# SMLC-NYSBC/TARGET-VAE

Hardware: AMD Instinct MI355X
Metric: training images/sec (fwd+bwd+Adam), P8 z=2 64x64 bs=256/GPU (higher is better)
Workload: dtype f32 (matrix products: operands as TWO fp16 parts under one power-of-two scale PER ROW of the operand (row / column of the product), 3 fp16 MFMAs per product block -- 2 where one operand is the exact 0 / 1 matrix -- fp32 accumulate: at least as accurate against fp64 as the fp32 matrix pipe (profiles/

## Files before the change

include/tvae_hip.h:

```cpp
#ifndef TVAE_HIP_H
#define TVAE_HIP_H
#ifdef __cplusplus
extern "C" {
#endif

typedef void* tvae_stream_t;

int tvae_abi_version(void);


int tvae_rotate_bank_fwd(const float* weight, const int* tap_idx, const float* tap_w, float* bank, int C, int Cin,
                         int ksz, int R, tvae_stream_t stream);
int tvae_rotate_bank_bwd(const float* dbank, const int* csr_ptr, const int* csr_r, const int* csr_dst,
                         const float* csr_w, float* dweight, int C, int Cin, int ksz, int R, int accumulate,
                         tvae_stream_t stream);

int tvae_conv1_fwd(const float* y, const float* bank, const float* bias, float* out, int B, int Cin, int n, int ksz,
                   int pad, int C, int R, int act, float slope, tvae_stream_t stream);
int tvae_conv1_wgrad(const float* y, const float* dpre, float* dbank, float* ws, long ws_floats, int B, int Cin,
                     int n, int ksz, int pad, int C, int R, tvae_stream_t stream);

int tvae_linear_fwd(const float* W, const float* X, const float* bias, const float* gbias, int group,
                    const float* res, float* Y, int M, int N, int K, long ldx, long ldy, int act, float slope,
                    tvae_stream_t stream);
int tvae_linear_dgrad(const float* W, const float* dpre, const float* add, const float* aux, float* dX, int M, int N,
                      int K, long ldd, long ldx, int mask, float slope, tvae_stream_t stream);
int tvae_linear_wgrad(const float* dpre, const float* X, float* dW, float* ws, long ws_floats, int M, int N, int K,
                      long ldd, long ldx, int accumulate, tvae_stream_t stream);

int tvae_rowdot_seg(const float* X, long ldx, const float* V, int no, int M, int N, int seglen, float* out, float* amax,
                    tvae_stream_t stream);
int tvae_seg_sum(const float* in, int S, long L, float* out, float scale, int accumulate, tvae_stream_t stream);
int tvae_coldot(const float* X, long ldx, int M, int N, const float* W, int wsm, int wso, const float* bias, int no,
                float* out, tvae_stream_t stream);
int tvae_outer_mask(const float* dy, int no, const float* W, int wsm, int wso, const float* H, long ldh, float* D,
                    long ldd, int M, int N, int act, float slope, tvae_stream_t stream);
int tvae_act_bwd(const float* dY, const float* Y, float* dpre, long n, int act, float slope, tvae_stream_t stream);

int tvae_conv1_x6_supported(int Cin, int n, int ksz, int pad);
long tvae_conv1_x6_bank_bytes(int C, int R, int Cin, int ksz);
long tvae_conv1_x6_dy_bytes(int B, int C, int R, int n, int ksz, int pad);
int tvae_bank_split3(const float* bank, void* a3, long a3_bytes, int C, int R, int Cin, int ksz, tvae_stream_t stream);
int tvae_conv1_fwd_x6(const float* y, const void* a3, const float* bias, float* out, int B, int Cin, int n, int ksz,
                      int pad, int C, int R, int act, float slope, tvae_stream_t stream);
int tvae_dy_split3(const float* dpre, void* d3, long d3_bytes, int B, int Cin, int n, int ksz, int pad, int C, int R,
                   tvae_stream_t stream);
int tvae_conv1_wgrad_x6(const float* y, const void* d3, float* dbank, float* ws, long ws_floats, int B, int Cin, int n,
                        int ksz, int pad, int C, int R, tvae_stream_t stream);

int tvae_conv1_dft_supported(int B, int Cin, int n, int ksz, int pad, int C, int R);
long tvae_conv1_dft_at_floats(int B, int Cin, int n, int ksz, int pad, int C, int R);
long tvae_conv1_dft_ws_floats(int B, int Cin, int n, int ksz, int pad, int C, int R);
int tvae_conv1_dft_frame(int B, int Cin, int n, int ksz, int pad, int C, int R);
int tvae_conv1_dft_ring(int B, int Cin, int n, int ksz, int pad, int C, int R);
int tvae_conv1_dft_route(int B, int Cin, int n, int ksz, int pad, int C, int R, int parts, int which);
int tvae_conv1_fwd_dft(const float* y, const float* bank, const float* bias, float* out, float* at, float* ws,
                       long ws_floats, int B, int Cin, int n, int ksz, int pad, int C, int R, int act, float slope,
                       int parts, tvae_stream_t stream);
int tvae_conv1_wgrad_dft(const float* dpre, const float* at, float* dbank, float* dbias, float* ws, long ws_floats, int B,
                         int Cin, int n, int ksz, int pad, int C, int R, int parts, tvae_stream_t stream);

long tvae_dense_x6_bytes(int rows, int K);
int tvae_dense_split3(const float* W, long ldw, void* a3, long a3_bytes, int rows, int K, int transpose,
                      const float* scale, float* rowsum, tvae_stream_t stream);
int tvae_dense_split2h(const float* W, long ldw, void* a3, long a3_bytes, int rows, int K, int transpose,
                       const float* scale, float* rowsum, tvae_stream_t stream);
int tvae_linear_fwd_x6(const void* w3, const float* X, const float* bias, const float* res, float* Y, int M, int N,
                       int K, long ldx, long ldy, int act, float slope, const float* col_w, const float* col_b,
                       float* col_y, const float* va_xr, const float* va_wc, const float* va_bc, const float* va_lb,
                       int va_np, void* sign_bits, int parts, const float* x_amax, float* y_amax, tvae_stream_t stream);
int tvae_linear_dgrad_x6(const void* w3t, const float* dpre, const float* add, const float* aux, float* dX, int M,
                         int N, int K, long ldd, long ldx, int mask, float slope, const float* in_xr,
                         const float* in_wc, float* in_gxr, float* in_part, long in_part_floats, const float* vg_wo,
                         const float* vg_gy, const float* vg_csum, const float* in_bc, const float* in_lb, int in_np,
                         float* rs_part, long rs_part_floats, const float* rs_wo, const float* rs_gysum, float* rs_db,
                         float* rs_dwo, int parts, const void* vg_bits, const float* rs_rowdot, const float* rs_bias,
                         const float* x_amax, float* y_amax, tvae_stream_t stream);
int tvae_dgrad_rowsum_total(const float* rs_part, int ntiles, int M, const float* rs_wo, const float* rs_gysum, float slope,
                            float* rs_db, float* rs_dwo, const float* rs_rowdot, const float* rs_bias, tvae_stream_t stream);
int tvae_dec_in_total(float* part, int B, int cpi, int F, float* Simg, float* dbc, float* dWc, tvae_stream_t stream);
long tvae_linear_wgrad_x6_ws_floats(int M, int N, int K);
int tvae_linear_wgrad_x6(const float* dpre, const float* X, float* dW, float* ws, long ws_floats, int M, int N, int K,
                         long ldd, long ldx, int accumulate, const float* vg_wo, const float* vg_gy, int vg_act,
                         float vg_slope, const float* va_xr, const float* va_wc, const float* va_bc, const float* va_lb,
                         int va_np, const void* vg_bits, int parts, const float* rd_w, long rd_ldw, float* rd_rowdot,
                         const float* a_amax, const float* x_amax, int x_amax_rows, tvae_stream_t stream);

int tvae_dec_out_bwd(const float* gy, int n_out, const float* Wo, const float* H, long ldh, float* D, long ldd, int F,
                     long N, int act, float slope, float* part, long part_floats, float* tot, tvae_stream_t stream);
int tvae_dec_in_bwd(const float* d, long ldd, const float* xr, const float* Wc, int F, int B, int Np, float* gxr,
                    float* Simg, float* dbc, float* dWc, float* part, long part_floats, tvae_stream_t stream);
int tvae_heads_fwd(const float* W, const float* X, long ldx, const float* bias, float* Y, long ldy, int nh, int C,
                   long N, tvae_stream_t stream);
int tvae_heads_bwd(const float* W, const float* dY, long ldy, const float* X, long ldx, float* dX, long lddx, int nh,
                   int C, long N, int act, float slope, float* part, long part_floats, float* tot,
                   tvae_stream_t stream);

int tvae_attn_head_fwd(const float* heads, long ldh, const float* E, const float* eps_z, const float* eps_t,
                       const float* p_r, const float* off, const float* p_tr, const float* grid, int B, int R, int P,
                       int zd, float sigma_p, float theta_off_scale, float* attn, float* q, float* a, float* z,
                       float* theta, float* dx, float* kl, float* part, long part_floats, tvae_stream_t stream);
int tvae_attn_head_bwd(const float* heads, long ldh, const float* q, const float* a, const float* eps_z,
                       const float* eps_t, const float* p_r, const float* off, const float* p_tr, const float* grid,
                       int B, int R, int P, int zd, float sigma_p, float theta_off_scale, const float* gz,
                       const float* gth, const float* gdx, const float* gkl, const float* g_attn, const float* g_q,
                       const float* g_a, float* dheads, float* part, long part_floats, tvae_stream_t stream);

int tvae_rot_pool_fwd(const float* A1, const float* fw, const float* fb, float* X, int C, int B, int R, int P,
                      tvae_stream_t stream);
int tvae_rot_pool_bwd(const float* A1, const float* dX, const float* fw, float* dA1, float* part, long part_floats,
                      float* dtot, int C, int B, int R, int P, int act, float slope, tvae_stream_t stream);

int tvae_enc_tail_fwd_x6(const void* w3, const float* A1, long lda, const float* b2, const float* Wh, const float* bh,
                         int nh, float* H, long ldh, float* heads, long ldo, void* bits_h, void* bits_a, int C, long N,
                         int act, float slope, int parts, const float* amax_a1, tvae_stream_t stream);
int tvae_enc_tail_dgrad_x6(const void* w3p, const void* wh3, const float* dheads, long ldd, int nh, const void* bits_h,
                           const void* bits_a, float* dA1, long lda, int C, long N, float slope, int parts,
                           tvae_stream_t stream);
long tvae_enc_tail_wgrad_x6_ws_floats(long N);
int tvae_enc_tail_wgrad_x6(const float* A1, long lda, const float* dheads, long ldd, int nh, const void* bits_h,
                           const float* Wh, float* dW2, float* ws, long ws_floats, int C, long N, float slope, int parts, const float* amax_a1,
                           tvae_stream_t stream);
int tvae_enc_tail_wide_max_rows(void);
int tvae_enc_tail_fwd_wide(const void* w3, const void* wh3, const float* A1, long lda, const float* b2, const float* bh, int nh,
                           float* H, long ldh, float* heads, long ldo, void* bits_h, void* bits_a, int C, long N, int act,
                           float slope, int parts, const float* amax_a1, tvae_stream_t stream);
int tvae_enc_tail_dgrad_wide(const void* wht3, const void* w3p, const float* dheads, long ldd, int nh, const void* bits_h,
                             const void* bits_a, float* dH, long ldh, float* dA1, long lda, int C, long N, float slope,
                             int parts, const float* amax_dheads, tvae_stream_t stream);
int tvae_enc_tail_wgrad_wide(const float* D, long ldd, int rows_d, const float* A, long lda, float* dW, float* ws,
                             long ws_floats, int C, long N, const float* amax_d, const float* amax_a, tvae_stream_t stream);
int tvae_get_latent(const float* heads, long ldh, const float* p_r, const float* off, const float* grid, int B, int R,
                    int P, int zd, float theta_off_scale, float* zc, float* theta_mu, float* dx, tvae_stream_t stream);

int tvae_coord_fwd(const float* xc, const float* dx, const float* theta, float* xr, int B, int Np,
                   tvae_stream_t stream);
int tvae_coord_bwd(const float* xc, const float* dx, const float* theta, const float* gxr, float* gdx, float* gtheta,
                   int B, int Np, tvae_stream_t stream);

int tvae_dec_l0_fwd(const float* xr, const float* Wc, const float* bc, const float* LB, float* h, long ldh, int F,
                    long Ntot, int Np, int act, float slope, tvae_stream_t stream);
int tvae_latent_bias(const float* Wl, const float* z, float* LB, int B, int F, int zd, tvae_stream_t stream);
int tvae_latent_bwd(const float* S, const float* Wl, const float* z, float* dWl, float* dz, int B, int F, int zd,
                    tvae_stream_t stream);
int tvae_fourier_fwd(const float* xr, const float* Wf, const float* bf, float sigma, float* feat, long ld, int F,
                     long Ntot, tvae_stream_t stream);
int tvae_fourier_bwd(const float* xr, const float* Wf, const float* bf, float sigma, const float* dfeat, long ld,
                     int F, long Ntot, float* gxr, tvae_stream_t stream);

int tvae_loglik_fwd(const float* yh, const float* y, float* lp, int B, int L, int kind, tvae_stream_t stream);
int tvae_loglik_bwd(const float* yh, const float* y, const float* glp, float* gyh, int B, int L, int kind,
                    tvae_stream_t stream);

int tvae_elbo_reduce(const float* lp, const float* kl, int B, double* elbo, float* logp, double* kld, tvae_stream_t stream);
int tvae_elbo_reduce_bwd(const double* g_elbo, const float* g_logp, const double* g_kld, int B, float* g_lp, float* g_kl,
                         tvae_stream_t stream);

int tvae_rccl_available(void);
int tvae_rccl_unique_id(void* id128);
int tvae_rccl_comm_init(void** comm, int nranks, const void* id128, int rank);
int tvae_allreduce_flat(void* comm, float* buf, long count, tvae_stream_t stream);
// ... 16 lines not shown
```

target-vae_amd/csrc/abi_common.hpp:

```cpp
#pragma once
#include <hip/hip_runtime.h>

#include <cstdlib>

#include "../../include/tvae_hip.h"
#include "gemm_f32_mfma.hpp"

#define TVAE_CHECK_LAUNCH()                      \
    do {                                         \
        hipError_t e__ = hipGetLastError();      \
        if (e__ != hipSuccess) return (int)e__;  \
    } while (0)

#define TVAE_INTERNAL __attribute__((visibility("hidden")))

namespace tvae {

static inline hipStream_t S(tvae_stream_t s) { return (hipStream_t)s; }
static inline bool aligned16(const void* p) { return (reinterpret_cast<size_t>(p) & 15) == 0; }
static inline int grid1d(long total, int block, int cap = 8192) {
    long g = (total + block - 1) / block;
    if (g < 1) g = 1;
    if (g > cap) g = cap;
    return (int)g;
}
template <class KernelT>
static hipError_t allow_big_lds(KernelT kernel, size_t bytes) {
    if (bytes <= 48 * 1024) return hipSuccess;
    return hipFuncSetAttribute(reinterpret_cast<const void*>(kernel), hipFuncAttributeMaxDynamicSharedMemorySize,
                               (int)bytes);
}
static inline int pick_splits(int tiles, long K) {
    long want = (1024 + tiles - 1) / tiles;
    long maxs = K / (4 * BK);
    if (maxs < 1) maxs = 1;
    if (want > maxs) want = maxs;
    if (want < 1) want = 1;
    return (int)want;
}
static inline int panels_of(long N, int width) { return (int)((N + width - 1) / width); }

static inline ConvGeom make_geom(int B, int Cin, int n, int ksz, int pad, int R) {
    ConvGeom g;
    g.B = B; g.Cin = Cin; g.n = n; g.ksz = ksz; g.pad = pad; g.R = R;
    g.Ho = n + 2 * pad - ksz + 1;
    g.P = g.Ho * g.Ho;
    g.K2 = ksz * ksz;
    return g;
}

static const size_t X6_LDS_MAX = 160 * 1024;

TVAE_INTERNAL int splitk_finalize(const float* ws, int splits, int M, int N, const Epilogue& ep, hipStream_t stream);

template <class AL, class BL>
static hipError_t launch_gemm(AL al, BL bl, const Epilogue& ep, int M, int N, int K, int splits_wanted,
                              float* ws, long ws_floats, hipStream_t stream) {
    if (M <= 0 || N <= 0) return hipSuccess;
    const int tilesM = cdiv(M, BM), tilesN = cdiv(N, BN);
    int splits = splits_wanted < 1 ? 1 : splits_wanted;
    if (splits > 1) {
        const long per = (long)M * N;
        const long cap = ws ? ws_floats / per : 0;
        if (cap < 2) splits = 1; else if (splits > cap) splits = (int)cap;
        if (splits > 65535) splits = 65535;
    }
    int kchunk = cdiv(cdiv(K > 0 ? K : 1, splits), BK) * BK;
    splits = cdiv(K > 0 ? K : 1, kchunk);
    const TileMap tm{tilesM, tilesN, splits};
    float* wsp = splits > 1 ? ws : nullptr;
    hipLaunchKernelGGL((gemm_f32_kernel<AL, BL>), dim3(tm.grid()), dim3(GEMM_THREADS), 0, stream, al, bl, ep, M, N, K,
                       kchunk, wsp, tm);
    hipError_t e = hipGetLastError();
    if (e != hipSuccess) return e;
    if (splits > 1) e = (hipError_t)splitk_finalize(ws, splits, M, N, ep, stream);
    return e;
}

}
```

target-vae_amd/csrc/abi_conv_dft.hip:

```cpp
#include "abi_dense_x6.hpp"
#include "conv_dft_kernels.hpp"
#include "conv_dft_h3_kernels.hpp"

using namespace tvae;

static __global__ void dft_zero_kernel(float4* __restrict__ p, long n4, float* __restrict__ tail, int ntail) {
    const float4 z = make_float4(0.f, 0.f, 0.f, 0.f);
    for (long i = (long)blockIdx.x * blockDim.x + threadIdx.x; i < n4; i += (long)gridDim.x * blockDim.x) p[i] = z;
    if (blockIdx.x == 0 && (int)threadIdx.x < ntail) tail[threadIdx.x] = 0.f;
}
static hipError_t dft_zero(float* p, long floats, hipStream_t st) {
    const long n4 = floats / 4;
    const int ntail = (int)(floats - 4 * n4);
    long blocks = (n4 + 255) / 256;
    if (blocks < 1) blocks = 1;
    if (blocks > 4096) blocks = 4096;
    hipLaunchKernelGGL(dft_zero_kernel, dim3((unsigned)blocks), dim3(256), 0, st, reinterpret_cast<float4*>(p), n4, p + 4 * n4,
                       ntail);
    return hipGetLastError();
}

static int dev_cu_count() {
    int dev = 0, n = 0;
    if (hipGetDevice(&dev) != hipSuccess) return 256;
// ... 374 lines not shown
    hipLaunchKernelGGL(dft_out_gen_kernel<N_>, dim3(grid), dim3(256), 0, st, (const float*)T, (const float*)EO, bias, out, \
                       q.M, R, B, q.Ho, q.Lh, q.NBpad, act, slope, a1max)
            switch (r_out - DFT_R_OUT_GEN) {
                case 1: TVAE_OUT_GEN(1); break;
                case 2: TVAE_OUT_GEN(2); break;
                case 3: TVAE_OUT_GEN(3); break;
                case 4: TVAE_OUT_GEN(4); break;
                default: TVAE_OUT_GEN(5); break;
            }
#undef TVAE_OUT_GEN
            TVAE_CHECK_LAUNCH();
            return 0;
        }
        if (r_out <= DFT_R_OUT_MF || r_out > DFT_R_OUT_MF + 9) return (int)hipErrorInvalidValue;
        const int mf_l = (r_out - DFT_R_OUT_MF - 1) / 3, mf_v = (r_out - DFT_R_OUT_MF - 1) % 3;
        const size_t lds_o = ((size_t)q.LHP * NTT * 64 + (size_t)4 * 32 * (q.Ho | 1)) * 4;
        const int grid = (int)((ntiles + 3) / 4 < 768 ? (ntiles + 3) / 4 : 768);
        const int iters = (int)((ntiles + 4L * grid - 1) / (4L * grid));
#define TVAE_OUT_MF(L_, N_, R_)                                                                                     \
    do {                                                                                                            \
        e = allow_big_lds(dft_out_mf_kernel<L_, N_, R_>, lds_o);                                                    \
        if (e != hipSuccess) return (int)e;                                                                         \
        hipLaunchKernelGGL((dft_out_mf_kernel<L_, N_, R_>), dim3(grid), dim3(256), lds_o, st, (const float*)T,      \
                           (const float*)EO, bias, out, q.M, R, B, q.Ho, q.Lh, q.NBpad, act, slope, iters, a1max); \
    } while (0)
#define TVAE_OUT_MF_L(L_)                                                                                           \
    do {                                                                                                            \
        if (mf_v == 1) TVAE_OUT_MF(L_, 1, true); else if (mf_v == 0) TVAE_OUT_MF(L_, 1, false); else TVAE_OUT_MF(L_, 2, false); \
    } while (0)
        if (mf_l == 0) TVAE_OUT_MF_L(23); else if (mf_l == 1) TVAE_OUT_MF_L(49); else TVAE_OUT_MF_L(64);
#undef TVAE_OUT_MF_L
#undef TVAE_OUT_MF
        TVAE_CHECK_LAUNCH();
    }
    return 0;
}

int tvae_conv1_wgrad_dft(const float* dpre, const float* at, float* dbank, float* dbias, float* ws, long ws_floats, int B,
                         int Cin, int n, int ksz, int pad, int C, int R, int parts, tvae_stream_t stream) {
    const DftPlan q = dft_plan(B, Cin, n, ksz, pad, C, R);
    const int r_dy = dft_route(q, parts, DFT_STEP_DY), r_wg = dft_route(q, parts, DFT_STEP_WGRAD_GEMM);
    if (r_dy < 0 || r_wg < 0 || ws_floats < tvae_conv1_dft_ws_floats(B, Cin, n, ksz, pad, C, R) || !aligned16(ws) ||
        !aligned16(at))
        return (int)hipErrorInvalidValue;
    hipStream_t st = S(stream);
    float* amax = const_cast<float*>(at) + ((q.at_floats + 3) & ~3L);
    float* smax = amax + q.o_smax;
    constexpr bool bf16_store = true;
    const bool s16 = bf16_store && parts == 1 && q.ring;
    const int rc0 = h3_zero_slots(smax, q.M, 256, st);
    if (rc0) return rc0;
    float* Sp = ws;
    float* slabs = Sp + ((q.t_floats + 3) & ~3L);
    float* tab = slabs + (((long)(q.splits > q.wsplits ? q.splits : q.wsplits) * q.g_floats + 3) & ~3L);
    float* EO = tab;
    float* ED = EO + ((q.eo_floats + 3) & ~3L);
    {
        hipLaunchKernelGGL(dft_wtab_kernel, dim3(64), dim3(256), 0, st, EO, ED, q.L, q.Lh, q.Ho, q.LHP, q.NT,
                           q.NT + q.REM1, q.NS, q.NRT, q.mixed ? 1.f / (float)q.L : 1.f / ((float)q.L * (float)q.L));
        TVAE_CHECK_LAUNCH();
        const long ntiles = (long)q.M * (q.NBpad / 32);
        if (r_dy == q.ring) {
            const int cus = dev_cu_count();
            const int grid = (int)((ntiles + 3) / 4 < 2 * cus ? (ntiles + 3) / 4 : 2 * cus);
            hipError_t er = hipSuccess;
#define TVAE_DY_RING_ONE(S_, T_, L2_, H_, Q_, S16_)                                                                  \
    do {                                                                                                            \
        const size_t lds_r = (size_t)4 * 2 * ((32 * H_ + 63) / 64) * 256;                                           \
        er = allow_big_lds(dft_dy_ring_kernel<S_, T_, L2_, H_, Q_, S16_>, lds_r);                                   \
        if (er != hipSuccess) return (int)er;                                                                       \
        hipLaunchKernelGGL((dft_dy_ring_kernel<S_, T_, L2_, H_, Q_, S16_>), dim3(grid), dim3(256), lds_r, st, dpre, \
                           (const float*)ED, Sp, q.M, R, B, q.Lh, q.NBpad, smax);                                   \
    } while (0)
#define TVAE_DY_RING(S_, T_, L2_, H_, Q_)                                                                           \
    do { if (s16) TVAE_DY_RING_ONE(S_, T_, L2_, H_, Q_, true); else TVAE_DY_RING_ONE(S_, T_, L2_, H_, Q_, false); } while (0)
            if (q.ring == 1) TVAE_DY_RING(9, 2, 38, 17, false);
            else if (q.ring == 2) TVAE_DY_RING(17, 3, 82, 33, false);
            else if (q.ring == 3) TVAE_DY_RING(20, 2, 62, 39, false);
            else if (q.ring == 4) TVAE_DY_RING(9, 2, 46, 17, false);
            else if (q.ring == 5) TVAE_DY_RING(17, 3, 98, 33, true);
            else TVAE_DY_RING(20, 3, 68, 39, false);
#undef TVAE_DY_RING
#undef TVAE_DY_RING_ONE
            TVAE_CHECK_LAUNCH();
        } else if (r_dy == DFT_R_H3) {
            uint4* EOc = reinterpret_cast<uint4*>(ED + ((q.ed_floats + 3) & ~3L) + ((q.M + 3) & ~3L));
            uint4* EDc = EOc + q.eoc_floats / 4;
            hipLaunchKernelGGL(dft_wtab_h3_kernel, dim3(64), dim3(256), 0, st, EOc, EDc, q.L, q.Lh, q.Ho, OH3_KS, OH3_NWT, DH3_WS,
                               DH3_NKT, q.mixed ? 1.f / (float)q.L : 1.f / ((float)q.L * (float)q.L));
            TVAE_CHECK_LAUNCH();
            const size_t lds_h = ((size_t)((32 * (q.Ho | 1) + 3) & ~3) + 2 * 2 * DH3_WS * 32 * 4 + 32) * 4;
            hipError_t eh = allow_big_lds(dft_dy_h3_kernel<DH3_WS, DH3_NKT, DH3_NLD>, lds_h);
            if (eh != hipSuccess) return (int)eh;
            const int cus = dev_cu_count();
            const int gridh = (int)(ntiles < 2L * cus ? ntiles : 2L * cus);
            hipLaunchKernelGGL((dft_dy_h3_kernel<DH3_WS, DH3_NKT, DH3_NLD>), dim3(gridh), dim3(64 * DH3_NKT), lds_h, st, dpre,
                               (const uint4*)EDc, Sp, q.M, R, B, q.Ho, q.Lh, q.NBpad, ldexpf(1.f, -14), smax);
            TVAE_CHECK_LAUNCH();
        } else if (r_dy >= DFT_R_DY_WIDE50 && r_dy <= DFT_R_DY_WIDE80) {
            const int NSR = r_dy == DFT_R_DY_WIDE50 ? 50 : (r_dy == DFT_R_DY_WIDE66 ? 66 : DFT_WIDE_NS);
            const size_t lds_w = (size_t)2 * (32 * (q.Ho | 1) + 2 * NSR + 2) * 4;
            const int cus = dev_cu_count();
            const long fit = (long)(150 * 1024 / lds_w);
            const long wg_per_cu = fit < 2 ? fit : 2;
            const int gridw = (int)(ntiles < wg_per_cu * cus ? ntiles : wg_per_cu * cus);
            hipError_t ew = hipSuccess;
#define TVAE_DY_WIDE(NSR_, NLD_, WPE_)                                                                               \
    do {                                                                                                            \
        ew = allow_big_lds(dft_dy_wide_kernel<NSR_, NLD_, WPE_>, lds_w);                                            \
        if (ew != hipSuccess) return (int)ew;                                                                       \
        hipLaunchKernelGGL((dft_dy_wide_kernel<NSR_, NLD_, WPE_>), dim3(gridw), dim3(64 * q.NRT), lds_w, st, dpre,  \
                           (const float*)ED, Sp, q.M, R, B, q.Ho, q.Lh, q.NBpad, q.NS, q.NRT, smax);                \
    } while (0)
            if (NSR == 50) TVAE_DY_WIDE(50, 16, 2);
            else if (NSR == 66) TVAE_DY_WIDE(66, 16, 2);
            else TVAE_DY_WIDE(DFT_WIDE_NS, 16, 2);
#undef TVAE_DY_WIDE
            TVAE_CHECK_LAUNCH();
        } else if (r_dy == DFT_R_DY_GEN) {
            const size_t lds_g = (size_t)4 * 32 * ((2 * q.NS) | 1) * 4;
            hipError_t eg = allow_big_lds(dft_dy_gen_kernel, lds_g);
            if (eg != hipSuccess) return (int)eg;
            const int gridg = (int)((ntiles + 3) / 4 < 4096 ? (ntiles + 3) / 4 : 4096);
            hipLaunchKernelGGL(dft_dy_gen_kernel, dim3(gridg), dim3(256), lds_g, st, dpre, (const float*)ED, Sp, q.M, R, B,
                               q.Ho, q.Lh, q.NBpad, q.NS, q.NRT, smax);
            TVAE_CHECK_LAUNCH();
        } else {
        if (r_dy <= DFT_R_DY_MF || r_dy > DFT_R_DY_MF + 5) return (int)hipErrorInvalidValue;
        const size_t lds_d = ((size_t)q.NS * q.NRT * 64 + (size_t)4 * (32 * ((2 * q.NS) | 1) + 64)) * 4;
        const int grid = (int)((ntiles + 3) / 4 < 768 ? (ntiles + 3) / 4 : 768);
        const int iters = (int)((ntiles + 4L * grid - 1) / (4L * grid));
        hipError_t e0 = hipSuccess;
#define TVAE_DY_MF(S_, T_, L2_, A_)                                                                                 \
    do {                                                                                                            \
        e0 = allow_big_lds(dft_dy_mf_kernel<S_, T_, L2_, A_>, lds_d);                                               \
        if (e0 != hipSuccess) return (int)e0;                                                                       \
        hipLaunchKernelGGL((dft_dy_mf_kernel<S_, T_, L2_, A_>), dim3(grid), dim3(256), lds_d, st, dpre,             \
                           (const float*)ED, Sp, q.M, R, B, q.Ho, q.Lh, q.NBpad, iters,                             \
                           smax);                                                        \
    } while (0)
        switch (r_dy - DFT_R_DY_MF) {
            case 1: TVAE_DY_MF(9, 2, 46, true); break;
            case 2: TVAE_DY_MF(9, 2, 0, true); break;
            case 3: TVAE_DY_MF(17, 4, 98, true); break;
            case 4: TVAE_DY_MF(17, 4, 0, true); break;
            default: TVAE_DY_MF(32, 4, 0, false); break;
        }
#undef TVAE_DY_MF
        TVAE_CHECK_LAUNCH();
        }
    }
    if (dbias) {
        float* dbpart = ED + ((q.ed_floats + 3) & ~3L);
        hipLaunchKernelGGL(dft_dbias_rows_kernel, dim3(q.M), dim3(256), 0, st, (const float*)Sp, dbpart, q.Lh, q.NB, q.M,
                           s16 ? 1 : 0);
        TVAE_CHECK_LAUNCH();
        hipLaunchKernelGGL(dft_dbias_kernel, dim3((C + 63) / 64), dim3(64), 0, st, (const float*)dbpart, dbias, R, C);
        TVAE_CHECK_LAUNCH();
    }
    const bool wide = r_wg == DFT_R_WG_WIDE;
    const int nslabs = wide ? q.wsplits : q.splits;
    {
        const int M2 = 2 * q.M;
        const int tiles_b = wide ? M2 / WW_ROWS : q.Mb / DX6_ROWS, tilesM = q.Lh * tiles_b;
        const int tilesK = wide ? (q.K2 <= 160 ? 1 : cdiv(q.K2, 192)) : cdiv(q.K2, 128);
        const int splits = nslabs;
        const int nchunk = cdiv(cdiv((int)q.NBpad, splits), 16) * 16;
        const TileMap tmk{tilesM, tilesK, splits};
        const DenseBatch bt{tiles_b, (long)q.K2 * q.NBpad, 0};
        int rc = dense_wgrad_x6_batched(Sp, (long)q.Lh * 128, at, q.NBpad, slabs, M2, q.K2, (int)q.NBpad, nchunk, tmk, bt,
                                        128L, ATile{7, 127, (long)M2 * q.Lh * 128}, parts, st,
                                        H3Scale{smax, amax + q.o_fmax, 1, 0, q.M, 1 << 30, 1}, s16, wide);
        if (rc) return rc;
    }
    constexpr bool dbank_mf = true;
    if (q.mixed) {
        hipError_t e = allow_big_lds(dft_dbank_x_kernel, q.lds_db);
        if (e != hipSuccess) return (int)e;
        hipLaunchKernelGGL(dft_dbank_x_kernel, dim3(q.M * Cin), dim3(256), q.lds_db, st, (const float*)slabs, nslabs, q.g_floats,
                           dbank, ksz, q.L, q.Lh, q.M, Cin);
    } else if (dbank_mf && ksz <= 64 && q.FXBd >= 17 && q.FXBd <= 64) {
        hipError_t e = allow_big_lds(dft_dbank_mf_kernel, q.lds_db);
        if (e != hipSuccess) return (int)e;
        hipLaunchKernelGGL(dft_dbank_mf_kernel, dim3(q.M * Cin), dim3(256), q.lds_db, st, (const float*)slabs, nslabs,
                           q.g_floats, dbank, ksz, q.L, q.Lh, q.M, Cin, q.FXBd);
    } else {
        hipError_t e = allow_big_lds(dft_dbank_kernel, q.lds_db);
        if (e != hipSuccess) return (int)e;
        hipLaunchKernelGGL(dft_dbank_kernel, dim3(q.M * Cin), dim3(256), q.lds_db, st, (const float*)slabs, nslabs, q.g_floats,
                           dbank, ksz, q.L, q.Lh, q.M, Cin, q.FXBd);
    }
    TVAE_CHECK_LAUNCH();
    return 0;
}

}
```

target-vae_amd/csrc/abi_dense_wgrad_x6.hip:

```cpp
#include "abi_dense_x6.hpp"

using namespace tvae;

namespace tvae {
static __global__ void dense_absmax_kernel(const float* __restrict__ W, long ldw, int Rrows, int K, int transpose,
                                           const float* __restrict__ scale, float* __restrict__ amax) {
    const long total = (long)Rrows * K;
    float mx = 0.f;
    if (!scale && (transpose ? ldw == Rrows : ldw == K) && (reinterpret_cast<size_t>(W) & 15) == 0) {
        const float4* w4 = reinterpret_cast<const float4*>(W);
        const long n4 = total / 4, gsz = (long)gridDim.x * blockDim.x;
        for (long i = (long)blockIdx.x * blockDim.x + threadIdx.x; i < n4; i += gsz) {
            const float4 v = w4[i];
            mx = fmaxf(fmaxf(mx, fabsf(v.x)), fmaxf(fabsf(v.y), fmaxf(fabsf(v.z), fabsf(v.w))));
        }
        for (long i = 4 * n4 + (long)blockIdx.x * blockDim.x + threadIdx.x; i < total; i += gsz) mx = fmaxf(mx, fabsf(W[i]));
        h3_block_amax(mx, amax);
        return;
    }
    for (long i = (long)blockIdx.x * blockDim.x + threadIdx.x; i < total; i += (long)gridDim.x * blockDim.x) {
        const int k = transpose ? (int)(i / Rrows) : (int)(i % K);
        const int row = transpose ? (int)(i % Rrows) : (int)(i / K);
        float v = transpose ? W[(long)k * ldw + row] : W[(long)row * ldw + k];
        if (scale) v *= scale[k];
        mx = fmaxf(mx, fabsf(v));
    }
    h3_block_amax(mx, amax);
}

int dense_wgrad_x6_batched(const float* dY, long ldd, const float* X, long ldx, float* slabs, int M, int Kf, int N,
                           int nchunk, const TileMap& tm, const DenseBatch& bt, long dy_stride, const ATile& atile,
                           int parts, hipStream_t st, H3Scale hs, bool a_bf16, bool wide) {
    const VirtGrad vg{nullptr, nullptr, 0, 0.f, nullptr, nullptr, nullptr, 0};
    const VirtAct va{nullptr, nullptr, nullptr, nullptr, 1, 0, 0.f};
    if (a_bf16) {
        if (parts != 1 || dy_stride % 2 != 0) return (int)hipErrorInvalidValue;
        return dense_wgrad_x6_launch_p1_abf(0, dY, ldd, X, ldx, slabs, M, Kf, N, nchunk, tm, bt, dy_stride, vg, va, atile, st, hs);
    }
    if (wide) {
        if (parts == 2 && hs.amax_a && hs.amax_x)
            return dense_wgrad_x6_wide_p2(dY, ldd, X, ldx, slabs, M, Kf, N, nchunk, tm, bt, dy_stride, atile, st, hs);
        if (parts == 3) return dense_wgrad_x6_wide_p3(dY, ldd, X, ldx, slabs, M, Kf, N, nchunk, tm, bt, dy_stride, atile, st, hs);
        return (int)hipErrorInvalidValue;
    }
    if (parts == 1) return dense_wgrad_x6_launch_p1(0, dY, ldd, X, ldx, slabs, M, Kf, N, nchunk, tm, bt, dy_stride, vg, va, atile, st, hs);
    if (parts == 2 && hs.amax_a && hs.amax_x)
        return dense_wgrad_x6_launch_p2(0, dY, ldd, X, ldx, slabs, M, Kf, N, nchunk, tm, bt, dy_stride, vg, va, atile, st, hs);
    if (parts == 3) return dense_wgrad_x6_launch_p3(0, dY, ldd, X, ldx, slabs, M, Kf, N, nchunk, tm, bt, dy_stride, vg, va, atile, st, hs);
    return (int)hipErrorInvalidValue;
}
}

namespace {
__global__ void wgrad_lrf_rowdot_kernel(int K, const float* __restrict__ wo, const float* __restrict__ W, long ldw,
                                        float* __restrict__ dW, float* __restrict__ rowdot) {
    __shared__ float sm[16];
    const int m = blockIdx.x;
    float acc[1] = {0.f};
    for (int k = threadIdx.x; k < K; k += blockDim.x) {
        const float g = dW[(long)m * K + k];
        dW[(long)m * K + k] = wo[m] * g;
        acc[0] = __fmaf_rn(W[(long)m * ldw + k], g, acc[0]);
    }
    block_sum<1>(acc, sm);
    if (threadIdx.x == 0) rowdot[m] = acc[0];
}
}

extern "C" {

static int wgrad_x6_splits(int M, int N, int K) {
    const int tilesM = cdiv(M, DX6_ROWS), tilesK = cdiv(K, 128);
    int splits = (2 * 256) / (tilesM * tilesK);
    if (splits > N / 16) splits = N / 16;
    if (splits < 2) splits = 2;
    const int nchunk = cdiv(cdiv(N, splits), 16) * 16;
    return cdiv(N, nchunk);
}
constexpr int WG_H3_SLOTS = 8;
long tvae_linear_wgrad_x6_ws_floats(int M, int N, int K) {
    if (M <= 0 || K <= 0 || N < 32) return 0;
    return (long)wgrad_x6_splits(M, N, K) * M * K + WG_H3_SLOTS + K;
}

int tvae_linear_wgrad_x6(const float* dpre, const float* X, float* dW, float* ws, long ws_floats, int M, int N, int K,
                         long ldd, long ldx, int accumulate, const float* vg_wo, const float* vg_gy, int vg_act,
                         float vg_slope, const float* va_xr, const float* va_wc, const float* va_bc, const float* va_lb,
                         int va_np, const void* vg_bits, int parts, const float* rd_w, long rd_ldw, float* rd_rowdot,
                         const float* a_amax, const float* x_amax, int x_amax_rows, tvae_stream_t stream) {
    if (M <= 0 || K <= 0) return 0;
    if (parts != 1 && parts != 2 && parts != 3) return (int)hipErrorInvalidValue;
    const bool from_bits = vg_bits && vg_wo && vg_act == ACT_LRELU;
    const bool h3_recomp = from_bits && va_xr && vg_gy;
    const bool h3_bits_mem = from_bits && !va_xr && vg_gy && x_amax;
    const bool h3_plain = !vg_wo && !va_xr && !vg_bits && a_amax && x_amax;
    if (parts == 2 && !(h3_recomp || h3_bits_mem || h3_plain)) return (int)hipErrorInvalidValue;
    if (vg_bits && !from_bits) return (int)hipErrorInvalidValue;
    if (N <= 0 || N % 16 != 0 || !ws || (from_bits ? N % 32 != 0 : (ldd % 4 != 0 || !dpre || !aligned16(dpre))))
        return (int)hipErrorInvalidValue;
    if (va_xr ? (va_np % 16 != 0 || !aligned16(va_xr))
            : (ldx % 4 != 0 || !X || !aligned16(X)))
        return (int)hipErrorInvalidValue;
    if (rd_rowdot && (!rd_w || !(vg_wo && vg_act == ACT_LRELU) || accumulate)) return (int)hipErrorInvalidValue;
    const VirtGrad vgs{vg_wo, vg_gy, vg_act, vg_slope, nullptr, (const unsigned*)vg_bits, nullptr, rd_rowdot ? 1 : 0};
    const VirtAct vas{va_xr, va_wc, va_bc, va_lb, va_np > 0 ? va_np : 1, vg_act, vg_slope};
    const int tilesM = cdiv(M, DX6_ROWS), tilesK = cdiv(K, 128);
    const long per = (long)M * K;
    if (N < 32 || ws_floats < tvae_linear_wgrad_x6_ws_floats(M, N, K)) return (int)hipErrorInvalidValue;
    const int splits = wgrad_x6_splits(M, N, K);
    const int nchunk = cdiv(cdiv(N, splits), 16) * 16;
    if (splits < 2) return (int)hipErrorInvalidValue;
    const TileMap tmk{tilesM, tilesK, splits};
    const bool lrf = vg_wo && vg_act == ACT_LRELU;
    const int variant = (vg_wo ? 1 : 0) | (va_xr ? 2 : 0) | (lrf ? (from_bits ? 8 : 4) : 0);
    int rc;
    if (parts == 2 && !h3_recomp) {
        rc = dense_wgrad_x6_launch_p2(variant, dpre, ldd, X, ldx, ws, M, K, N, nchunk, tmk, DenseBatch{0, 0, 0}, 0L, vgs, vas,
                                      ATILE_PLAIN, S(stream),
                                      H3Scale{a_amax, x_amax, 0, 0, 0, x_amax_rows ? 1 : 0, x_amax_rows ? K : 0});
    } else if (parts == 2) {
        float* slots = ws + (long)splits * per;
        rc = h3_zero_slots(slots, 4 + K, 256, S(stream));
        if (rc) return rc;
        const long nlb = va_lb ? (long)(N / vas.Np) * K : 0;
        rc = dec_l0_bound(va_xr, N, va_wc, va_bc, va_lb, nlb, K, slots, S(stream));
        if (rc) return rc;
        hipLaunchKernelGGL(dense_absmax_kernel, dim3(grid1d((long)N, 256 * 8, 512)), dim3(256), 0, S(stream), vg_gy, (long)N, 1, N,
                           0, (const float*)nullptr, slots + 3);
        TVAE_CHECK_LAUNCH();
        rc = dense_wgrad_x6_launch_p2(variant, dpre, ldd, X, ldx, ws, M, K, N, nchunk, tmk, DenseBatch{0, 0, 0}, 0L, vgs, vas,
                                      ATILE_PLAIN, S(stream), H3Scale{nullptr, slots, 0, 0, 0, 0, 0});
    } else {
        rc = parts == 1
            ? dense_wgrad_x6_launch_p1(variant, dpre, ldd, X, ldx, ws, M, K, N, nchunk, tmk, DenseBatch{0, 0, 0}, 0L, vgs, vas, ATILE_PLAIN, S(stream), H3_NONE)
            : dense_wgrad_x6_launch_p3(variant, dpre, ldd, X, ldx, ws, M, K, N, nchunk, tmk, DenseBatch{0, 0, 0}, 0L, vgs, vas, ATILE_PLAIN, S(stream), H3_NONE);
    }
    if (rc) return rc;
    TVAE_CHECK_LAUNCH();
    Epilogue ep;
    ep.C = dW; ep.ldc = K;
    ep.accumulate = accumulate;
    rc = splitk_finalize(ws, splits, M, K, ep, S(stream));
    if (rc) return rc;
    if (rd_rowdot) {
        hipLaunchKernelGGL(wgrad_lrf_rowdot_kernel, dim3(M), dim3(128), 0, S(stream), K, vg_wo, rd_w, rd_ldw, dW, rd_rowdot);
        TVAE_CHECK_LAUNCH();
    }
    return 0;
}

}
```

target-vae_amd/csrc/abi_dense_x6.hip:

```cpp
#include "abi_dense_x6.hpp"
#include "dense_prepass_kernels.hpp"

using namespace tvae;

namespace {
struct Dx6Instance {
    int xv, epi, parts;
    int (*launch)(TVAE_DX6_LAUNCH_ARGS);
};
const Dx6Instance DX6_INSTANCES[] = {
#define TVAE_DX6(XV_, E_, NP_) {XV_, E_, NP_, dense_x6_launch<XV_, E_, NP_>},
#include "dense_x6_instances.def"
#undef TVAE_DX6
};
int dense_x6_dispatch(int xv, int epi, int parts, TVAE_DX6_LAUNCH_ARGS) {
    for (const Dx6Instance& i : DX6_INSTANCES)
        if (i.xv == xv && i.epi == epi && i.parts == parts)
            return i.launch(a3, X, ldx, ep, M, Mpad, N, K, K8pad, tm, bt, cd, it, vg, va, st, hs);
    return (int)hipErrorInvalidValue;
}
}

namespace tvae {
int h3_zero_slots(float* p, int n, int threads, hipStream_t st) {
    hipLaunchKernelGGL(h3_zero_slots_kernel, dim3(1), dim3(threads), 0, st, p, n);
    return (int)hipGetLastError();
}
int dense_split2h(const float* W, long ldw, uint4* a3, int rows, int Rpad, int K, int K8pad, int transpose, const float* scale,
                  const float* rowmax, hipStream_t st) {
    if (!transpose && K8pad <= 48)
        hipLaunchKernelGGL(dense_split2h_rows_kernel, dim3(Rpad / 32), dim3(256), (size_t)32 * K8pad * 32, st, W, ldw, a3, rows,
                           Rpad, K, K8pad, scale, rowmax);
    else
        hipLaunchKernelGGL(dense_split2h_kernel, dim3(grid1d((long)K8pad * Rpad, 256)), dim3(256), 0, st, W, ldw, a3, rows, Rpad,
                           K, K8pad, transpose, scale, rowmax);
    return (int)hipGetLastError();
}
int dec_l0_bound(const float* xr, int N, const float* wc, const float* bc, const float* lb, long nlb, int K, float* slots,
                 hipStream_t st) {
    hipLaunchKernelGGL(dec_l0_bound_kernel, dim3(grid1d(N / 2, 256, 512)), dim3(256), 0, st, xr, 2L * N, wc, bc, lb, nlb, K,
                       slots);
    return (int)hipGetLastError();
}

int dense_x6_batched(const void* w3, const float* X, long ldx, const Epilogue& ep, int rows_per_problem, int rows_total,
                     int N, int K, const TileMap& tm, const DenseBatch& bt, int parts, hipStream_t st, H3Scale hs) {
    const int Rpad = x6_round_up(rows_total, DX6_ROWS), K8pad = dense_k8pad(K);
    if (N % 128 != 0 || !aligned16(w3)) return (int)hipErrorInvalidValue;
    if (parts != 1 && parts != 2 && parts != 3) return (int)hipErrorInvalidValue;
    if (parts == 2 && (!hs.amax_a || !hs.amax_x)) return (int)hipErrorInvalidValue;
    const bool lean = !ep.bias && !ep.res && !ep.aux && ep.act == ACT_NONE && ep.mask == ACT_NONE && ep.ctile > 0 && ep.C &&
                      !ep.accumulate && !ep.amax_out && rows_per_problem % DX6_ROWS == 0 && ep.ldc * 8 * 4 < (1L << 31);
    return dense_x6_dispatch(0, lean ? 4 : 0, parts, (const uint4*)w3, X, ldx, ep, rows_per_problem, Rpad, N, K, K8pad, tm, bt,
                             ColDot{nullptr, nullptr, nullptr},
                             InTail{nullptr, nullptr, nullptr, nullptr, nullptr, nullptr, 1},
                             VirtGrad{nullptr, nullptr, 0, 0.f, nullptr, nullptr, nullptr, 0},
                             VirtAct{nullptr, nullptr, nullptr, nullptr, 1, 0, 0.f}, st, hs);
}
int dense_x6_batched4(const void* w3, const float* X, long ldx, const Epilogue& ep, int rows_per_problem, int rows_total,
                      int N, int K, const TileMap& tm, const DenseBatch& bt, int parts, hipStream_t st, H3Scale hs, bool out_bf16) {
    const int Rpad = x6_round_up(rows_total, DX6_ROWS), K8pad = dense_k8pad(K);
    if (N % 128 != 0 || !aligned16(w3) || (parts != 1 && parts != 2 && parts != 3)) return (int)hipErrorInvalidValue;
    if (parts == 2 && (!hs.amax_a || !hs.amax_x)) return (int)hipErrorInvalidValue;
    const bool lean = !ep.bias && !ep.res && !ep.aux && ep.act == ACT_NONE && ep.mask == ACT_NONE && ep.ctile > 0 && ep.C &&
                      !ep.accumulate && rows_per_problem % DX4_ROWS == 0 && ep.ldc * 8 * 4 < (1L << 31);
#define TVAE_DX4_LAUNCH(NP_, E_)                                                                                       \
    hipLaunchKernelGGL((dense_x6_plain4_kernel<NP_, E_>), dim3(tm.grid()), dim3(DX4_THREADS), 0, st, (const uint4*)w3, X, ldx, \
                       ep, rows_per_problem, Rpad, N, K, K8pad, tm, bt, hs)
    if (out_bf16) {
        if (!lean || parts != 1) return (int)hipErrorInvalidValue;
        TVAE_DX4_LAUNCH(1, 2);
        return (int)hipGetLastError();
    }
    if (parts == 3) { if (lean) TVAE_DX4_LAUNCH(3, 1); else TVAE_DX4_LAUNCH(3, 0); }
    else if (parts == 2) { if (lean) TVAE_DX4_LAUNCH(2, 1); else TVAE_DX4_LAUNCH(2, 0); }
    else { if (lean) TVAE_DX4_LAUNCH(1, 1); else TVAE_DX4_LAUNCH(1, 0); }
#undef TVAE_DX4_LAUNCH
    return (int)hipGetLastError();
}
bool dense_x6_batched_xres(const void* w3, const float* X, long ldx, const Epilogue& ep, int rows_per_problem, int Mb, int nprob,
                           int N, int K, long x_stride, long c_stride, int parts, hipStream_t st, H3Scale hs, int* rc) {
    constexpr bool on = true;
    const int K8pad = dense_k8pad(K), nk = K8pad / 2;
    const size_t lds = (size_t)nk * parts * 256 * 16 + (size_t)(Mb + 128) * 4;
    const bool lean = !ep.bias && !ep.res && !ep.aux && ep.act == ACT_NONE && ep.mask == ACT_NONE && ep.ctile > 0 && ep.C &&
                      !ep.accumulate && rows_per_problem % DX6_ROWS == 0 && ep.ldc * 8 * 4 < (1L << 31);
    if (!on || !lean || !dense_x6_xres_fits(rows_per_problem, Mb, N, K, parts) || !aligned16(w3) ||
        (parts == 2 && (!hs.amax_a || !hs.amax_x)))
        return false;
    const int Rpad = x6_round_up(nprob * Mb, DX6_ROWS), tilesN = N / 128, nch = 4, cs = cdiv(tilesN, nch);
    const unsigned grid = 8u * cdiv(nprob * nch, 8) * cs;
#define TVAE_XRES_LAUNCH(NP_, NK_)                                                                                     \
    do {                                                                                                               \
        hipError_t e_ = allow_big_lds(dense_x6_xres_kernel<NP_, NK_>, lds);                                            \
        if (e_ != hipSuccess) { *rc = (int)e_; return true; }                                                          \
        hipLaunchKernelGGL((dense_x6_xres_kernel<NP_, NK_>), dim3(grid), dim3(256), lds, st, (const uint4*)w3, X, ldx, ep.C,  \
                           ep.ldc, ep.ctile, rows_per_problem, Mb, Rpad, K, nprob, tilesN, nch, x_stride, c_stride, hs);  \
    } while (0)
    if (nk == 12) { if (parts == 3) TVAE_XRES_LAUNCH(3, 12); else TVAE_XRES_LAUNCH(2, 12); }
    else if (nk == 10) { if (parts == 3) TVAE_XRES_LAUNCH(3, 10); else TVAE_XRES_LAUNCH(2, 10); }
    else { if (parts == 3) TVAE_XRES_LAUNCH(3, 8); else TVAE_XRES_LAUNCH(2, 8); }
#undef TVAE_XRES_LAUNCH
    *rc = (int)hipGetLastError();
    return true;
}
}

namespace {
__global__ void dgrad_rowsum_total_kernel(const float* __restrict__ part, int ntiles, int K, const float* __restrict__ wo,
                                          const float* __restrict__ gysum, float slope, float* __restrict__ db,
                                          float* __restrict__ dwo, const float* __restrict__ rowdot,
                                          const float* __restrict__ bias) {
    __shared__ float sm[2 * 16];
    const int m = blockIdx.x;
    float s[2] = {0.f, 0.f};
    for (int t = threadIdx.x; t < ntiles; t += blockDim.x) {
        const float2 v = *reinterpret_cast<const float2*>(part + ((long)m * ntiles + t) * 2);
        s[0] += v.x;
        if (!rowdot) s[1] += v.y;
    }
    block_sum<2>(s, sm);
    if (threadIdx.x == 0) {
        const float g0 = __fmaf_rn(1.f - slope, s[0], slope * gysum[0]);
        db[m] = wo[m] * g0;
        dwo[m] = rowdot ? __fmaf_rn(bias ? bias[m] : 0.f, g0, rowdot[m]) : s[1];
    }
}
}

extern "C" {

long tvae_dense_x6_bytes(int rows, int K) { return dense_x6_bytes(rows, K); }
static int dense_split(const float* W, long ldw, void* a3, long a3_bytes, int rows, int K, int transpose,
                       const float* scale, float* rowsum, int parts, tvae_stream_t stream) {
    if (rows <= 0 || K <= 0) return 0;
    if (a3_bytes < tvae_dense_x6_bytes(rows, K) || !aligned16(a3)) return (int)hipErrorInvalidValue;
    const int Rpad = x6_round_up(rows, DX6_ROWS), K8pad = dense_k8pad(K);
    const long total = (long)K8pad * Rpad;
    if (parts == 2) {
        float* tr = h3_trailer(a3, rows, K);
        if (transpose)
            hipLaunchKernelGGL(dense_rowmax_kernel, dim3(Rpad / 64), dim3(1024), 0, S(stream), W, ldw, rows, Rpad, K, transpose,
                               scale, tr);
        else
            hipLaunchKernelGGL(dense_rowmax_rows_kernel, dim3(Rpad / 4), dim3(256), 0, S(stream), W, ldw, rows, Rpad, K, scale, tr);
        TVAE_CHECK_LAUNCH();
        const int rc = dense_split2h(W, ldw, (uint4*)a3, rows, Rpad, K, K8pad, transpose, scale, tr, S(stream));
        if (rc) return rc;
    } else {
        hipLaunchKernelGGL(dense_split3_kernel, dim3(grid1d(total, 256)), dim3(256), 0, S(stream), W, ldw, (uint4*)a3, rows,
                           Rpad, K, K8pad, transpose, scale);
        TVAE_CHECK_LAUNCH();
    }
    if (rowsum) {
        hipLaunchKernelGGL(dense_rowsum_kernel, dim3((rows + 63) / 64), dim3(1024), 0, S(stream), W, ldw, rows, K, transpose,
                           scale, rowsum);
        TVAE_CHECK_LAUNCH();
    }
    return 0;
}
int tvae_dense_split3(const float* W, long ldw, void* a3, long a3_bytes, int rows, int K, int transpose,
                      const float* scale, float* rowsum, tvae_stream_t stream) {
    return dense_split(W, ldw, a3, a3_bytes, rows, K, transpose, scale, rowsum, 3, stream);
}
int tvae_dense_split2h(const float* W, long ldw, void* a3, long a3_bytes, int rows, int K, int transpose,
                       const float* scale, float* rowsum, tvae_stream_t stream) {
    return dense_split(W, ldw, a3, a3_bytes, rows, K, transpose, scale, rowsum, 2, stream);
}
static int launch_dense_x6(const void* a3, const float* X, long ldx, const Epilogue& ep, int rows, int N, int K, int parts,
                           hipStream_t st, ColDot cd = ColDot{nullptr, nullptr, nullptr},
                           InTail it = InTail{nullptr, nullptr, nullptr, nullptr, nullptr, nullptr, 1},
                           VirtGrad vg = VirtGrad{nullptr, nullptr, 0, 0.f, nullptr, nullptr, nullptr, 0},
                           VirtAct va = VirtAct{nullptr, nullptr, nullptr, nullptr, 1, 0, 0.f}, const float* x_amax = nullptr) {
    if ((cd.w || it.xr) && rows > DX6_ROWS) return (int)hipErrorInvalidValue;
    if (rows <= 0 || N <= 0) return 0;
    if (N % 128 != 0 || !aligned16(a3) || (parts != 1 && parts != 2 && parts != 3)) return (int)hipErrorInvalidValue;
    const int Rpad = x6_round_up(rows, DX6_ROWS), K8pad = dense_k8pad(K);
    TileMap tm{Rpad / DX6_ROWS, N / 128, 1};
    tm.pack = 1;
    H3Scale hs = H3_NONE;
    if (parts == 2) {
        float* tr = h3_trailer(a3, rows, K);
        hs.amax_a = tr;
        hs.a_rows = 1;
        if (va.xr) {
            float* bw = tr + Rpad;
            int rc = h3_zero_slots(bw, 4 + K, 256, st);
            if (rc) return rc;
            const long nlb = va.lb ? (long)(N / va.Np) * K : 0;
            rc = dec_l0_bound(va.xr, N, va.wc, va.bc, va.lb, nlb, K, bw, st);
            if (rc) return rc;
            hs.amax_x = bw;
        } else if (x_amax && !vg.wo && !vg.csum) {
            hs.amax_x = x_amax;
        } else if (!vg.csum) {
            return (int)hipErrorInvalidValue;
        }
    }
    if ((va.xr && (K > 512 || va.Np % 128 != 0 || vg.wo || vg.csum)) || (vg.csum && (!vg.gy || vg.act != ACT_LRELU)) || (it.bc && it.Np % 128 != 0) ||
        (!va.xr && !X && !(vg.bits && vg.csum && vg.rpart)))
        return (int)hipErrorInvalidValue;
    const DenseBatch nb{0, 0, 0};
    if (vg.csum && vg.rpart && vg.bits) {
        if (K > DX6_ROWS || N % 32 != 0) return (int)hipErrorInvalidValue;
        if (rows == DX6_ROWS && !ep.C && it.xr && it.bc && !ep.res && ep.mask == ACT_LRELU && !cd.w && !cd.bits)
            return dense_x6_dispatch(5, 2, parts, (const uint4*)a3, X, ldx, ep, rows, Rpad, N, K, K8pad, tm, nb, cd, it, vg, va, st, hs);
        if (rows % DX6_ROWS == 0 && ep.C && !it.xr && !ep.res && ep.mask == ACT_LRELU && ep.aux && !cd.w && !cd.bits && !ep.ctile &&
            ep.ldc * 8 * 4 < (1L << 31) && ep.ldaux * 8 * 4 < (1L << 31))
            return dense_x6_dispatch(5, 3, parts, (const uint4*)a3, X, ldx, ep, rows, Rpad, N, K, K8pad, tm, nb, cd, it, vg, va, st, hs);
        return dense_x6_dispatch(5, 0, parts, (const uint4*)a3, X, ldx, ep, rows, Rpad, N, K, K8pad, tm, nb, cd, it, vg, va, st, hs);
    }
    if (vg.csum && vg.rpart) {
        if (K > DX6_ROWS) return (int)hipErrorInvalidValue;
        return dense_x6_dispatch(4, 0, parts, (const uint4*)a3, X, ldx, ep, rows, Rpad, N, K, K8pad, tm, nb, cd, it, vg, va, st, hs);
    }
    if (vg.csum) return dense_x6_dispatch(3, 0, parts, (const uint4*)a3, X, ldx, ep, rows, Rpad, N, K, K8pad, tm, nb, cd, it, vg, va, st, hs);
    if (va.xr && rows == DX6_ROWS && !ep.C && cd.w && !it.xr && !ep.res && ep.mask == ACT_NONE && ep.act == ACT_LRELU)
        return dense_x6_dispatch(2, 1, parts, (const uint4*)a3, X, ldx, ep, rows, Rpad, N, K, K8pad, tm, nb, cd, it, vg, va, st, hs);
    if (va.xr) return dense_x6_dispatch(2, 0, parts, (const uint4*)a3, X, ldx, ep, rows, Rpad, N, K, K8pad, tm, nb, cd, it, vg, va, st, hs);
    if (!vg.wo && X && rows == DX6_ROWS && N % 128 == 0 && !ep.C && cd.w && !it.xr && !ep.res && ep.mask == ACT_NONE &&
        ep.act == ACT_LRELU)
        return dense_x6_dispatch(0, 1, parts, (const uint4*)a3, X, ldx, ep, rows, Rpad, N, K, K8pad, tm, nb, cd, it, vg, va, st, hs);
    if (vg.wo) return dense_x6_dispatch(1, 0, parts, (const uint4*)a3, X, ldx, ep, rows, Rpad, N, K, K8pad, tm, nb, cd, it, vg, va, st, hs);
    if (X && rows % DX6_ROWS == 0 && ep.C && !ep.res && !cd.w && !cd.bits && !it.xr && !ep.ctile && !ep.accumulate && !ep.gbias &&
        ((ep.mask == ACT_NONE && (ep.act == ACT_LRELU || ep.act == ACT_NONE)) || (ep.mask == ACT_LRELU && ep.aux && ep.act == ACT_NONE && !ep.bias)) &&
        ep.ldc * 8 * 4 < (1L << 31) && ep.ldaux * 8 * 4 < (1L << 31))
        return dense_x6_dispatch(0, 3, parts, (const uint4*)a3, X, ldx, ep, rows, Rpad, N, K, K8pad, tm, nb, cd, it, vg, va, st, hs);
    return dense_x6_dispatch(0, 0, parts, (const uint4*)a3, X, ldx, ep, rows, Rpad, N, K, K8pad, tm, nb, cd, it, vg, va, st, hs);
}
int tvae_linear_fwd_x6(const void* w3, const float* X, const float* bias, const float* res, float* Y, int M, int N,
                       int K, long ldx, long ldy, int act, float slope, const float* col_w, const float* col_b,
                       float* col_y, const float* va_xr, const float* va_wc, const float* va_bc, const float* va_lb,
                       int va_np, void* sign_bits, int parts, const float* x_amax, float* y_amax, tvae_stream_t stream) {
    Epilogue ep;
    ep.C = Y; ep.ldc = ldy;
    if (y_amax && (!Y || col_w || sign_bits)) return (int)hipErrorInvalidValue;
    ep.amax_out = y_amax;
    if (sign_bits && (act != ACT_LRELU || N % 32 != 0)) return (int)hipErrorInvalidValue;
    ep.bias = bias;
    ep.res = res; ep.ldres = ldy;
    ep.act = act; ep.slope = slope;
    return launch_dense_x6(w3, X, ldx, ep, M, N, K, parts, S(stream), ColDot{col_w, col_b, col_y, (unsigned*)sign_bits},
                           InTail{nullptr, nullptr, nullptr, nullptr, nullptr, nullptr, 1}, VirtGrad{nullptr, nullptr, 0, 0.f, nullptr, nullptr, nullptr, 0},
                           VirtAct{va_xr, va_wc, va_bc, va_lb, va_np > 0 ? va_np : 1, act, slope}, x_amax);
}
int tvae_linear_dgrad_x6(const void* w3t, const float* dpre, const float* add, const float* aux, float* dX, int M,
                         int N, int K, long ldd, long ldx, int mask, float slope, const float* in_xr,
                         const float* in_wc, float* in_gxr, float* in_part, long in_part_floats, const float* vg_wo,
                         const float* vg_gy, const float* vg_csum, const float* in_bc, const float* in_lb, int in_np,
                         float* rs_part, long rs_part_floats, const float* rs_wo, const float* rs_gysum, float* rs_db,
                         float* rs_dwo, int parts, const void* vg_bits, const float* rs_rowdot, const float* rs_bias,
                         const float* x_amax, float* y_amax, tvae_stream_t stream) {
    Epilogue ep;
    ep.C = dX; ep.ldc = ldx;
    if (y_amax && (!dX || in_xr)) return (int)hipErrorInvalidValue;
    ep.amax_out = y_amax;
    ep.res = add; ep.ldres = ldx;
    ep.aux = aux; ep.ldaux = ldx;
    ep.mask = (aux || in_bc) ? mask : ACT_NONE; ep.slope = slope;
    if (in_bc && !in_xr) return (int)hipErrorInvalidValue;
    if (in_xr) {
        if (!in_wc || !in_gxr || !in_part || in_part_floats < (long)(N / 128) * K * 3) return (int)hipErrorInvalidValue;
    } else if (!dX) {
        return (int)hipErrorInvalidValue;
    }
    if (vg_bits && !(vg_csum && rs_part && (rs_rowdot || !rs_db) && N % 32 == 0))
        return (int)hipErrorInvalidValue;
    if (rs_rowdot && !vg_bits) return (int)hipErrorInvalidValue;
    if (rs_part) {
        if (!vg_csum || !vg_gy || !rs_wo || !rs_gysum || (!rs_db != !rs_dwo) || M > DX6_ROWS || N % 128 != 0 ||
            rs_part_floats < (long)(N / 128) * M * 2 || (reinterpret_cast<size_t>(rs_part) & 7))
            return (int)hipErrorInvalidValue;
    }
    int rc = launch_dense_x6(w3t, dpre, ldd, ep, K, N, M, parts, S(stream), ColDot{nullptr, nullptr, nullptr},
                             InTail{in_xr, in_wc, in_gxr, in_part, in_bc, in_lb, in_np > 0 ? in_np : 1},
                             VirtGrad{vg_wo, vg_gy, mask, slope, vg_csum, (const unsigned*)vg_bits, rs_part, 0},
                             VirtAct{nullptr, nullptr, nullptr, nullptr, 1, 0, 0.f}, x_amax);
    if (rc || !rs_part || !rs_db || N <= 0 || K <= 0) return rc;
    hipLaunchKernelGGL(dgrad_rowsum_total_kernel, dim3(M), dim3(256), 0, S(stream), (const float*)rs_part, N / 128, M, rs_wo,
                       rs_gysum, slope, rs_db, rs_dwo, rs_rowdot, rs_bias);
    TVAE_CHECK_LAUNCH();
    return 0;
}
int tvae_dgrad_rowsum_total(const float* rs_part, int ntiles, int M, const float* rs_wo, const float* rs_gysum, float slope,
                            float* rs_db, float* rs_dwo, const float* rs_rowdot, const float* rs_bias, tvae_stream_t stream) {
    if (!rs_part || !rs_wo || !rs_gysum || !rs_db || !rs_dwo || ntiles <= 0 || M <= 0) return (int)hipErrorInvalidValue;
    hipLaunchKernelGGL(dgrad_rowsum_total_kernel, dim3(M), dim3(256), 0, S(stream), rs_part, ntiles, M, rs_wo, rs_gysum, slope,
                       rs_db, rs_dwo, rs_rowdot, rs_bias);
    TVAE_CHECK_LAUNCH();
    return 0;
}


}
```

target-vae_amd/csrc/abi_dense_x6.hpp:

```cpp
#pragma once
#include "abi_common.hpp"
#include "dense_x6_kernels.hpp"

namespace tvae {

static inline int dense_k8pad(int K) { return x6_round_up((K + 7) / 8, 2); }
static inline long dense_x6_bytes(int rows, int K) {
    const long Rpad = x6_round_up(rows, DX6_ROWS), K8pad = dense_k8pad(K);
    return 3 * K8pad * Rpad * 16;
}

static inline bool dense_x6_xres_fits(int rows_per_problem, int Mb, int N, int K, int parts) {
    const int nk = dense_k8pad(K) / 2;
    const size_t lds = (size_t)nk * parts * 256 * 16 + (size_t)(Mb + 128) * 4;
    return (parts == 2 || parts == 3) && (nk == 12 || nk == 10 || nk == 8) && N % 128 == 0 && rows_per_problem % DX6_ROWS == 0 &&
           Mb >= rows_per_problem && lds <= X6_LDS_MAX;
}

static inline float* h3_trailer(const void* a3, int rows, int K) {
    const long total = (long)dense_k8pad(K) * x6_round_up(rows, DX6_ROWS);
    return reinterpret_cast<float*>(const_cast<void*>(a3)) + 2 * total * 4;
}

#define TVAE_DX6_LAUNCH_ARGS                                                                                          \
    const uint4 *a3, const float *X, long ldx, const Epilogue &ep, int M, int Mpad, int N, int K, int K8pad,          \
        const TileMap &tm, const DenseBatch &bt, const ColDot &cd, const InTail &it, const VirtGrad &vg,              \
        const VirtAct &va, hipStream_t st, const H3Scale &hs
template <int XV, int EPI, int NP>
TVAE_INTERNAL int dense_x6_launch(TVAE_DX6_LAUNCH_ARGS);

#define TVAE_WG_LAUNCH_ARGS                                                                                           \
    int variant, const float *dY, long ldd, const float *X, long ldx, float *ws, int M, int Kf, int N, int nchunk,     \
        const TileMap &tm, const DenseBatch &bt, long dy_stride, const VirtGrad &vg, const VirtAct &va,               \
        const ATile &atile, hipStream_t st, const H3Scale &hs
TVAE_INTERNAL int dense_wgrad_x6_launch_p3(TVAE_WG_LAUNCH_ARGS);
TVAE_INTERNAL int dense_wgrad_x6_launch_p2(TVAE_WG_LAUNCH_ARGS);
TVAE_INTERNAL int dense_wgrad_x6_launch_p1(TVAE_WG_LAUNCH_ARGS);
TVAE_INTERNAL int dense_wgrad_x6_launch_p1_abf(TVAE_WG_LAUNCH_ARGS);

#define TVAE_WGW_LAUNCH_ARGS                                                                                          \
    const float *dY, long ldd, const float *X, long ldx, float *ws, int M, int Kf, int N, int nchunk, const TileMap &tm, \
        const DenseBatch &bt, long dy_stride, const ATile &atile, hipStream_t st, const H3Scale &hs
TVAE_INTERNAL int dense_wgrad_x6_wide_p3(TVAE_WGW_LAUNCH_ARGS);
TVAE_INTERNAL int dense_wgrad_x6_wide_p2(TVAE_WGW_LAUNCH_ARGS);

TVAE_INTERNAL int h3_zero_slots(float* p, int n, int threads, hipStream_t st);
TVAE_INTERNAL int dense_split2h(const float* W, long ldw, uint4* a3, int rows, int Rpad, int K, int K8pad, int transpose,
                                const float* scale, const float* rowmax, hipStream_t st);
TVAE_INTERNAL int dec_l0_bound(const float* xr, int N, const float* wc, const float* bc, const float* lb, long nlb, int K,
                               float* slots, hipStream_t st);

TVAE_INTERNAL int dense_x6_batched4(const void* w3, const float* X, long ldx, const Epilogue& ep, int rows_per_problem,
                                    int rows_total, int N, int K, const TileMap& tm, const DenseBatch& bt, int parts,
                                    hipStream_t st, H3Scale hs = H3_NONE, bool out_bf16 = false);
TVAE_INTERNAL bool dense_x6_batched_xres(const void* w3, const float* X, long ldx, const Epilogue& ep, int rows_per_problem,
                                         int Mb, int nprob, int N, int K, long x_stride, long c_stride, int parts,
                                         hipStream_t st, H3Scale hs, int* rc);
TVAE_INTERNAL int dense_x6_batched(const void* w3, const float* X, long ldx, const Epilogue& ep, int rows_per_problem,
                                   int rows_total, int N, int K, const TileMap& tm, const DenseBatch& bt, int parts,
                                   hipStream_t st, H3Scale hs = H3_NONE);
TVAE_INTERNAL int dense_wgrad_x6_batched(const float* dY, long ldd, const float* X, long ldx, float* slabs, int M,
                                         int Kf, int N, int nchunk, const TileMap& tm, const DenseBatch& bt,
                                         long dy_stride, const ATile& atile, int parts, hipStream_t st,
                                         H3Scale hs = H3_NONE, bool a_bf16 = false, bool wide = false);

}
```

target-vae_amd/csrc/abi_small.hip:

```cpp
#include "abi_common.hpp"
#include "small_kernels.hpp"
#include "rotate_bank_kernels.hpp"
#include "fused_tail_kernels.hpp"

using namespace tvae;

template <int NO>
static void launch_heads_fwd(const float* W, const float* X, long ldx, const float* bias, float* Y, long ldy, int C,
                             long N, int vec, hipStream_t st) {
    hipLaunchKernelGGL(heads_fwd_kernel<NO>, dim3(panels_of(N, 1024)), dim3(256), 0, st, W, X, ldx, bias, Y, ldy, C, N,
                       vec);
}
template <int NO>
static void launch_heads_bwd(const float* W, const float* dY, long ldy, const float* X, long ldx, float* dX, long lddx,
                             int C, long N, int act, float slope, float* part, int vec, hipStream_t st) {
    hipLaunchKernelGGL(heads_bwd_kernel<NO>, dim3(panels_of(N, PANEL8)), dim3(256), 0, st, W, dY, ldy, X, ldx, dX, lddx,
                       C, N, act, slope, part, vec);
}

extern "C" {

int tvae_abi_version(void) { return 7; }

int tvae_rotate_bank_fwd(const float* weight, const int* tap_idx, const float* tap_w, float* bank, int C, int Cin,
                         int ksz, int R, tvae_stream_t stream) {
    const int k2 = ksz * ksz;
    const long total = (long)C * R * Cin * k2;
    if (total >= 2147483647L || !aligned16(tap_idx) || !aligned16(tap_w)) return (int)hipErrorInvalidValue;
    const long npair = (long)C * Cin;
    if ((npair + RB_CH - 1) / RB_CH > 65535) return (int)hipErrorInvalidValue;
    const int npx32 = (ksz + 31) / 32, npy8 = (ksz + 7) / 8;
    hipLaunchKernelGGL(rotate_bank_fwd_kernel, dim3((unsigned)(R * npx32 * npy8), (unsigned)((npair + RB_CH - 1) / RB_CH)),
                       dim3(256), 0, S(stream), weight, tap_idx, tap_w, bank, C, Cin, ksz, R);
    TVAE_CHECK_LAUNCH();
    return 0;
}

int tvae_rotate_bank_bwd(const float* dbank, const int* csr_ptr, const int* csr_r, const int* csr_dst,
                         const float* csr_w, float* dweight, int C, int Cin, int ksz, int R, int accumulate,
                         tvae_stream_t stream) {
    const int k2 = ksz * ksz;
    const long total = (long)C * Cin * k2;
    if (total * R >= 2147483647L) return (int)hipErrorInvalidValue;
    const long npair = (long)C * Cin;
    if (k2 > (1 << 24) || R > 127) return (int)hipErrorInvalidValue;
    const int npx = (ksz + 7) / 8;
    const bool big = (long)npx * npx * ((npair + 15) / 16) >= 512;
    const int ppw = big ? 16 : 8;
    if ((npair + ppw - 1) / ppw > 65535) return (int)hipErrorInvalidValue;
    const dim3 grid((unsigned)(npx * npx), (unsigned)((npair + ppw - 1) / ppw));
    if (big)
        hipLaunchKernelGGL(rotate_bank_bwd_kernel<4>, grid, dim3(256), 0, S(stream), dbank, csr_ptr, csr_r, csr_dst, csr_w, dweight,
                           C, Cin, ksz, R, accumulate);
    else
        hipLaunchKernelGGL(rotate_bank_bwd_kernel<2>, grid, dim3(256), 0, S(stream), dbank, csr_ptr, csr_r, csr_dst, csr_w, dweight,
                           C, Cin, ksz, R, accumulate);
    TVAE_CHECK_LAUNCH();
    return 0;
}
int tvae_rowdot_seg(const float* X, long ldx, const float* V, int no, int M, int N, int seglen, float* out, float* amax,
                    tvae_stream_t stream) {
    if (seglen <= 0 || M <= 0) return (int)hipErrorInvalidValue;
    const int nseg = (N + seglen - 1) / seglen;
    dim3 grid(M, nseg), block(256);
    if (!V) no = 1;
    switch (no) {
        case 1: hipLaunchKernelGGL(rowdot_seg_kernel<1>, grid, block, 0, S(stream), X, ldx, V, N, seglen, out, M, amax); break;
        case 2: hipLaunchKernelGGL(rowdot_seg_kernel<2>, grid, block, 0, S(stream), X, ldx, V, N, seglen, out, M, amax); break;
        case 3: hipLaunchKernelGGL(rowdot_seg_kernel<3>, grid, block, 0, S(stream), X, ldx, V, N, seglen, out, M, amax); break;
        case 4: hipLaunchKernelGGL(rowdot_seg_kernel<4>, grid, block, 0, S(stream), X, ldx, V, N, seglen, out, M, amax); break;
        default: return (int)hipErrorInvalidValue;
    }
    TVAE_CHECK_LAUNCH();
    return 0;
}

int tvae_seg_sum(const float* in, int S_, long L, float* out, float scale, int accumulate, tvae_stream_t stream) {
    if (L <= 64 && S_ >= 32)
        hipLaunchKernelGGL(seg_sum_wave_kernel, dim3((unsigned)L), dim3(64), 0, S(stream), in, S_, L, out, scale, accumulate);
    else if (S_ >= 64 && L <= 65536)
        hipLaunchKernelGGL(seg_sum_tile_kernel, dim3((unsigned)((L + 63) / 64)), dim3(1024), 0, S(stream), in, S_, L, out, scale,
                           accumulate);
    else
        hipLaunchKernelGGL(seg_sum_kernel, dim3(grid1d(L, 256)), dim3(256), 0, S(stream), in, S_, L, out, scale, accumulate);
    TVAE_CHECK_LAUNCH();
    return 0;
}

int tvae_elbo_reduce(const float* lp, const float* kl, int B, double* elbo, float* logp, double* kld, tvae_stream_t stream) {
    if (B <= 0 || !lp || !kl || !elbo || !logp || !kld) return (int)hipErrorInvalidValue;
    hipLaunchKernelGGL(elbo_reduce_kernel, dim3(1), dim3(256), 0, S(stream), lp, kl, B, elbo, logp, kld);
    TVAE_CHECK_LAUNCH();
    return 0;
}
int tvae_elbo_reduce_bwd(const double* g_elbo, const float* g_logp, const double* g_kld, int B, float* g_lp, float* g_kl,
                         tvae_stream_t stream) {
    if (B <= 0 || !g_lp || !g_kl) return (int)hipErrorInvalidValue;
    hipLaunchKernelGGL(elbo_reduce_bwd_kernel, dim3((B + 255) / 256), dim3(256), 0, S(stream), g_elbo, g_logp, g_kld, B, g_lp, g_kl);
    TVAE_CHECK_LAUNCH();
    return 0;
}

int tvae_coldot(const float* X, long ldx, int M, int N, const float* W, int wsm, int wso, const float* bias, int no,
                float* out, tvae_stream_t stream) {
    dim3 grid((N + 255) / 256), block(256);
    const size_t sh = (size_t)M * no * sizeof(float);
    switch (no) {
        case 1: hipLaunchKernelGGL(coldot_kernel<1>, grid, block, sh, S(stream), X, ldx, M, N, W, wsm, wso, bias, out); break;
        case 2: hipLaunchKernelGGL(coldot_kernel<2>, grid, block, sh, S(stream), X, ldx, M, N, W, wsm, wso, bias, out); break;
        case 3: hipLaunchKernelGGL(coldot_kernel<3>, grid, block, sh, S(stream), X, ldx, M, N, W, wsm, wso, bias, out); break;
        case 4: hipLaunchKernelGGL(coldot_kernel<4>, grid, block, sh, S(stream), X, ldx, M, N, W, wsm, wso, bias, out); break;
        default: return (int)hipErrorInvalidValue;
    }
    TVAE_CHECK_LAUNCH();
    return 0;
}

int tvae_outer_mask(const float* dy, int no, const float* W, int wsm, int wso, const float* H, long ldh, float* D,
                    long ldd, int M, int N, int act, float slope, tvae_stream_t stream) {
    dim3 grid((N + 255) / 256, (M + 15) / 16), block(256);
    switch (no) {
        case 1: hipLaunchKernelGGL(outer_mask_kernel<1>, grid, block, 0, S(stream), dy, W, wsm, wso, H, ldh, D, ldd, M, N, act, slope); break;
        case 2: hipLaunchKernelGGL(outer_mask_kernel<2>, grid, block, 0, S(stream), dy, W, wsm, wso, H, ldh, D, ldd, M, N, act, slope); break;
        case 3: hipLaunchKernelGGL(outer_mask_kernel<3>, grid, block, 0, S(stream), dy, W, wsm, wso, H, ldh, D, ldd, M, N, act, slope); break;
        case 4: hipLaunchKernelGGL(outer_mask_kernel<4>, grid, block, 0, S(stream), dy, W, wsm, wso, H, ldh, D, ldd, M, N, act, slope); break;
        default: return (int)hipErrorInvalidValue;
    }
    TVAE_CHECK_LAUNCH();
    return 0;
}


int tvae_dec_out_bwd(const float* gy, int n_out, const float* Wo, const float* H, long ldh, float* D, long ldd, int F,
                     long N, int act, float slope, float* part, long part_floats, float* tot, tvae_stream_t stream) {
    if (F <= 0 || N <= 0) return 0;
    const int np = panels_of(N, PANEL16);
    if (n_out < 1 || n_out > 4 || part_floats < (long)np * F * (1 + n_out)) return (int)hipErrorInvalidValue;
    const int vec = (aligned16(H) && (!D || aligned16(D)) && ldh % 4 == 0 && ldd % 4 == 0) ? 1 : 0;
    int fs = np >= 1024 ? 1 : (1024 + np - 1) / np;
    if (fs > F / 16) fs = F / 16 > 0 ? F / 16 : 1;
    dim3 grid(np, fs), block(256);
    switch (n_out) {
        case 1: hipLaunchKernelGGL(dec_out_bwd_kernel<1>, grid, block, 0, S(stream), gy, Wo, H, ldh, D, ldd, F, N, act, slope, part, vec); break;
        case 2: hipLaunchKernelGGL(dec_out_bwd_kernel<2>, grid, block, 0, S(stream), gy, Wo, H, ldh, D, ldd, F, N, act, slope, part, vec); break;
        case 3: hipLaunchKernelGGL(dec_out_bwd_kernel<3>, grid, block, 0, S(stream), gy, Wo, H, ldh, D, ldd, F, N, act, slope, part, vec); break;
        default: hipLaunchKernelGGL(dec_out_bwd_kernel<4>, grid, block, 0, S(stream), gy, Wo, H, ldh, D, ldd, F, N, act, slope, part, vec); break;
    }
    TVAE_CHECK_LAUNCH();
    hipLaunchKernelGGL(part_total_kernel, dim3(F), dim3(256), 0, S(stream), (const float*)part, np, F, 1 + n_out, tot);
    TVAE_CHECK_LAUNCH();
    return 0;
}

int tvae_dec_in_bwd(const float* d, long ldd, const float* xr, const float* Wc, int F, int B, int Np, float* gxr,
                    float* Simg, float* dbc, float* dWc, float* part, long part_floats, tvae_stream_t stream) {
    if (F <= 0 || B <= 0 || Np <= 0) return 0;
    const int cpi = panels_of(Np, PANEL16);
    if (part_floats < (long)B * cpi * F * 3) return (int)hipErrorInvalidValue;
    const int vec = (aligned16(d) && ldd % 4 == 0 && Np % 4 == 0) ? 1 : 0;
    hipLaunchKernelGGL(dec_in_bwd_kernel, dim3(B * cpi), dim3(256), 0, S(stream), d, ldd, xr, Wc, F, Np, cpi, gxr, part,
                       vec);
    TVAE_CHECK_LAUNCH();
    return tvae_dec_in_total(part, B, cpi, F, Simg, dbc, dWc, stream);
}

int tvae_heads_fwd(const float* W, const float* X, long ldx, const float* bias, float* Y, long ldy, int nh, int C,
                   long N, tvae_stream_t stream) {
    if (N <= 0 || C <= 0) return 0;
    if (nh < 1 || nh > 8) return (int)hipErrorInvalidValue;
    const int vec = (aligned16(X) && aligned16(Y) && ldx % 4 == 0 && ldy % 4 == 0) ? 1 : 0;
    switch (nh) {
        case 1: launch_heads_fwd<1>(W, X, ldx, bias, Y, ldy, C, N, vec, S(stream)); break;
        case 2: launch_heads_fwd<2>(W, X, ldx, bias, Y, ldy, C, N, vec, S(stream)); break;
        case 3: launch_heads_fwd<3>(W, X, ldx, bias, Y, ldy, C, N, vec, S(stream)); break;
        case 4: launch_heads_fwd<4>(W, X, ldx, bias, Y, ldy, C, N, vec, S(stream)); break;
        case 5: launch_heads_fwd<5>(W, X, ldx, bias, Y, ldy, C, N, vec, S(stream)); break;
        case 6: launch_heads_fwd<6>(W, X, ldx, bias, Y, ldy, C, N, vec, S(stream)); break;
        case 7: launch_heads_fwd<7>(W, X, ldx, bias, Y, ldy, C, N, vec, S(stream)); break;
        default: launch_heads_fwd<8>(W, X, ldx, bias, Y, ldy, C, N, vec, S(stream)); break;
    }
    TVAE_CHECK_LAUNCH();
    return 0;
}

int tvae_heads_bwd(const float* W, const float* dY, long ldy, const float* X, long ldx, float* dX, long lddx, int nh,
                   int C, long N, int act, float slope, float* part, long part_floats, float* tot,
                   tvae_stream_t stream) {
    if (N <= 0 || C <= 0) return 0;
    const int np = panels_of(N, PANEL8);
    if (nh < 1 || nh > 8 || part_floats < (long)np * C * (nh + 1)) return (int)hipErrorInvalidValue;
    const int vec = (aligned16(X) && (!dX || aligned16(dX)) && aligned16(dY) && ldx % 4 == 0 && lddx % 4 == 0 && ldy % 4 == 0) ? 1 : 0;
    switch (nh) {
        case 1: launch_heads_bwd<1>(W, dY, ldy, X, ldx, dX, lddx, C, N, act, slope, part, vec, S(stream)); break;
        case 2: launch_heads_bwd<2>(W, dY, ldy, X, ldx, dX, lddx, C, N, act, slope, part, vec, S(stream)); break;
        case 3: launch_heads_bwd<3>(W, dY, ldy, X, ldx, dX, lddx, C, N, act, slope, part, vec, S(stream)); break;
        case 4: launch_heads_bwd<4>(W, dY, ldy, X, ldx, dX, lddx, C, N, act, slope, part, vec, S(stream)); break;
        case 5: launch_heads_bwd<5>(W, dY, ldy, X, ldx, dX, lddx, C, N, act, slope, part, vec, S(stream)); break;
        case 6: launch_heads_bwd<6>(W, dY, ldy, X, ldx, dX, lddx, C, N, act, slope, part, vec, S(stream)); break;
        case 7: launch_heads_bwd<7>(W, dY, ldy, X, ldx, dX, lddx, C, N, act, slope, part, vec, S(stream)); break;
        default: launch_heads_bwd<8>(W, dY, ldy, X, ldx, dX, lddx, C, N, act, slope, part, vec, S(stream)); break;
    }
    TVAE_CHECK_LAUNCH();
    const long used = (long)np * C * (nh + 1), mv = (long)C * (nh + 1);
    if (np >= 4 * PT_GROUPS && mv % 4 == 0 && part_floats >= ((used + 3) & ~3L) + PT_GROUPS * mv && aligned16(part)) {
        float* partial = part + ((used + 3) & ~3L);
        hipLaunchKernelGGL(part_total_s1_kernel, dim3(PT_GROUPS), dim3(256), 0, S(stream), (const float*)part, np, (int)(mv / 4),
                           partial);
        TVAE_CHECK_LAUNCH();
        hipLaunchKernelGGL(part_total_s2_kernel, dim3((unsigned)((mv + 255) / 256)), dim3(256), 0, S(stream),
                           (const float*)partial, C, nh + 1, tot);
        TVAE_CHECK_LAUNCH();
        return 0;
    }
    hipLaunchKernelGGL(part_total_kernel, dim3(C), dim3(256), 0, S(stream), (const float*)part, np, C, nh + 1, tot);
    TVAE_CHECK_LAUNCH();
    return 0;
}

int tvae_act_bwd(const float* dY, const float* Y, float* dpre, long n, int act, float slope, tvae_stream_t stream) {
    hipLaunchKernelGGL(act_bwd_kernel, dim3(grid1d(n, 256)), dim3(256), 0, S(stream), dY, Y, dpre, n, act, slope);
    TVAE_CHECK_LAUNCH();
    return 0;
}

static HeadParams make_head(const float* heads, long ldh, const float* E, const float* eps_z, const float* eps_t,
                            const float* p_r, const float* off, const float* p_tr, const float* grid, int R, int P,
                            int zd, float sigma_p, float theta_off_scale) {
    HeadParams hp;
    hp.heads = heads; hp.ldh = ldh; hp.E = E; hp.eps_z = eps_z; hp.eps_t = eps_t;
    hp.p_r = p_r; hp.off = off; hp.p_tr = p_tr; hp.grid = grid;
    hp.R = R; hp.P = P; hp.zd = zd; hp.sigma_p = sigma_p; hp.theta_off_scale = theta_off_scale;
    return hp;
}

static int head_chunks(int B, int RP, int zd, long part_floats, int per_chunk_floats, int& chunk) {
    chunk = RP;
    if (B >= 128 || RP < 16384 || zd > 64) return 1;
    int G = (RP + 4095) / 4096;
    const int cap = 1024 / (B > 0 ? B : 1);
    if (G > cap) G = cap;
    if (G < 2 || part_floats < (long)B * G * per_chunk_floats) return 1;
    chunk = (RP + G - 1) / G;
    return (RP + chunk - 1) / chunk;
}

int tvae_attn_head_fwd(const float* heads, long ldh, const float* E, const float* eps_z, const float* eps_t,
                       const float* p_r, const float* off, const float* p_tr, const float* grid, int B, int R, int P,
                       int zd, float sigma_p, float theta_off_scale, float* attn, float* q, float* a, float* z,
                       float* theta, float* dx, float* kl, float* part, long part_floats, tvae_stream_t stream) {
    if (B <= 0) return 0;
    HeadParams hp = make_head(heads, ldh, E, eps_z, eps_t, p_r, off, p_tr, grid, R, P, zd, sigma_p, theta_off_scale);
    int chunk;
    const int G = part ? head_chunks(B, R * P, zd, part_floats, head_part_floats(zd), chunk) : 1;
    if (G > 1) {
        hipLaunchKernelGGL(attn_head_fwd_a_kernel, dim3(B * G), dim3(1024), 0, S(stream), hp, G, chunk, attn, part);
        TVAE_CHECK_LAUNCH();
        hipLaunchKernelGGL(attn_head_fwd_b_kernel, dim3(B * G), dim3(1024), 0, S(stream), hp, G, chunk, (const float*)attn,
                           q, a, part);
        TVAE_CHECK_LAUNCH();
        hipLaunchKernelGGL(attn_head_fwd_c_kernel, dim3(B), dim3(256), 0, S(stream), hp, B, G, (const float*)part, z, theta,
                           dx, kl);
        TVAE_CHECK_LAUNCH();
        return 0;
    }
    hipLaunchKernelGGL(attn_head_fwd_kernel, dim3(B), dim3(1024), 0, S(stream), hp, attn, q, a, z, theta, dx, kl);
    TVAE_CHECK_LAUNCH();
    return 0;
}

int tvae_attn_head_bwd(const float* heads, long ldh, const float* q, const float* a, const float* eps_z,
                       const float* eps_t, const float* p_r, const float* off, const float* p_tr, const float* grid,
                       int B, int R, int P, int zd, float sigma_p, float theta_off_scale, const float* gz,
                       const float* gth, const float* gdx, const float* gkl, const float* g_attn, const float* g_q,
                       const float* g_a, float* dheads, float* part, long part_floats, tvae_stream_t stream) {
    if (B <= 0) return 0;
    HeadParams hp = make_head(heads, ldh, nullptr, eps_z, eps_t, p_r, off, p_tr, grid, R, P, zd, sigma_p,
                              theta_off_scale);
    int chunk;
    const int G = part ? head_chunks(B, R * P, zd, part_floats, 2, chunk) : 1;
    if (G > 1) {
        hipLaunchKernelGGL(attn_head_bwd_a_kernel, dim3(B * G), dim3(1024), 0, S(stream), hp, G, chunk, q, a, gz, gth, gdx,
                           gkl, g_q, g_a, part);
        TVAE_CHECK_LAUNCH();
        hipLaunchKernelGGL(attn_head_bwd_b_kernel, dim3(B * G), dim3(1024), 0, S(stream), hp, G, chunk, q, a, gz, gth, gdx,
                           gkl, g_attn, g_q, g_a, (const float*)part, dheads);
        TVAE_CHECK_LAUNCH();
        return 0;
    }
    hipLaunchKernelGGL(attn_head_bwd_kernel, dim3(B), dim3(1024), 0, S(stream), hp, q, a, gz, gth, gdx, gkl, g_attn,
                       g_q, g_a, dheads);
    TVAE_CHECK_LAUNCH();
    return 0;
}

int tvae_rot_pool_fwd(const float* A1, const float* fw, const float* fb, float* X, int C, int B, int R, int P,
                      tvae_stream_t stream) {
    if ((long)C * B * P <= 0) return 0;
    if (R < 1 || R > 16) return (int)hipErrorInvalidValue;
    hipLaunchKernelGGL(rot_pool_fwd_kernel, dim3(grid1d((long)C * B * P, 256)), dim3(256), 0, S(stream), A1, fw, fb, X, C, B,
                       R, P);
    TVAE_CHECK_LAUNCH();
    return 0;
}

int tvae_rot_pool_bwd(const float* A1, const float* dX, const float* fw, float* dA1, float* part, long part_floats,
                      float* dtot, int C, int B, int R, int P, int act, float slope, tvae_stream_t stream) {
    if ((long)C * B * P <= 0) return 0;
    const int nb = grid1d((long)C * B * P, 256, 1024);
    if (R < 1 || R > 16 || part_floats < (long)(R + 1) * nb) return (int)hipErrorInvalidValue;
    hipLaunchKernelGGL(rot_pool_bwd_kernel, dim3(nb), dim3(256), 0, S(stream), A1, dX, fw, dA1, part, C, B, R, P, act, slope);
    TVAE_CHECK_LAUNCH();
    hipLaunchKernelGGL(seg_sum_kernel, dim3(1), dim3(64), 0, S(stream), (const float*)part, nb, (long)(R + 1), dtot, 1.f, 0);
    TVAE_CHECK_LAUNCH();
    return 0;
}

int tvae_get_latent(const float* heads, long ldh, const float* p_r, const float* off, const float* grid, int B, int R,
                    int P, int zd, float theta_off_scale, float* zc, float* theta_mu, float* dx, tvae_stream_t stream) {
    if (B <= 0) return 0;
    HeadParams hp = make_head(heads, ldh, nullptr, nullptr, nullptr, p_r, off, nullptr, grid, R, P, zd, 1.f,
                              theta_off_scale);
    hipLaunchKernelGGL(get_latent_kernel, dim3(B), dim3(1024), 0, S(stream), hp, zc, theta_mu, dx);
    TVAE_CHECK_LAUNCH();
    return 0;
}

int tvae_coord_fwd(const float* xc, const float* dx, const float* theta, float* xr, int B, int Np,
                   tvae_stream_t stream) {
    hipLaunchKernelGGL(coord_fwd_kernel, dim3(grid1d((long)B * Np, 256)), dim3(256), 0, S(stream), xc, dx, theta, xr,
                       B, Np);
    TVAE_CHECK_LAUNCH();
    return 0;
}

int tvae_coord_bwd(const float* xc, const float* dx, const float* theta, const float* gxr, float* gdx, float* gtheta,
                   int B, int Np, tvae_stream_t stream) {
    if (B <= 0) return 0;
    hipLaunchKernelGGL(coord_bwd_kernel, dim3(B), dim3(256), 0, S(stream), xc, dx, theta, gxr, gdx, gtheta, Np);
    TVAE_CHECK_LAUNCH();
    return 0;
}

int tvae_dec_l0_fwd(const float* xr, const float* Wc, const float* bc, const float* LB, float* h, long ldh, int F,
                    long Ntot, int Np, int act, float slope, tvae_stream_t stream) {
    dim3 grid((unsigned)((Ntot + 255) / 256), (F + 15) / 16), block(256);
    hipLaunchKernelGGL(dec_l0_fwd_kernel, grid, block, 0, S(stream), xr, Wc, bc, LB, h, ldh, F, Ntot, Np, act, slope);
    TVAE_CHECK_LAUNCH();
    return 0;
}

int tvae_latent_bias(const float* Wl, const float* z, float* LB, int B, int F, int zd, tvae_stream_t stream) {
    hipLaunchKernelGGL(latent_bias_kernel, dim3((B * F + 255) / 256), dim3(256), 0, S(stream), Wl, z, LB, B, F, zd);
    TVAE_CHECK_LAUNCH();
    return 0;
}

int tvae_latent_bwd(const float* S_, const float* Wl, const float* z, float* dWl, float* dz, int B, int F, int zd,
                    tvae_stream_t stream) {
    const int tot = (F * zd > B * zd) ? F * zd : B * zd;
    if (tot <= 0) return 0;
    hipLaunchKernelGGL(latent_bwd_kernel, dim3((tot + 63) / 64), dim3(1024), 0, S(stream), S_, Wl, z, dWl, dz, B, F, zd);
    TVAE_CHECK_LAUNCH();
    return 0;
}

int tvae_fourier_fwd(const float* xr, const float* Wf, const float* bf, float sigma, float* feat, long ld, int F,
                     long Ntot, tvae_stream_t stream) {
    dim3 grid((unsigned)((Ntot + 255) / 256), (F + 15) / 16), block(256);
    hipLaunchKernelGGL(fourier_fwd_kernel, grid, block, 0, S(stream), xr, Wf, bf, sigma, feat, ld, F, Ntot);
    TVAE_CHECK_LAUNCH();
    return 0;
}

int tvae_fourier_bwd(const float* xr, const float* Wf, const float* bf, float sigma, const float* dfeat, long ld,
                     int F, long Ntot, float* gxr, tvae_stream_t stream) {
    hipLaunchKernelGGL(fourier_bwd_kernel, dim3((unsigned)((Ntot + 255) / 256)), dim3(256), 0, S(stream), xr, Wf, bf,
                       sigma, dfeat, ld, F, Ntot, gxr);
    TVAE_CHECK_LAUNCH();
    return 0;
}

int tvae_loglik_fwd(const float* yh, const float* y, float* lp, int B, int L, int kind, tvae_stream_t stream) {
    if (B <= 0) return 0;
    const int bt = (B < 256 && L >= 16384) ? 1024 : 256;
    hipLaunchKernelGGL(loglik_fwd_kernel, dim3(B), dim3(bt), 0, S(stream), yh, y, lp, L, kind);
    TVAE_CHECK_LAUNCH();
    return 0;
}

int tvae_loglik_bwd(const float* yh, const float* y, const float* glp, float* gyh, int B, int L, int kind,
                    tvae_stream_t stream) {
    hipLaunchKernelGGL(loglik_bwd_kernel, dim3(grid1d((long)B * L, 256)), dim3(256), 0, S(stream), yh, y, glp, gyh, B,
                       L, kind);
    TVAE_CHECK_LAUNCH();
    return 0;
}

int tvae_ctf_corr(const float* in, const float* ctf, float* out, int B, int n, int kc, int flip, tvae_stream_t stream) {
    if (B <= 0) return 0;
    if ((kc & 1) == 0) return (int)hipErrorInvalidValue;
    dim3 grid((n * n + 255) / 256, B), block(256);
    hipLaunchKernelGGL(ctf_corr_kernel, grid, block, 0, S(stream), in, ctf, out, n, kc, flip);
    TVAE_CHECK_LAUNCH();
    return 0;
}

int tvae_loglik_masked_fwd(const float* yh, const float* y, const float* dx, float inv_spacing, float radius, int B,
                           int n, float* lp, tvae_stream_t stream) {
    if (B <= 0) return 0;
    hipLaunchKernelGGL(loglik_masked_fwd_kernel, dim3(B), dim3(256), 0, S(stream), yh, y, dx, inv_spacing, radius, n,
                       lp);
    TVAE_CHECK_LAUNCH();
    return 0;
}

int tvae_loglik_masked_bwd(const float* yh, const float* y, const float* dx, float inv_spacing, float radius, int B,
                           int n, const float* glp, float* gyh, tvae_stream_t stream) {
    hipLaunchKernelGGL(loglik_masked_bwd_kernel, dim3(grid1d((long)B * n * n, 256)), dim3(256), 0, S(stream), yh, y, dx,
                       inv_spacing, radius, n, glp, gyh, B);
    TVAE_CHECK_LAUNCH();
    return 0;
}

int tvae_adam_flat(float* p, const float* g, float* m, float* v, long n, float lr, float b1, float b2, float eps,
                   float bc1, float bc2_sqrt, float grad_scale, tvae_stream_t stream) {
    hipLaunchKernelGGL(adam_flat_kernel, dim3(grid1d(n, 256, 2048)), dim3(256), 0, S(stream), p, g, m, v, n, lr, b1,
                       b2, eps, bc1, bc2_sqrt, grad_scale);
    TVAE_CHECK_LAUNCH();
    return 0;
}
int tvae_dec_in_total(float* part, int B, int cpi, int F, float* Simg, float* dbc, float* dWc, tvae_stream_t stream) {
    if (B <= 0 || F <= 0 || cpi <= 0) return 0;
    hipLaunchKernelGGL(dec_in_total_img_kernel, dim3(B), dim3(256), 0, S(stream), part, cpi, F, Simg);
    TVAE_CHECK_LAUNCH();
    hipLaunchKernelGGL(dec_in_total_sum_kernel, dim3((3 * F + 63) / 64), dim3(256), 0, S(stream), (const float*)part, B, cpi, F,
                       dbc, dWc);
    TVAE_CHECK_LAUNCH();
    return 0;
}

}
```

target-vae_amd/csrc/conv_dft_kernels.hpp:

```cpp
#pragma once
#include <hip/hip_runtime.h>
#include "small_device.hpp"
#include "conv_x6_device.hpp"

namespace tvae {

__device__ __forceinline__ long dft_t_off(long n, int row, int rows2, int Lh) {
    return (((n >> 7) * rows2 + row) * Lh) * 128 + (n & 127);
}

__device__ __forceinline__ float2 cmul(float2 a, float2 b) { return make_float2(a.x * b.x - a.y * b.y, a.x * b.y + a.y * b.x); }

__device__ __forceinline__ void fill_twiddles(float2* tw, int L) {
    for (int j = threadIdx.x; j < L; j += blockDim.x) {
        float s, c;
        sincospif(2.0f * (float)j / (float)L, &s, &c);
        tw[j] = make_float2(c, s);
    }
}

__device__ __forceinline__ void dft_plane_spectrum(float* sm_dft, const float* __restrict__ pl, int S, int pad, int L,
                                                   int fx0, int nfx, int FXB, float2*& Yh, float2*& tw) {
    float2* Rw = reinterpret_cast<float2*>(sm_dft);
    Yh = Rw + S * FXB;
// ... 1045 lines not shown
#pragma unroll
        for (int s_ = 0; s_ < NSR; s_ += 2) {
            acc0 = __builtin_amdgcn_mfma_f32_32x32x2f32(areg[s_], bs[2 * s_], acc0, 0, 0, 0);
            if (s_ + 1 < NSR) acc1 = __builtin_amdgcn_mfma_f32_32x32x2f32(areg[s_ + 1 < NSR ? s_ + 1 : s_], bs[2 * s_ + 2], acc1, 0, 0, 0);
        }
        if (m != m_prev && m_prev >= 0) h3_tile_flush_rd(mx, amax + m_prev, lane);
        m_prev = m;
        if (tile + 1 < t_end) tile_put(slot ^ 1);
        float* p0 = Sp + dft_t_off(n0 + j, m, 2 * M, Lh);
        float* p1 = Sp + dft_t_off(n0 + j, M + m, 2 * M, Lh);
#pragma unroll
        for (int r = 0; r < 16; ++r) {
            const int kk = 32 * rt + (r & 3) + 8 * (r >> 2) + 4 * kh;
            const int fx = kk >> 1;
            const float v = acc0[r] + acc1[r];
            if (fx < Lh) {
                ((kk & 1) ? p1 : p0)[(long)fx * 128] = v;
                mx = fmaxf(mx, fabsf(v));
            }
        }
        dft_lds_barrier();
    }
    if (m_prev >= 0) h3_tile_flush_rd(mx, amax + m_prev, lane);
}

template <int LHR, int NLD>
static __global__ __launch_bounds__(512) void dft_out_wide_kernel(const float* __restrict__ T, const float* __restrict__ EO,
                                                                  const float* __restrict__ bias, float* __restrict__ out,
                                                                  int M, int R, int B, int Ho, int Lh, long NBpad, int NT,
                                                                  int NTW, int act, float slope, float* __restrict__ amax) {
    extern __shared__ __attribute__((aligned(16))) float sm_w[];
    const int lane = threadIdx.x & 63, j = lane & 31, ri = lane >> 5;
    const int wt = __builtin_amdgcn_readfirstlane((int)(threadIdx.x >> 6));
    const int SLOT = LHR * 64, nthr = blockDim.x;
    const bool xrow = NT > NTW;
    float* patch = sm_w + 2 * SLOT + wt * (32 * 33);
    float* ex = sm_w + 2 * SLOT + NTW * (32 * 33);
    float eo[LHR];
#pragma unroll
    for (int fx = 0; fx < LHR; ++fx) eo[fx] = fx < Lh ? EO[((long)fx * NT + wt) * 64 + lane] : 0.f;
    if (xrow)
        for (int i = threadIdx.x; i < 2 * Lh; i += nthr) ex[i] = EO[((long)(i >> 1) * NT + NTW) * 64 + (i & 1) * 32];
    const long tiles_n = NBpad / 32, ntiles = (long)M * tiles_n, NB = (long)B * Ho;
    const int P = Ho * Ho;
    const long per = (ntiles + gridDim.x - 1) / gridDim.x;
    const long t_beg = (long)blockIdx.x * per, t_end = min(ntiles, t_beg + per);
    if (t_beg >= t_end) return;
    const int npc = Lh * 16;
    float4 stage[NLD];
    auto tile_load = [&](long tile) __attribute__((always_inline)) {
        const int m = (int)(tile / tiles_n);
        const long n0 = (tile - (long)m * tiles_n) * 32;
        const float* t0 = T + dft_t_off(n0, m, 2 * M, Lh);
        const float* t1 = T + dft_t_off(n0, M + m, 2 * M, Lh);
#pragma unroll
        for (int i = 0; i < NLD; ++i) {
            const int pc = min(i * nthr + (int)threadIdx.x, npc - 1);
            const int q4 = pc & 7, rr = pc >> 3, fx = rr >> 1;
            stage[i] = *reinterpret_cast<const float4*>(((rr & 1) ? t1 : t0) + (long)fx * 128 + 4 * q4);
        }
    };
    auto tile_put = [&](int slot) __attribute__((always_inline)) {
        float4* dst = reinterpret_cast<float4*>(sm_w + slot * SLOT);
#pragma unroll
        for (int i = 0; i < NLD; ++i) {
            const int pc = i * nthr + (int)threadIdx.x;
            if (pc < npc) dst[pc] = stage[i];
        }
    };
    for (int i = threadIdx.x; i < 2 * SLOT; i += nthr) sm_w[i] = 0.f;
    __syncthreads();
    tile_load(t_beg);
    tile_put(0);
    __syncthreads();
    float amx = 0.f;
    int c_prev = -1;
    for (long tile = t_beg; tile < t_end; ++tile) {
        const int slot = (int)((tile - t_beg) & 1);
        if (tile + 1 < t_end) tile_load(tile + 1);
        const int m = (int)(tile / tiles_n);
        const long n0 = (tile - (long)m * tiles_n) * 32;
        const float* vs = sm_w + slot * SLOT + lane;
        f32x16 acc0, acc1;
#pragma unroll
        for (int r = 0; r < 16; ++r) acc0[r] = acc1[r] = 0.f;
#pragma unroll
        for (int fx = 0; fx < LHR; fx += 2) {
            acc0 = __builtin_amdgcn_mfma_f32_32x32x2f32(eo[fx], vs[fx * 64], acc0, 0, 0, 0);
            if (fx + 1 < LHR) acc1 = __builtin_amdgcn_mfma_f32_32x32x2f32(eo[fx + 1 < LHR ? fx + 1 : fx], vs[(fx + 1) * 64], acc1, 0, 0, 0);
        }
        float racc = 0.f;
        if (xrow && wt == 0) {
            for (int fx = 0; fx < Lh; ++fx) racc = __fmaf_rn(ex[2 * fx + ri], vs[fx * 64], racc);
            racc += __shfl_xor(racc, 32, 64);
        }
        const int c = m / R, r_ = m - c * R;
        if (c != c_prev && c_prev >= 0) h3_tile_flush_rd(amx, amax + c_prev, lane);
        c_prev = c;
        if (tile + 1 < t_end) tile_put(slot ^ 1);
        if (n0 < NB) {
            const float bv = bias ? bias[c] : 0.f;
#pragma unroll
            for (int r = 0; r < 16; ++r) {
                float x = acc0[r] + acc1[r] + bv;
                if (act == ACT_LRELU) x = x > 0.f ? x : x * slope;
                else if (act == ACT_TANH) x = tanhf(x);
                patch[j * 33 + (r & 3) + 8 * (r >> 2) + 4 * ri] = x;
            }
            __builtin_amdgcn_wave_barrier();
            const int tmax = (int)(NB - n0 < 32 ? NB - n0 : 32);
            const int wn = min(32, Ho - 32 * wt);
            const int w = lane & 31;
            const int b0 = (int)(n0 / Ho), h0 = (int)(n0 - (long)b0 * Ho);
            float* obase = out + (((long)c * B + b0) * R + r_) * P + (long)h0 * Ho + 32 * wt + w;
            const long jump = (long)(R - 1) * P;
#pragma unroll 4
            for (int col = lane >> 5; col < tmax; col += 2) {
                if (w < wn) {
                    const int nb = Ho >= 32 ? (h0 + col >= Ho ? 1 : 0) : (h0 + col) / Ho;
                    const float sv = patch[col * 33 + w];
                    amx = fmaxf(amx, fabsf(sv));
                    obase[(long)col * Ho + nb * jump] = sv;
                }
            }
            if (xrow && wt == 0 && ri == 0 && j < tmax) {
                float x = racc + bv;
                if (act == ACT_LRELU) x = x > 0.f ? x : x * slope;
                else if (act == ACT_TANH) x = tanhf(x);
                const int nb = Ho >= 32 ? (h0 + j >= Ho ? 1 : 0) : (h0 + j) / Ho;
                amx = fmaxf(amx, fabsf(x));
                out[(((long)c * B + b0) * R + r_) * P + (long)h0 * Ho + (long)j * Ho + nb * jump + 32 * NTW] = x;
            }
            __builtin_amdgcn_wave_barrier();
        }
        dft_lds_barrier();
    }
    if (c_prev >= 0) h3_tile_flush_rd(amx, amax + c_prev, lane);
}

static __global__ void dft_dbias_rows_kernel(const float* __restrict__ Sp, float* __restrict__ part, int Lh, long NB, int M,
                                             int s16) {
    __shared__ float sm[16];
    const int m = blockIdx.x;
    float acc[1] = {0.f};
    if (s16) {
        const unsigned short* S16p = reinterpret_cast<const unsigned short*>(Sp);
        for (long n = threadIdx.x; n < NB; n += blockDim.x)
            acc[0] += __uint_as_float((unsigned)S16p[dft_t_off(n, m, 2 * M, Lh)] << 16);
    } else
    for (long n = threadIdx.x; n < NB; n += blockDim.x) acc[0] += Sp[dft_t_off(n, m, 2 * M, Lh)];
    block_sum<1>(acc, sm);
    if (threadIdx.x == 0) part[m] = acc[0];
}
static __global__ void dft_dbias_kernel(const float* __restrict__ part, float* __restrict__ db, int R, int C) {
    const int c = blockIdx.x * blockDim.x + threadIdx.x;
    if (c >= C) return;
    float s = 0.f;
    for (int r = 0; r < R; ++r) s += part[c * R + r];
    db[c] = s;
}

static __global__ void dft_dbank_kernel(const float* __restrict__ G, int nsl, long gs, float* __restrict__ dbank, int ksz,
                                        int L, int Lh, int M, int Cin, int FXB) {
    extern __shared__ float sm_dft[];
    float2* Kh = reinterpret_cast<float2*>(sm_dft);
    float2* Z = Kh + L * FXB;
    float2* tw = Z + ksz * FXB;
    float* outp = reinterpret_cast<float*>(tw + L);
    const int m = blockIdx.x / Cin, ci = blockIdx.x - m * Cin;
    fill_twiddles(tw, L);
    for (int i = threadIdx.x; i < ksz * ksz; i += blockDim.x) outp[i] = 0.f;
    const long rowlen = 2L * L * Cin;
    for (int fx0 = 0; fx0 < Lh; fx0 += FXB) {
        const int nfx = min(FXB, Lh - fx0);
        __syncthreads();
        for (int i = threadIdx.x; i < nfx * L; i += blockDim.x) {
            const int fy = i % L, f = i / L;
            const float* r0 = G + ((long)(fx0 + f) * 2 * M + m) * rowlen + (long)(2 * ci) * L;
            const float* r1 = G + ((long)(fx0 + f) * 2 * M + M + m) * rowlen + (long)(2 * ci) * L;
            float a = 0.f, b = 0.f, c = 0.f, d = 0.f;
            for (int sl = 0; sl < nsl; ++sl) {
                a += r0[sl * gs + fy];
                b += r1[sl * gs + L + fy];
                c += r0[sl * gs + L + fy];
                d += r1[sl * gs + fy];
            }
            Kh[fy * FXB + f] = make_float2(a + b, c - d);
        }
        __syncthreads();
        for (int i = threadIdx.x; i < ksz * nfx; i += blockDim.x) {
            const int u = i / nfx, f = i - u * nfx;
            float2 acc = make_float2(0.f, 0.f);
            int ph = 0;
#pragma unroll 4
            for (int fy = 0; fy < L; ++fy) {
                const float2 p = cmul(Kh[fy * FXB + f], tw[ph]);
                acc.x += p.x;
                acc.y += p.y;
                ph += u;
                if (ph >= L) ph -= L;
            }
            Z[u * FXB + f] = acc;
        }
        __syncthreads();
        for (int i = threadIdx.x; i < ksz * ksz; i += blockDim.x) {
            const int u = i / ksz, v = i - u * ksz;
            float acc = 0.f;
            int ph = (int)(((long)fx0 * v) % L);
            for (int f = 0; f < nfx; ++f) {
                const int fx = fx0 + f;
                const float cf = ((fx == 0) || (2 * fx == L)) ? 1.f : 2.f;
                const float2 z = Z[u * FXB + f];
                acc += cf * (z.x * tw[ph].x - z.y * tw[ph].y);
                ph += v;
                if (ph >= L) ph -= L;
            }
            outp[i] += acc;
        }
    }
    const float inv = 1.f / ((float)L * (float)L);
    for (int i = threadIdx.x; i < ksz * ksz; i += blockDim.x) dbank[((long)m * Cin + ci) * ksz * ksz + i] = outp[i] * inv;
}

static __global__ __launch_bounds__(256) void dft_dbank_mf_kernel(const float* __restrict__ G, int nsl, long gs,
                                                                  float* __restrict__ dbank, int ksz, int L, int Lh, int M,
                                                                  int Cin, int FXB) {
    extern __shared__ float sm_dft[];
    float2* Kh = reinterpret_cast<float2*>(sm_dft);
    float2* Z = Kh + L * FXB;
    float2* tw = Z + ksz * FXB;
    float* outp = reinterpret_cast<float*>(tw + L);
    const int m = blockIdx.x / Cin, ci = blockIdx.x - m * Cin;
    const int lane = threadIdx.x & 63, wave = threadIdx.x >> 6, li = lane & 31, kh = lane >> 5;
    const int ut = wave & 1, xt = wave >> 1;
    fill_twiddles(tw, L);
    for (int i = threadIdx.x; i < ksz * ksz; i += blockDim.x) outp[i] = 0.f;
    const long rowlen = 2L * L * Cin;
    const int u = 32 * ut + li;
    for (int fx0 = 0; fx0 < Lh; fx0 += FXB) {
        const int nfx = min(FXB, Lh - fx0);
        __syncthreads();
        for (int i = threadIdx.x; i < nfx * L; i += blockDim.x) {
            const int fy = i % L, f = i / L;
            const float* r0 = G + ((long)(fx0 + f) * 2 * M + m) * rowlen + (long)(2 * ci) * L;
            const float* r1 = G + ((long)(fx0 + f) * 2 * M + M + m) * rowlen + (long)(2 * ci) * L;
            float a = 0.f, b = 0.f, c = 0.f, d = 0.f;
            for (int sl = 0; sl < nsl; ++sl) {
                a += r0[sl * gs + fy];
                b += r1[sl * gs + L + fy];
                c += r0[sl * gs + L + fy];
                d += r1[sl * gs + fy];
            }
            Kh[fy * FXB + f] = make_float2(a + b, c - d);
        }
        __syncthreads();
        if (32 * ut < ksz && 32 * xt < nfx) {
            f32x16 zr, zi;
#pragma unroll
            for (int r = 0; r < 16; ++r) zr[r] = zi[r] = 0.f;
            const int f = min(32 * xt + li, nfx - 1);
            int ph = (kh * u) % L;
            const int dph = (2 * u) % L;
            for (int t = 0; 2 * t < L; ++t) {
                const int fy = 2 * t + kh;
                const float2 w = tw[ph];
                const float2 kv = Kh[min(fy, L - 1) * FXB + f];
                const float ok = fy < L ? 1.f : 0.f;
                const float c = w.x * ok, s_ = w.y * ok;
                zr = __builtin_amdgcn_mfma_f32_32x32x2f32(c, kv.x, zr, 0, 0, 0);
                zr = __builtin_amdgcn_mfma_f32_32x32x2f32(-s_, kv.y, zr, 0, 0, 0);
                zi = __builtin_amdgcn_mfma_f32_32x32x2f32(s_, kv.x, zi, 0, 0, 0);
                zi = __builtin_amdgcn_mfma_f32_32x32x2f32(c, kv.y, zi, 0, 0, 0);
                ph += dph;
                if (ph >= L) ph -= L;
            }
            const int fc = 32 * xt + li;
            if (fc < nfx) {
#pragma unroll
                for (int r = 0; r < 16; ++r) {
                    const int ur = 32 * ut + (r & 3) + 8 * (r >> 2) + 4 * kh;
                    if (ur < ksz) Z[ur * FXB + fc] = make_float2(zr[r], zi[r]);
                }
            }
        }
        __syncthreads();
        if (32 * ut < ksz && 32 * xt < ksz) {
            f32x16 o;
#pragma unroll
            for (int r = 0; r < 16; ++r) o[r] = 0.f;
            const int v = 32 * xt + li;
            const int ua = min(u, ksz - 1);
            int ph = (int)(((long)(fx0 + kh) * v) % L);
            const int dph = (2 * v) % L;
            for (int t = 0; 2 * t < nfx; ++t) {
                const int fl = 2 * t + kh, fx = fx0 + fl;
                const float2 z = Z[ua * FXB + min(fl, nfx - 1)];
                const float cf = fl < nfx ? (((fx == 0) || (2 * fx == L)) ? 1.f : 2.f) : 0.f;
                const float2 w = tw[ph];
                o = __builtin_amdgcn_mfma_f32_32x32x2f32(z.x, cf * w.x, o, 0, 0, 0);
                o = __builtin_amdgcn_mfma_f32_32x32x2f32(z.y, -cf * w.y, o, 0, 0, 0);
                ph += dph;
                if (ph >= L) ph -= L;
            }
            if (v < ksz) {
#pragma unroll
                for (int r = 0; r < 16; ++r) {
// ... 68 lines not shown
```

target-vae_amd/csrc/dense_prepass_kernels.hpp:

```cpp
#pragma once
#include "conv_x6_device.hpp"

namespace tvae {

static __global__ void dense_split3_kernel(const float* __restrict__ W, long ldw, uint4* __restrict__ A3, int Rrows, int Rpad,
                                           int K, int K8pad, int transpose, const float* __restrict__ scale) {
    const long total = (long)K8pad * Rpad;
    for (long i = (long)blockIdx.x * blockDim.x + threadIdx.x; i < total; i += (long)gridDim.x * blockDim.x) {
        const int row = (int)(i % Rpad);
        const int o = (int)(i / Rpad);
        float r[8];
#pragma unroll
        for (int j = 0; j < 8; ++j) {
            const int k = 8 * o + j;
            r[j] = (row < Rrows && k < K) ? (transpose ? W[(long)k * ldw + row] : W[(long)row * ldw + k]) : 0.f;
            if (scale && k < K) r[j] *= scale[k];
        }
        Cell16 h, m, l;
        split3x8(r, h, m, l);
        A3[i] = h.u;
        A3[total + i] = m.u;
        A3[2 * total + i] = l.u;
    }
}

static __global__ __launch_bounds__(1024) void dense_rowmax_kernel(const float* __restrict__ W, long ldw, int Rrows, int Rpad,
                                                                   int K, int transpose, const float* __restrict__ scale,
                                                                   float* __restrict__ rowmax) {
    __shared__ float part[16][64];
    const int r = threadIdx.x & 63, sl = threadIdx.x >> 6;
    const int row = blockIdx.x * 64 + r;
    float mx = 0.f;
    if (row < Rrows)
        for (int k = sl; k < K; k += 16) {
            float v = transpose ? W[(long)k * ldw + row] : W[(long)row * ldw + k];
            if (scale) v *= scale[k];
            mx = fmaxf(mx, fabsf(v));
        }
    part[sl][r] = mx;
    __syncthreads();
    if (sl == 0 && row < Rpad) {
        float t = 0.f;
#pragma unroll
        for (int q = 0; q < 16; ++q) t = fmaxf(t, part[q][r]);
        rowmax[row] = t;
    }
}
static __global__ __launch_bounds__(256) void dense_rowmax_rows_kernel(const float* __restrict__ W, long ldw, int Rrows, int Rpad,
                                                                      int K, const float* __restrict__ scale,
                                                                      float* __restrict__ rowmax) {
    const int lane = threadIdx.x & 63, row = blockIdx.x * 4 + (threadIdx.x >> 6);
    if (row >= Rpad) return;
    float mx = 0.f;
    if (row < Rrows)
        for (int k = lane; k < K; k += 64) {
            float v = W[(long)row * ldw + k];
            if (scale) v *= scale[k];
            mx = fmaxf(mx, fabsf(v));
        }
    mx = h3_wave_max(mx);
    if (lane == 0) rowmax[row] = mx;
}
static __global__ void h3_zero_slots_kernel(float* p, int n) {
    for (int i = threadIdx.x; i < n; i += blockDim.x) p[i] = 0.f;
}
static __global__ void dense_split2h_kernel(const float* __restrict__ W, long ldw, uint4* __restrict__ A3, int Rrows, int Rpad,
                                            int K, int K8pad, int transpose, const float* __restrict__ scale,
                                            const float* __restrict__ rowmax) {
    const long total = (long)K8pad * Rpad;
    for (long i = (long)blockIdx.x * blockDim.x + threadIdx.x; i < total; i += (long)gridDim.x * blockDim.x) {
        const int row = transpose ? (int)(i % Rpad) : (int)(i / K8pad);
        const int o = transpose ? (int)(i / Rpad) : (int)(i % K8pad);
        const long ci = (long)o * Rpad + row;
        const float s = h3_scale(rowmax[row]);
        float r[8];
#pragma unroll
        for (int j = 0; j < 8; ++j) {
            const int k = 8 * o + j;
            r[j] = (row < Rrows && k < K) ? (transpose ? W[(long)k * ldw + row] : W[(long)row * ldw + k]) : 0.f;
            if (scale && k < K) r[j] *= scale[k];
            r[j] *= s;
        }
        Cell16 h, l;
        split2hx8(r, h, l);
        A3[ci] = h.u;
        A3[total + ci] = l.u;
    }
}

static __global__ __launch_bounds__(256) void dense_split2h_rows_kernel(const float* __restrict__ W, long ldw, uint4* __restrict__ A3,
                                                                        int Rrows, int Rpad, int K, int K8pad,
                                                                        const float* __restrict__ scale,
                                                                        const float* __restrict__ rowmax) {
    extern __shared__ __attribute__((aligned(16))) unsigned char split_lds[];
    uint4* Hs = reinterpret_cast<uint4*>(split_lds);
    uint4* Ls = Hs + 32 * K8pad;
    const long total = (long)K8pad * Rpad;
    const int r0 = blockIdx.x * 32, ncell = 32 * K8pad;
    const bool vec = (ldw & 3) == 0 && (reinterpret_cast<size_t>(W) & 15) == 0;
    for (int c = threadIdx.x; c < ncell; c += 256) {
        const int rl = c / K8pad, o = c - rl * K8pad, row = r0 + rl;
        const float s = h3_scale(rowmax[row]);
        float r[8];
        if (vec && row < Rrows && 8 * o + 8 <= K) {
            const float4 a = *reinterpret_cast<const float4*>(W + (long)row * ldw + 8 * o);
            const float4 b = *reinterpret_cast<const float4*>(W + (long)row * ldw + 8 * o + 4);
            r[0] = a.x; r[1] = a.y; r[2] = a.z; r[3] = a.w; r[4] = b.x; r[5] = b.y; r[6] = b.z; r[7] = b.w;
        } else {
#pragma unroll
            for (int j = 0; j < 8; ++j) {
                const int k = 8 * o + j;
                r[j] = (row < Rrows && k < K) ? W[(long)row * ldw + k] : 0.f;
            }
        }
#pragma unroll
        for (int j = 0; j < 8; ++j) {
            const int k = 8 * o + j;
            if (scale && k < K) r[j] *= scale[k];
            r[j] *= s;
        }
        Cell16 h, l;
        split2hx8(r, h, l);
        Hs[o * 32 + rl] = h.u;
        Ls[o * 32 + rl] = l.u;
    }
    __syncthreads();
    for (int c = threadIdx.x; c < ncell; c += 256) {
        const int o = c >> 5, rl = c & 31;
        const long ci = (long)o * Rpad + r0 + rl;
        A3[ci] = Hs[c];
        A3[total + ci] = Ls[c];
    }
}

static __global__ void dec_l0_bound_kernel(const float* __restrict__ xr, long nxr, const float* __restrict__ wc,
                                           const float* __restrict__ bc, const float* __restrict__ lb, long nlb, int K,
                                           float* __restrict__ slots) {
    const long gid = (long)blockIdx.x * blockDim.x + threadIdx.x, gsz = (long)gridDim.x * blockDim.x;
    float m0 = 0.f, m1 = 0.f, m2 = 0.f;
    const long n4 = (reinterpret_cast<size_t>(xr) & 15) == 0 ? nxr / 4 : 0;
    const float4* x4 = reinterpret_cast<const float4*>(xr);
#pragma unroll 4
    for (long i = gid; i < n4; i += gsz) {
        const float4 v = x4[i];
        m0 = fmaxf(fmaxf(m0, fabsf(v.x)), fmaxf(fabsf(v.y), fmaxf(fabsf(v.z), fabsf(v.w))));
    }
    for (long i = 4 * n4 + gid; i < nxr; i += gsz) m0 = fmaxf(m0, fabsf(xr[i]));
    for (long i = gid; i < K; i += gsz) m1 = fmaxf(m1, fabsf(wc[2 * i]) + fabsf(wc[2 * i + 1]));
    if (lb) {
        const long nimg = nlb / K, per = (nimg + 15) / 16;
        for (long t = gid; t < 16L * K; t += gsz) {
            const int k = (int)(t % K);
            const long b0 = (t / K) * per, b1 = b0 + per < nimg ? b0 + per : nimg;
            float v = 0.f;
            for (long b = b0; b < b1; ++b) v = fmaxf(v, fabsf(bc[k] + lb[b * K + k]));
            if (b1 > b0) {
                m2 = fmaxf(m2, v);
                h3_atomic_amax(slots + 4 + k, v);
            }
        }
    } else {
        for (long i = gid; i < K; i += gsz) {
            m2 = fmaxf(m2, fabsf(bc[i]));
            slots[4 + i] = fabsf(bc[i]);
        }
    }
    h3_block_amax(m0, slots);
    h3_block_amax(m1, slots + 1);
    h3_block_amax(m2, slots + 2);
}

static __global__ __launch_bounds__(1024) void dense_rowsum_kernel(const float* __restrict__ W, long ldw, int Rrows, int K,
                                                                   int transpose, const float* __restrict__ scale,
                                                                   float* __restrict__ rowsum) {
    __shared__ float part[16][64];
    const int r = threadIdx.x & 63, sl = threadIdx.x >> 6;
    const int row = blockIdx.x * 64 + r;
    float s = 0.f;
    if (row < Rrows)
        for (int k = sl; k < K; k += 16) {
            float v = transpose ? W[(long)k * ldw + row] : W[(long)row * ldw + k];
            if (scale) v *= scale[k];
            s += v;
        }
    part[sl][r] = s;
    __syncthreads();
    if (sl == 0 && row < Rrows) {
        float t = 0.f;
#pragma unroll
        for (int q = 0; q < 16; ++q) t += part[q][r];
        rowsum[row] = t;
    }
}
}
```

target-vae_amd/csrc/fused_tail_kernels.hpp:

```cpp
#pragma once
#include <hip/hip_runtime.h>
#include "small_kernels.hpp"

namespace tvae {

constexpr int PANEL16 = 1024;
constexpr int PANEL8 = 512;

__device__ __forceinline__ float4 load4(const float* __restrict__ row, long col, long cend, bool vec) {
    if (vec && col + 3 < cend) return *reinterpret_cast<const float4*>(row + col);
    float4 v;
    v.x = col < cend ? row[col] : 0.f;
    v.y = col + 1 < cend ? row[col + 1] : 0.f;
    v.z = col + 2 < cend ? row[col + 2] : 0.f;
    v.w = col + 3 < cend ? row[col + 3] : 0.f;
    return v;
}
__device__ __forceinline__ void store4(float* __restrict__ row, long col, long cend, bool vec, float4 v) {
    if (vec && col + 3 < cend) { *reinterpret_cast<float4*>(row + col) = v; return; }
    if (col < cend) row[col] = v.x;
    if (col + 1 < cend) row[col + 1] = v.y;
    if (col + 2 < cend) row[col + 2] = v.z;
    if (col + 3 < cend) row[col + 3] = v.w;
}
__device__ __forceinline__ float f4get(const float4& v, int e) { return e == 0 ? v.x : (e == 1 ? v.y : (e == 2 ? v.z : v.w)); }

static __global__ void part_total_kernel(const float* __restrict__ part, int npanels, int M, int NV, float* __restrict__ out) {
    __shared__ float sm[16 * 16];
    const int m = blockIdx.x;
    float s[16];
#pragma unroll
    for (int v = 0; v < 16; ++v) s[v] = 0.f;
    for (int p = threadIdx.x; p < npanels; p += blockDim.x) {
        const float* q = part + ((long)p * M + m) * NV;
#pragma unroll
        for (int v = 0; v < 16; ++v)
            if (v < NV) s[v] += q[v];
    }
    block_sum<16>(s, sm);
    if (threadIdx.x == 0) {
#pragma unroll
        for (int v = 0; v < 16; ++v)
            if (v < NV) out[(long)v * M + m] = s[v];
    }
}

constexpr int PT_GROUPS = 64;
static __global__ __launch_bounds__(256) void part_total_s1_kernel(const float* __restrict__ part, int npanels, int MV4,
                                                                  float* __restrict__ partial) {
    const float4* p4 = reinterpret_cast<const float4*>(part);
    const int per = (npanels + PT_GROUPS - 1) / PT_GROUPS;
    const int pb = blockIdx.x * per, pe = min(npanels, pb + per);
    for (int idx = threadIdx.x; idx < MV4; idx += 256) {
        float4 a = make_float4(0.f, 0.f, 0.f, 0.f), b = make_float4(0.f, 0.f, 0.f, 0.f);
        int p = pb;
        for (; p + 1 < pe; p += 2) {
            const float4 u = p4[(long)p * MV4 + idx], v = p4[(long)(p + 1) * MV4 + idx];
            a.x += u.x; a.y += u.y; a.z += u.z; a.w += u.w;
            b.x += v.x; b.y += v.y; b.z += v.z; b.w += v.w;
        }
        if (p < pe) {
            const float4 u = p4[(long)p * MV4 + idx];
            a.x += u.x; a.y += u.y; a.z += u.z; a.w += u.w;
        }
        reinterpret_cast<float4*>(partial)[(long)blockIdx.x * MV4 + idx] = make_float4(a.x + b.x, a.y + b.y, a.z + b.z, a.w + b.w);
    }
}
static __global__ void part_total_s2_kernel(const float* __restrict__ partial, int M, int NV, float* __restrict__ out) {
    const int i = blockIdx.x * blockDim.x + threadIdx.x;
    if (i >= M * NV) return;
    float s = 0.f;
#pragma unroll 8
    for (int g = 0; g < PT_GROUPS; ++g) s += partial[(long)g * M * NV + i];
    const int m = i / NV, v = i - m * NV;
    out[(long)v * M + m] = s;
}

template <int NO>
static __global__ __launch_bounds__(256) void dec_out_bwd_kernel(const float* __restrict__ gy, const float* __restrict__ Wo,
                                                          const float* __restrict__ H, long ldh, float* __restrict__ D,
                                                          long ldd, int F, long N, int act, float slope,
                                                          float* __restrict__ part, int vec) {
    const int lane = threadIdx.x & 63, wave = threadIdx.x >> 6;
    const long c0 = (long)blockIdx.x * PANEL16;
    const long cend = min(N, c0 + PANEL16);
    float g[4][4][NO];
#pragma unroll
    for (int q = 0; q < 4; ++q)
#pragma unroll
        for (int e = 0; e < 4; ++e) {
            const long n = c0 + q * 256 + lane * 4 + e;
#pragma unroll
            for (int o = 0; o < NO; ++o) g[q][e][o] = n < cend ? gy[n * NO + o] : 0.f;
        }
    const int fper = (F + (int)gridDim.y - 1) / (int)gridDim.y;
    const int f_beg = (int)blockIdx.y * fper, f_end = min(F, f_beg + fper);
    for (int f = f_beg + wave; f < f_end; f += 4) {
        float w[NO];
#pragma unroll
        for (int o = 0; o < NO; ++o) w[o] = Wo[(long)o * F + f];
        const float* hrow = H + (long)f * ldh;
        float* drow = D + (long)f * ldd;
        float acc[1 + NO];
#pragma unroll
        for (int v = 0; v <= NO; ++v) acc[v] = 0.f;
        float4 h[4];
#pragma unroll
        for (int q = 0; q < 4; ++q) h[q] = load4(hrow, c0 + q * 256 + lane * 4, cend, vec);
#pragma unroll
        for (int q = 0; q < 4; ++q) {
            float dv[4];
#pragma unroll
            for (int e = 0; e < 4; ++e) {
                const float he = f4get(h[q], e);
                float s = 0.f;
#pragma unroll
                for (int o = 0; o < NO; ++o) {
                    s += w[o] * g[q][e][o];
                    acc[1 + o] += he * g[q][e][o];
                }
                dv[e] = s * act_deriv_from_out(he, act, slope);
                acc[0] += dv[e];
            }
            if (D) store4(drow, c0 + q * 256 + lane * 4, cend, vec, make_float4(dv[0], dv[1], dv[2], dv[3]));
        }
#pragma unroll
        for (int v = 0; v <= NO; ++v) acc[v] = wave_sum(acc[v]);
        if (lane == 0) {
#pragma unroll
            for (int v = 0; v <= NO; ++v) part[((long)blockIdx.x * F + f) * (1 + NO) + v] = acc[v];
        }
    }
}

static __global__ __launch_bounds__(256) void dec_in_bwd_kernel(const float* __restrict__ d, long ldd,
                                                         const float* __restrict__ xr, const float* __restrict__ Wc,
                                                         int F, int Np, int cpi, float* __restrict__ gxr,
                                                         float* __restrict__ part, int vec) {
    __shared__ float sm[4 * PANEL16 * 2];
    const int lane = threadIdx.x & 63, wave = threadIdx.x >> 6;
    const int img = blockIdx.x / cpi, ch = blockIdx.x - img * cpi;
    const long c0 = (long)img * Np + (long)ch * PANEL16;
    const long cend = min((long)(img + 1) * Np, c0 + PANEL16);
    float x0[4][4], x1[4][4], gx0[4][4], gx1[4][4];
#pragma unroll
    for (int q = 0; q < 4; ++q)
#pragma unroll
        for (int e = 0; e < 4; ++e) {
            const long n = c0 + q * 256 + lane * 4 + e;
            x0[q][e] = n < cend ? xr[2 * n] : 0.f;
            x1[q][e] = n < cend ? xr[2 * n + 1] : 0.f;
            gx0[q][e] = 0.f;
            gx1[q][e] = 0.f;
        }
    for (int f = wave; f < F; f += 4) {
        const float wc0 = Wc[2 * f], wc1 = Wc[2 * f + 1];
        const float* drow = d + (long)f * ldd;
        float4 v[4];
#pragma unroll
        for (int q = 0; q < 4; ++q) v[q] = load4(drow, c0 + q * 256 + lane * 4, cend, vec);
        float acc[3] = {0.f, 0.f, 0.f};
#pragma unroll
        for (int q = 0; q < 4; ++q)
#pragma unroll
            for (int e = 0; e < 4; ++e) {
                const float de = f4get(v[q], e);
                gx0[q][e] += wc0 * de;
                gx1[q][e] += wc1 * de;
                acc[0] += de;
                acc[1] += de * x0[q][e];
                acc[2] += de * x1[q][e];
            }
#pragma unroll
        for (int k = 0; k < 3; ++k) acc[k] = wave_sum(acc[k]);
        if (lane == 0) {
#pragma unroll
            for (int k = 0; k < 3; ++k) part[((long)blockIdx.x * F + f) * 3 + k] = acc[k];
        }
    }
#pragma unroll
    for (int q = 0; q < 4; ++q)
#pragma unroll
        for (int e = 0; e < 4; ++e) {
            const int cl = q * 256 + lane * 4 + e;
            sm[(wave * PANEL16 + cl) * 2] = gx0[q][e];
            sm[(wave * PANEL16 + cl) * 2 + 1] = gx1[q][e];
        }
    __syncthreads();
    for (int i = threadIdx.x; i < PANEL16 * 2; i += 256) {
        const long n = c0 + (i >> 1);
        if (n < cend) gxr[2 * n + (i & 1)] = sm[i] + sm[PANEL16 * 2 + i] + sm[2 * PANEL16 * 2 + i] + sm[3 * PANEL16 * 2 + i];
    }
}

static __global__ void dec_in_total_img_kernel(float* __restrict__ part, int cpi, int F, float* __restrict__ Simg) {
    const int b = blockIdx.x, n3 = 3 * F;
    float* base = part + (long)b * cpi * n3;
    for (int e = threadIdx.x; e < n3; e += blockDim.x) {
        float s = 0.f;
#pragma unroll 4
        for (int c = 0; c < cpi; ++c) s += base[(long)c * n3 + e];
        base[e] = s;
        const int f = e / 3;
        if (e - 3 * f == 0) Simg[(long)b * F + f] = s;
    }
}
static __global__ void dec_in_total_sum_kernel(const float* __restrict__ part, int B, int cpi, int F, float* __restrict__ dbc,
                                               float* __restrict__ dWc) {
    __shared__ float sm[4][64];
    const int n3 = 3 * F, e = blockIdx.x * 64 + (threadIdx.x & 63), q = threadIdx.x >> 6;
    float s = 0.f;
    if (e < n3)
        for (int b = q; b < B; b += 4) s += part[(long)b * cpi * n3 + e];
    sm[q][threadIdx.x & 63] = s;
    __syncthreads();
    if (q == 0 && e < n3) {
        const float t = (sm[0][threadIdx.x] + sm[1][threadIdx.x]) + (sm[2][threadIdx.x] + sm[3][threadIdx.x]);
        const int f = e / 3, k = e - 3 * f;
        if (k == 0) dbc[f] = t;
        else dWc[2 * f + k - 1] = t;
    }
}

template <int NO>
static __global__ __launch_bounds__(256) void heads_fwd_kernel(const float* __restrict__ W, const float* __restrict__ X,
                                                        long ldx, const float* __restrict__ bias,
                                                        float* __restrict__ Y, long ldy, int C, long N, int vec) {
    const long col = ((long)blockIdx.x * 256 + threadIdx.x) * 4;
    if (col >= N) return;
    float acc[NO][4];
#pragma unroll
    for (int j = 0; j < NO; ++j) {
        const float b = bias ? bias[j] : 0.f;
#pragma unroll
        for (int e = 0; e < 4; ++e) acc[j][e] = b;
    }
#pragma unroll 8
    for (int c = 0; c < C; ++c) {
        const float4 x = load4(X + (long)c * ldx, col, N, vec);
#pragma unroll
        for (int j = 0; j < NO; ++j) {
            const float w = W[(long)j * C + c];
            acc[j][0] += w * x.x; acc[j][1] += w * x.y; acc[j][2] += w * x.z; acc[j][3] += w * x.w;
        }
    }
#pragma unroll
    for (int j = 0; j < NO; ++j)
        store4(Y + (long)j * ldy, col, N, vec, make_float4(acc[j][0], acc[j][1], acc[j][2], acc[j][3]));
}

template <int NO>
static __global__ __launch_bounds__(256) void heads_bwd_kernel(const float* __restrict__ W, const float* __restrict__ dY,
                                                        long ldy, const float* __restrict__ X, long ldx,
                                                        float* __restrict__ dX, long lddx, int C, long N, int act,
                                                        float slope, float* __restrict__ part, int vec) {
    const int lane = threadIdx.x & 63, wave = threadIdx.x >> 6;
    const long c0 = (long)blockIdx.x * PANEL8;
    const long cend = min(N, c0 + PANEL8);
    float g[2][4][NO];
#pragma unroll
    for (int j = 0; j < NO; ++j)
#pragma unroll
        for (int q = 0; q < 2; ++q) {
            const float4 t = load4(dY + (long)j * ldy, c0 + q * 256 + lane * 4, cend, vec);
            g[q][0][j] = t.x; g[q][1][j] = t.y; g[q][2][j] = t.z; g[q][3][j] = t.w;
        }
    for (int c = wave; c < C; c += 4) {
        float w[NO];
#pragma unroll
        for (int j = 0; j < NO; ++j) w[j] = W[(long)j * C + c];
        const float* xrow = X + (long)c * ldx;
        float* orow = dX + (long)c * lddx;
        float4 x[2];
#pragma unroll
        for (int q = 0; q < 2; ++q) x[q] = load4(xrow, c0 + q * 256 + lane * 4, cend, vec);
        float acc[NO + 1];
#pragma unroll
        for (int v = 0; v <= NO; ++v) acc[v] = 0.f;
#pragma unroll
        for (int q = 0; q < 2; ++q) {
            float dv[4];
#pragma unroll
            for (int e = 0; e < 4; ++e) {
                const float xe = f4get(x[q], e);
                float s = 0.f;
#pragma unroll
                for (int j = 0; j < NO; ++j) {
                    s += w[j] * g[q][e][j];
                    acc[j] += g[q][e][j] * xe;
                }
                dv[e] = s * act_deriv_from_out(xe, act, slope);
                acc[NO] += dv[e];
            }
            if (dX) store4(orow, c0 + q * 256 + lane * 4, cend, vec, make_float4(dv[0], dv[1], dv[2], dv[3]));
        }
        if (NO == 7) {
            float a8[8];
#pragma unroll
            for (int v = 0; v < 8; ++v) a8[v] = acc[v < NO + 1 ? v : 0];
            const float tot = wave_sum8(a8, lane);
            if (lane < 8) part[((long)blockIdx.x * C + c) * (NO + 1) + lane] = tot;
        } else {
#pragma unroll
            for (int v = 0; v <= NO; ++v) acc[v] = wave_sum(acc[v]);
            if (lane == 0) {
#pragma unroll
                for (int v = 0; v <= NO; ++v) part[((long)blockIdx.x * C + c) * (NO + 1) + v] = acc[v];
            }
        }
    }
}

}
```

target-vae_amd/csrc/small_kernels.hpp:

```cpp
#pragma once
#include <hip/hip_runtime.h>
#include "gemm_f32_mfma.hpp"
#include "small_device.hpp"

namespace tvae {


template <int NO>
static __global__ void rowdot_seg_kernel(const float* __restrict__ X, long ldx, const float* __restrict__ V, int N,
                                  int seglen, float* __restrict__ out, int M, float* __restrict__ amax) {
    __shared__ float sm[NO * 16];
    const int m = blockIdx.x, seg = blockIdx.y;
    const int nbeg = seg * seglen;
    const int nend = min(N, nbeg + seglen);
    float acc[NO];
#pragma unroll
    for (int o = 0; o < NO; ++o) acc[o] = 0.f;
    float mx = 0.f;
    const float* xr = X + (long)m * ldx;
    if (!V && ((ldx | nbeg) & 3) == 0 && (reinterpret_cast<size_t>(X) & 15) == 0) {
        const float4* x4 = reinterpret_cast<const float4*>(xr + nbeg);
        const int n4 = (nend - nbeg) >> 2;
        float a0 = 0.f, a1 = 0.f;
        int i = threadIdx.x;
// ... 64 lines not shown

static __global__ __launch_bounds__(1024) void seg_sum_tile_kernel(const float* __restrict__ in, int S, long L,
                                                                   float* __restrict__ out, float scale, int accumulate) {
    __shared__ float sm[16][64];
    const int li = threadIdx.x & 63, sl = threadIdx.x >> 6;
    const long i = (long)blockIdx.x * 64 + li;
    float s0 = 0.f, s1 = 0.f, s2 = 0.f, s3 = 0.f;
    if (i < L) {
        int k = sl;
        for (; k + 48 < S; k += 64) {
            s0 += in[(long)k * L + i];
            s1 += in[(long)(k + 16) * L + i];
            s2 += in[(long)(k + 32) * L + i];
            s3 += in[(long)(k + 48) * L + i];
        }
        for (; k < S; k += 16) s0 += in[(long)k * L + i];
    }
    sm[sl][li] = (s0 + s1) + (s2 + s3);
    __syncthreads();
    if (sl == 0 && i < L) {
        float s = 0.f;
#pragma unroll
        for (int j = 0; j < 16; ++j) s += sm[j][li];
        s *= scale;
        if (accumulate) out[i] += s; else out[i] = s;
    }
}

template <int NO>
static __global__ void coldot_kernel(const float* __restrict__ X, long ldx, int M, int N, const float* __restrict__ W,
                              int wsm, int wso, const float* __restrict__ bias, float* __restrict__ out) {
    extern __shared__ float wsh[];
    for (int i = threadIdx.x; i < M * NO; i += blockDim.x) {
        const int m = i / NO, o = i - m * NO;
        wsh[i] = W[(long)m * wsm + (long)o * wso];
    }
    __syncthreads();
    const int n = blockIdx.x * blockDim.x + threadIdx.x;
    if (n >= N) return;
    float acc[NO];
#pragma unroll
    for (int o = 0; o < NO; ++o) acc[o] = bias ? bias[o] : 0.f;
    for (int m = 0; m < M; ++m) {
        const float x = X[(long)m * ldx + n];
#pragma unroll
        for (int o = 0; o < NO; ++o) acc[o] += wsh[m * NO + o] * x;
    }
#pragma unroll
    for (int o = 0; o < NO; ++o) out[(long)n * NO + o] = acc[o];
}

template <int NO>
static __global__ void outer_mask_kernel(const float* __restrict__ dy, const float* __restrict__ W, int wsm, int wso,
                                  const float* __restrict__ H, long ldh, float* __restrict__ D, long ldd, int M, int N,
                                  int act, float slope) {
    const int n = blockIdx.x * blockDim.x + threadIdx.x;
    if (n >= N) return;
    float g[NO];
#pragma unroll
    for (int o = 0; o < NO; ++o) g[o] = dy[(long)n * NO + o];
    const int mbeg = blockIdx.y * 16;
    const int mend = min(M, mbeg + 16);
    for (int m = mbeg; m < mend; ++m) {
        float s = 0.f;
#pragma unroll
        for (int o = 0; o < NO; ++o) s += W[(long)m * wsm + (long)o * wso] * g[o];
        const float h = H[(long)m * ldh + n];
        D[(long)m * ldd + n] = s * act_deriv_from_out(h, act, slope);
    }
}

static __global__ void act_bwd_kernel(const float* __restrict__ dY, const float* __restrict__ Y, float* __restrict__ dpre,
                               long n, int act, float slope) {
    for (long i = (long)blockIdx.x * blockDim.x + threadIdx.x; i < n; i += (long)gridDim.x * blockDim.x)
        dpre[i] = dY[i] * act_deriv_from_out(Y[i], act, slope);
}

static __global__ void coord_fwd_kernel(const float* __restrict__ xc, const float* __restrict__ dx,
                                 const float* __restrict__ theta, float* __restrict__ xr, int B, int Np) {
    const long total = (long)B * Np;
    for (long i = (long)blockIdx.x * blockDim.x + threadIdx.x; i < total; i += (long)gridDim.x * blockDim.x) {
        const int b = (int)(i / Np), p = (int)(i - (long)b * Np);
        const float c = cosf(theta[b]), s = sinf(theta[b]);
        const float x0 = xc[2 * p] - dx[2 * b], x1 = xc[2 * p + 1] - dx[2 * b + 1];
        xr[2 * i] = x0 * c - x1 * s;
        xr[2 * i + 1] = x0 * s + x1 * c;
    }
}
static __global__ void coord_bwd_kernel(const float* __restrict__ xc, const float* __restrict__ dx,
                                 const float* __restrict__ theta, const float* __restrict__ gxr,
                                 float* __restrict__ gdx, float* __restrict__ gtheta, int Np) {
    __shared__ float sm[3 * 16];
    const int b = blockIdx.x;
    const float c = cosf(theta[b]), s = sinf(theta[b]);
    float acc[3] = {0.f, 0.f, 0.f};
    for (int p = threadIdx.x; p < Np; p += blockDim.x) {
        const float x0 = xc[2 * p] - dx[2 * b], x1 = xc[2 * p + 1] - dx[2 * b + 1];
        const float g0 = gxr[2 * ((long)b * Np + p)], g1 = gxr[2 * ((long)b * Np + p) + 1];
        acc[0] += -(g0 * c + g1 * s);
        acc[1] += g0 * s - g1 * c;
        const float r0 = x0 * c - x1 * s, r1 = x0 * s + x1 * c;
        acc[2] += -g0 * r1 + g1 * r0;
    }
    block_sum<3>(acc, sm);
    if (threadIdx.x == 0) { gdx[2 * b] = acc[0]; gdx[2 * b + 1] = acc[1]; gtheta[b] = acc[2]; }
}

static __global__ void dec_l0_fwd_kernel(const float* __restrict__ xr, const float* __restrict__ Wc,
                                  const float* __restrict__ bc, const float* __restrict__ LB, float* __restrict__ h,
                                  long ldh, int F, long Ntot, int Np, int act, float slope) {
    const long n = (long)blockIdx.x * blockDim.x + threadIdx.x;
    if (n >= Ntot) return;
    const float x0 = xr[2 * n], x1 = xr[2 * n + 1];
    const int img = (int)(n / Np);
    const int fbeg = blockIdx.y * 16, fend = min(F, fbeg + 16);
    for (int f = fbeg; f < fend; ++f) {
        const float v = dec_l0_pre(Wc[2 * f], Wc[2 * f + 1], bc[f], LB ? LB[(long)img * F + f] : 0.f, x0, x1);
        h[(long)f * ldh + n] = act_apply(v, act, slope);
    }
}
static __global__ void latent_bias_kernel(const float* __restrict__ Wl, const float* __restrict__ z, float* __restrict__ LB,
                                   int B, int F, int zd) {
    const int i = blockIdx.x * blockDim.x + threadIdx.x;
    if (i >= B * F) return;
    const int img = i / F, f = i - img * F;
    float s = 0.f;
    for (int d = 0; d < zd; ++d) s += Wl[f * zd + d] * z[img * zd + d];
    LB[i] = s;
}
static __global__ __launch_bounds__(1024) void latent_bwd_kernel(const float* __restrict__ S, const float* __restrict__ Wl,
                                                                 const float* __restrict__ z, float* __restrict__ dWl,
                                                                 float* __restrict__ dz, int B, int F, int zd) {
    __shared__ float part[2][16][64];
    const int o = threadIdx.x & 63, sl = threadIdx.x >> 6;
    const int i = blockIdx.x * 64 + o;
    float s0 = 0.f, s1 = 0.f;
    if (i < F * zd) {
        const int f = i / zd, d = i - f * zd;
        for (int b = sl; b < B; b += 16) s0 += S[(long)b * F + f] * z[b * zd + d];
    }
    if (i < B * zd) {
        const int b = i / zd, d = i - b * zd;
        for (int f = sl; f < F; f += 16) s1 += Wl[f * zd + d] * S[(long)b * F + f];
    }
    part[0][sl][o] = s0;
    part[1][sl][o] = s1;
    __syncthreads();
    if (sl < 2) {
        float t = 0.f;
#pragma unroll
        for (int q = 0; q < 16; ++q) t += part[sl][q][o];
        if (sl == 0 && i < F * zd) dWl[i] = t;
        if (sl == 1 && i < B * zd) dz[i] = t;
    }
}

static __global__ void fourier_fwd_kernel(const float* __restrict__ xr, const float* __restrict__ Wf,
                                   const float* __restrict__ bf, float sigma, float* __restrict__ feat, long ld, int F,
                                   long Ntot) {
    __shared__ float wsm[16][3];
    const long n = (long)blockIdx.x * blockDim.x + threadIdx.x;
    const int fbeg = blockIdx.y * 16, fend = min(F, fbeg + 16);
    if ((int)threadIdx.x < fend - fbeg) {
        const int f = fbeg + threadIdx.x;
        wsm[threadIdx.x][0] = Wf[2 * f] / sigma;
        wsm[threadIdx.x][1] = Wf[2 * f + 1] / sigma;
        wsm[threadIdx.x][2] = bf[f];
    }
    __syncthreads();
    if (n >= Ntot) return;
    const float x0 = xr[2 * n], x1 = xr[2 * n + 1];
    for (int f = fbeg; f < fend; ++f) {
        const float w0 = wsm[f - fbeg][0], w1 = wsm[f - fbeg][1];
        feat[(long)f * ld + n] = cosf(x0 * w0 + x1 * w1 + wsm[f - fbeg][2]);
    }
}
static __global__ void fourier_bwd_kernel(const float* __restrict__ xr, const float* __restrict__ Wf,
                                   const float* __restrict__ bf, float sigma, const float* __restrict__ dfeat, long ld,
                                   int F, long Ntot, float* __restrict__ gxr) {
    __shared__ float wsm[256][3];
    const long n = (long)blockIdx.x * blockDim.x + threadIdx.x;
    const bool live = n < Ntot;
    const float x0 = live ? xr[2 * n] : 0.f, x1 = live ? xr[2 * n + 1] : 0.f;
    float g0 = 0.f, g1 = 0.f;
    for (int f0 = 0; f0 < F; f0 += 256) {
        __syncthreads();
        if (f0 + (int)threadIdx.x < F) {
            const int f = f0 + threadIdx.x;
            wsm[threadIdx.x][0] = Wf[2 * f] / sigma;
            wsm[threadIdx.x][1] = Wf[2 * f + 1] / sigma;
            wsm[threadIdx.x][2] = bf[f];
        }
        __syncthreads();
        const int fe = min(256, F - f0);
        if (live)
            for (int q = 0; q < fe; ++q) {
                const float w0 = wsm[q][0], w1 = wsm[q][1];
                const float a_ = x0 * w0 + x1 * w1 + wsm[q][2];
                const float t_ = a_ * 0.15915494f;
                const float e_ = __fmaf_rn(a_, 6.4206383e-09f, __fmaf_rn(a_, 0.15915494f, -t_));
                const float t = -__builtin_amdgcn_sinf(__builtin_amdgcn_fractf(t_) + e_) * dfeat[(long)(f0 + q) * ld + n];
                g0 += t * w0;
                g1 += t * w1;
            }
    }
    if (live) {
        gxr[2 * n] = g0;
        gxr[2 * n + 1] = g1;
    }
}

__device__ __forceinline__ float gauss_sub(float acc, float d) {
#pragma clang fp contract(off)
    const float t = (0.5f * d) * d;
    return acc - t;
}
static __global__ void loglik_fwd_kernel(const float* __restrict__ yh, const float* __restrict__ y, float* __restrict__ lp,
                                  int L, int kind) {
    __shared__ float sm[16];
    const int b = blockIdx.x;
    const long ldy = kind == 2 ? 2L * L : L;
    const float* a = yh + (long)b * ldy;
    const float* t = y + (long)b * L;
    float acc[1] = {0.f};
    for (int i = threadIdx.x; i < L; i += blockDim.x) {
        const float x = a[i], yy = t[i];
        if (kind == 0) acc[0] -= fmaxf(x, 0.f) - x * yy + log1pf(expf(-fabsf(x)));
        else if (kind == 1) acc[0] = gauss_sub(acc[0], x - yy);
        else { const float lv = a[L + i]; acc[0] -= 0.5f * ((x - yy) * (x - yy) * expf(-lv) + lv); }
    }
    block_sum<1>(acc, sm);
    if (threadIdx.x == 0) lp[b] = acc[0];
}
static __global__ void loglik_bwd_kernel(const float* __restrict__ yh, const float* __restrict__ y,
                                  const float* __restrict__ glp, float* __restrict__ gyh, int B, int L, int kind) {
    const long total = (long)B * L;
    const long ldy = kind == 2 ? 2L * L : L;
    for (long i = (long)blockIdx.x * blockDim.x + threadIdx.x; i < total; i += (long)gridDim.x * blockDim.x) {
        const int b = (int)(i / L), j = (int)(i - (long)b * L);
        const float g = glp[b];
        const float x = yh[(long)b * ldy + j], yy = y[i];
        if (kind == 0) gyh[(long)b * ldy + j] = -g * (1.f / (1.f + expf(-x)) - yy);
        else if (kind == 1) gyh[(long)b * ldy + j] = -g * (x - yy);
        else {
            const float lv = yh[(long)b * ldy + L + j];
            const float e = expf(-lv), d = x - yy;
            gyh[(long)b * ldy + j] = -g * d * e;
            gyh[(long)b * ldy + L + j] = -0.5f * g * (1.f - d * d * e);
        }
    }
}


static __global__ void ctf_corr_kernel(const float* __restrict__ in, const float* __restrict__ ctf, float* __restrict__ out,
                                int n, int kc, int flip) {
    const int b = blockIdx.y;
    const int pix = blockIdx.x * blockDim.x + threadIdx.x;
    if (pix >= n * n) return;
    const int i = pix / n, j = pix - i * n;
    const int p = kc / 2;
    const float* src = in + (long)b * n * n;
    const float* w = ctf + (long)b * kc * kc;
    float acc = 0.f;
    for (int a = 0; a < kc; ++a) {
        const int ii = i + a - p;
        if (ii < 0 || ii >= n) continue;
        const float* wr = flip ? (w + (long)(kc - 1 - a) * kc) : (w + (long)a * kc);
        const float* sr = src + (long)ii * n;
        for (int c = 0; c < kc; ++c) {
            const int jj = j + c - p;
            if (jj >= 0 && jj < n) acc += sr[jj] * (flip ? wr[kc - 1 - c] : wr[c]);
        }
    }
    out[(long)b * n * n + pix] = acc;
}

__device__ __forceinline__ bool mask_keep(int i, int j, int n, float cx, float cy, float r2) {
    const float gx = (float)(j - (n + 1) / 2);
    const float gy = (float)(n / 2 - i);
    const float ddx = cx - gx, ddy = cy - gy;
    return ddx * ddx + ddy * ddy < r2;
}
static __global__ void loglik_masked_fwd_kernel(const float* __restrict__ yh, const float* __restrict__ y,
                                         const float* __restrict__ dx, float inv_spacing, float radius, int n,
                                         float* __restrict__ lp) {
    __shared__ float sm[16];
    const int b = blockIdx.x;
    const int L = n * n;
    const float cx = dx[2 * b] * inv_spacing, cy = dx[2 * b + 1] * inv_spacing, r2 = radius * radius;
    float acc[1] = {0.f};
    for (int t = threadIdx.x; t < L; t += blockDim.x) {
        const int i = t / n, j = t - i * n;
        if (mask_keep(i, j, n, cx, cy, r2)) {
            acc[0] = gauss_sub(acc[0], yh[(long)b * L + t] - y[(long)b * L + t]);
        }
    }
    block_sum<1>(acc, sm);
    if (threadIdx.x == 0) lp[b] = acc[0];
}
static __global__ void loglik_masked_bwd_kernel(const float* __restrict__ yh, const float* __restrict__ y,
                                         const float* __restrict__ dx, float inv_spacing, float radius, int n,
                                         const float* __restrict__ glp, float* __restrict__ gyh, int B) {
    const long L = (long)n * n, total = (long)B * L;
    const float r2 = radius * radius;
    for (long t = (long)blockIdx.x * blockDim.x + threadIdx.x; t < total; t += (long)gridDim.x * blockDim.x) {
        const int b = (int)(t / L);
// ... 533 lines not shown
```

target-vae_amd/tvae/_lib.py:

```python
from __future__ import annotations

import ctypes
import os

import torch

_HERE = os.path.dirname(os.path.abspath(__file__))
LIB_PATH = os.environ.get('TVAE_LIB') or os.path.join(os.path.dirname(_HERE), 'csrc', 'build', 'libtvae_hip.so')

SIGNATURES = {
    'tvae_rotate_bank_fwd': 'ppppiiii',
    'tvae_rotate_bank_bwd': 'ppppppiiiii',
    'tvae_conv1_fwd': 'ppppiiiiiiiif',
    'tvae_conv1_wgrad': 'ppppl iiiiiii'.replace(' ', ''),
    'tvae_bank_split3': 'ppliiii',
    'tvae_conv1_fwd_x6': 'ppppiiiiiiiif',
    'tvae_dy_split3': 'ppliiiiiii',
    'tvae_conv1_wgrad_x6': 'ppppliiiiiii',
    'tvae_conv1_fwd_dft': 'ppppppliiiiiiiifi',
    'tvae_conv1_wgrad_dft': 'pppppliiiiiiii',
    'tvae_dense_split3': 'plpliiipp',
    'tvae_dense_split2h': 'plpliiipp',
    'tvae_linear_fwd_x6': 'pppppiiillifpppppppipipp',
    'tvae_linear_dgrad_x6': 'pppppiiillifpppplpppppiplppppippppp',
    'tvae_dec_in_total': 'piiippp',
    'tvae_dgrad_rowsum_total': 'piippfpppp',
    'tvae_linear_wgrad_x6': 'ppppliiillippifppppipiplpppi',
    'tvae_linear_fwd': 'ppppippiiillif',
    'tvae_linear_dgrad': 'pppppiiillif',
    'tvae_linear_wgrad': 'ppppliiilli',
    'tvae_rowdot_seg': 'plpiiiipp',
    'tvae_seg_sum': 'pilpfi',
    'tvae_coldot': 'pliipiipip',
    'tvae_outer_mask': 'pipiiplpliiif',
    'tvae_act_bwd': 'ppplif',
    'tvae_dec_out_bwd': 'pipplplilifplp',
    'tvae_dec_in_bwd': 'plppiiipppppl',
    'tvae_heads_fwd': 'pplppliil',
    'tvae_heads_bwd': 'pplplpliilifplp',
    'tvae_attn_head_fwd': 'plpppppppiiiiffppppppppl',
    'tvae_attn_head_bwd': 'plppppppppiiiiffpppppppppl',
    'tvae_get_latent': 'plpppiiiifppp',
    'tvae_enc_tail_fwd_x6': 'pplpppiplplppilifip',
    'tvae_enc_tail_dgrad_x6': 'ppplippplilfi',
    'tvae_enc_tail_wgrad_x6': 'plplipppplilfip',
    'tvae_enc_tail_fwd_wide': 'ppplppiplplppilifip',
    'tvae_enc_tail_dgrad_wide': 'ppplippplplilfip',
    'tvae_enc_tail_wgrad_wide': 'pliplpplilpp',
    'tvae_rot_pool_fwd': 'ppppiiii',
    'tvae_rot_pool_bwd': 'ppppplpiiiiif',
    'tvae_coord_fwd': 'ppppii',
    'tvae_coord_bwd': 'ppppppii',
    'tvae_dec_l0_fwd': 'pppppliliif',
    'tvae_latent_bias': 'pppiii',
    'tvae_latent_bwd': 'pppppiii',
    'tvae_fourier_fwd': 'pppfplil',
    'tvae_fourier_bwd': 'pppfplilp',
    'tvae_loglik_fwd': 'pppiii',
    'tvae_loglik_bwd': 'ppppiii',
    'tvae_elbo_reduce': 'ppippp',
    'tvae_elbo_reduce_bwd': 'pppipp',
    'tvae_ctf_corr': 'pppiiii',
    'tvae_loglik_masked_fwd': 'pppffiip',
    'tvae_loglik_masked_bwd': 'pppffiipp',
    'tvae_adam_flat': 'pppplfffffff',
}

QUERIES = {
    'tvae_conv1_x6_supported': ('iiii', 'i'),
    'tvae_conv1_x6_bank_bytes': ('iiii', 'l'),
    'tvae_conv1_x6_dy_bytes': ('iiiiii', 'l'),
    'tvae_dense_x6_bytes': ('ii', 'l'),
    'tvae_conv1_dft_supported': ('iiiiiii', 'i'),
    'tvae_conv1_dft_at_floats': ('iiiiiii', 'l'),
    'tvae_conv1_dft_ws_floats': ('iiiiiii', 'l'),
    'tvae_conv1_dft_frame': ('iiiiiii', 'i'),
    'tvae_conv1_dft_ring': ('iiiiiii', 'i'),
    'tvae_conv1_dft_route': ('iiiiiiiii', 'i'),
    'tvae_enc_tail_wgrad_x6_ws_floats': ('l', 'l'),
    'tvae_enc_tail_wide_max_rows': ('', 'i'),
    'tvae_linear_wgrad_x6_ws_floats': ('iii', 'l'),
}

OPTIONAL_TAIL = {'tvae_linear_wgrad_x6': 6}

_CT = {'p': ctypes.c_void_p, 'i': ctypes.c_int, 'l': ctypes.c_long, 'f': ctypes.c_float}
_lib = None


class TvaeHipError(RuntimeError):
    pass


def lib():
    global _lib
    if _lib is None:
        if not os.path.exists(LIB_PATH):
            raise TvaeHipError(
                f'{LIB_PATH} not found: build it with `make -C target-vae_amd/csrc` '
                '(or __graft_entry__.build()).  There is no CPU fallback.')
        L = ctypes.CDLL(LIB_PATH)
        for name, sig in SIGNATURES.items():
            fn = getattr(L, name)
            fn.restype = ctypes.c_int
            fn.argtypes = [_CT[c] for c in sig] + [ctypes.c_void_p]
        for name, (sig, ret) in QUERIES.items():
            fn = getattr(L, name)
            fn.restype = _CT[ret]
            fn.argtypes = [_CT[c] for c in sig]
        L.tvae_abi_version.restype = ctypes.c_int
        if L.tvae_abi_version() != ABI_VERSION:
            raise TvaeHipError(f'{LIB_PATH} has ABI version {L.tvae_abi_version()}, this package needs {ABI_VERSION}: rebuild')
        _lib = L
    return _lib


ABI_VERSION = 7
GEMM_MODES = ('f32', 'x6', 'h3', 'bf16')
_mode = os.environ.get('TVAE_GEMM', 'h3')
if _mode not in GEMM_MODES:
    raise TvaeHipError(f'TVAE_GEMM={_mode!r}: choose from {GEMM_MODES}')


def set_gemm_mode(mode: str) -> None:
    global _mode
    if mode not in GEMM_MODES:
        raise TvaeHipError(f'unknown GEMM mode {mode!r}; choose from {GEMM_MODES}')
    _mode = mode


def get_gemm_mode() -> str:
    return _mode


def split_pipe() -> bool:
    return _mode in ('x6', 'h3', 'bf16')


def parts() -> int:
    return {'bf16': 1, 'h3': 2}.get(_mode, 3)


class arithmetic:

    def __init__(self, mode: str):
        if mode not in GEMM_MODES:
            raise TvaeHipError(f'unknown GEMM mode {mode!r}; choose from {GEMM_MODES}')
        self.mode = mode

    def __enter__(self):
        global _mode
        self.old, _mode = _mode, self.mode
        return self

    def __exit__(self, *exc):
        global _mode
        _mode = self.old
        return False


RCCL_SYMBOLS = ('tvae_rccl_available', 'tvae_rccl_unique_id', 'tvae_rccl_comm_init', 'tvae_allreduce_flat',
                'tvae_rccl_comm_destroy')


def exported_symbols():
    return ['tvae_abi_version'] + sorted(SIGNATURES) + sorted(QUERIES) + list(RCCL_SYMBOLS)


class RcclComm:

    @staticmethod
    def _check_instance():
        import sys
        src = lib().tvae_rccl_available()
        if not src:
            raise TvaeHipError('no RCCL library could be resolved in this process')
        if src == 2 and 'torch.distributed' in sys.modules and os.environ.get('TVAE_RCCL_OWN_COPY', '0') != '1':
            import torch.distributed as dist
            if dist.is_available() and dist.is_nccl_available():
                raise TvaeHipError('libtvae_hip.so would load a SECOND copy of RCCL beside the one torch.distributed uses '
                                   '(RTLD_NOLOAD found none): set TVAE_RCCL_OWN_COPY=1 to allow it')
        return src

    def __init__(self, nranks: int, id128: bytes, rank: int):
        L = lib()
        self._comm = ctypes.c_void_p()
        self.instance = self._check_instance()
        buf = ctypes.create_string_buffer(bytes(id128), 128)
        rc = L.tvae_rccl_comm_init(ctypes.byref(self._comm), int(nranks), buf, int(rank))
        if rc:
            raise TvaeHipError(f'tvae_rccl_comm_init failed ({_rccl_rc(rc)})')

    @staticmethod
    def unique_id() -> bytes:
        RcclComm._check_instance()
        buf = ctypes.create_string_buffer(128)
        rc = lib().tvae_rccl_unique_id(buf)
        if rc:
            raise TvaeHipError(f'tvae_rccl_unique_id failed ({_rccl_rc(rc)})')
        return buf.raw

    def all_reduce_(self, t) -> None:
        if not (t.is_cuda and t.dtype == torch.float32 and t.is_contiguous()):
            raise TvaeHipError('tvae_allreduce_flat: contiguous fp32 CUDA tensor expected')
        if not self._comm:
            raise TvaeHipError('tvae_allreduce_flat on a closed communicator')
        L = lib()
        L.tvae_allreduce_flat.argtypes = [ctypes.c_void_p, ctypes.c_void_p, ctypes.c_long, ctypes.c_void_p]
        rc = L.tvae_allreduce_flat(self._comm, t.data_ptr(), t.numel(), torch.cuda.current_stream().cuda_stream)
        if rc:
            raise TvaeHipError(f'tvae_allreduce_flat failed ({_rccl_rc(rc)})')

    def close(self) -> None:
        if getattr(self, '_comm', None):
            lib().tvae_rccl_comm_destroy(self._comm)
            self._comm = ctypes.c_void_p()

    def __del__(self):
        try:
            self.close()
        except Exception:
            pass


_NCCL_RESULT = {1: 'ncclUnhandledCudaError', 2: 'ncclSystemError', 3: 'ncclInternalError', 4: 'ncclInvalidArgument',
                5: 'ncclInvalidUsage', 6: 'ncclRemoteError', 7: 'ncclInProgress'}


def _rccl_rc(rc: int) -> str:
    if rc == 100001:
        return 'no RCCL library resolved'
    if rc > 100100:
        return f'ncclResult_t {rc - 100100} {_NCCL_RESULT.get(rc - 100100, "?")}'
    return f'hipError_t {rc}'


def query(name, *args) -> int:
    sig, _ = QUERIES[name]
    if len(args) != len(sig):
        raise TvaeHipError(f'{name}: expected {len(sig)} arguments, got {len(args)}')
    return int(getattr(lib(), name)(*[int(a) for a in args]))


_F64_OK = {('tvae_elbo_reduce', 3), ('tvae_elbo_reduce', 5), ('tvae_elbo_reduce_bwd', 0), ('tvae_elbo_reduce_bwd', 2)}
_F64_OK |= {('tvae_ward_merge', p) for p in (0, 4, 6, 11, 13)}
_F64_OK |= {('tvae_tsne_repulsion', 3), ('tvae_tsne_step', 6), ('tvae_tsne_step', 11)}
_F64_OK |= {('tvae_tsne_kl', p) for p in (6, 7, 8)}
_F64_OK |= {('tvae_class_frc', 3)}
_F64_OK |= {('tvae_image_normalize', 2)}
_F64_OK |= {('tvae_ctf_eval', 0), ('tvae_fourier_filter', 2), ('tvae_ctf_power', 0), ('tvae_ctf_power', 3)}


def _ptr(t, name, pos):
    if t is None:
        return None
    if not torch.is_tensor(t):
        raise TvaeHipError(f'{name} arg {pos}: expected a tensor or None, got {type(t)}')
    if not t.is_cuda:
        raise TvaeHipError(f'{name} arg {pos}: tensor must live on the GPU (no CPU fallback)')
    if (name, pos) in _F64_OK:
        if t.dtype != torch.float64:
            raise TvaeHipError(f'{name} arg {pos}: dtype {t.dtype}, the C ABI takes double* here')
    elif t.dtype not in (torch.float32, torch.int32):
        raise TvaeHipError(f'{name} arg {pos}: dtype {t.dtype} not supported (fp32 / int32 only)')
    if not t.is_contiguous():
        raise TvaeHipError(f'{name} arg {pos}: tensor must be contiguous')
    return t.data_ptr()


CALL_HOOK = None


def set_call_hook(hook):
    global CALL_HOOK
    old, CALL_HOOK = CALL_HOOK, hook
    return old


def call(name, *args):
    sig = SIGNATURES[name]
    if len(args) < len(sig) and (set(sig[len(args):]) == {'p'} or len(sig) - len(args) <= OPTIONAL_TAIL.get(name, 0)):
        args = args + tuple(None if c == 'p' else 0 for c in sig[len(args):])
    if len(args) != len(sig):
        raise TvaeHipError(f'{name}: expected {len(sig)} arguments, got {len(args)}')
    hook = CALL_HOOK
    if hook is not None and not torch.cuda.is_current_stream_capturing():
        return hook(name, sig, tuple(args), lambda a: _launch(name, sig, a))
# ... 18 lines not shown
```

Baseline: 29040.

## Add side-fusion path fusing small prepass and reduction kernels with wider unrolled loads

Adds a runtime toggle, on by default, that sends several small side kernels to new versions. Row-max and fp16 split are fused into one kernel. The decoder L0 bound, slot zeroing and grad absmax are merged into a two-pass kernel using workspace scratch. The latent backward grid is split so dWl and dz are separate block ranges, and several reductions (dbias rows, part totals, dec_in totals) get 8-way unrolled loads or a 2D grid. The goal is fewer launches and more memory-level parallelism in these minor kernels, at the cost of extra code paths and scratch-size conditions.

Result: slower. 28600 (-1.5%).

```diff
diff --git a/include/tvae_hip.h b/include/tvae_hip.h
--- a/include/tvae_hip.h
+++ b/include/tvae_hip.h
@@ -7,6 +7,8 @@
 typedef void* tvae_stream_t;
 
 int tvae_abi_version(void);
+
+int tvae_side_fusion(int on);
 
 
 int tvae_rotate_bank_fwd(const float* weight, const int* tap_idx, const float* tap_w, float* bank, int C, int Cin,
diff --git a/target-vae_amd/csrc/abi_common.hpp b/target-vae_amd/csrc/abi_common.hpp
--- a/target-vae_amd/csrc/abi_common.hpp
+++ b/target-vae_amd/csrc/abi_common.hpp
@@ -49,6 +49,8 @@
     return g;
 }
 
+TVAE_INTERNAL bool side_fusion();
+
 static const size_t X6_LDS_MAX = 160 * 1024;
 
 TVAE_INTERNAL int splitk_finalize(const float* ws, int splits, int M, int N, const Epilogue& ep, hipStream_t stream);
diff --git a/target-vae_amd/csrc/abi_conv_dft.hip b/target-vae_amd/csrc/abi_conv_dft.hip
--- a/target-vae_amd/csrc/abi_conv_dft.hip
+++ b/target-vae_amd/csrc/abi_conv_dft.hip
@@ -550,8 +550,12 @@
     }
     if (dbias) {
         float* dbpart = ED + ((q.ed_floats + 3) & ~3L);
-        hipLaunchKernelGGL(dft_dbias_rows_kernel, dim3(q.M), dim3(256), 0, st, (const float*)Sp, dbpart, q.Lh, q.NB, q.M,
-                           s16 ? 1 : 0);
+        if (side_fusion())
+            hipLaunchKernelGGL(dft_dbias_rows_wide_kernel, dim3(q.M), dim3(256), 0, st, (const float*)Sp, dbpart, q.Lh, q.NB, q.M,
+                               s16 ? 1 : 0);
+        else
+            hipLaunchKernelGGL(dft_dbias_rows_kernel, dim3(q.M), dim3(256), 0, st, (const float*)Sp, dbpart, q.Lh, q.NB, q.M,
+                               s16 ? 1 : 0);
         TVAE_CHECK_LAUNCH();
         hipLaunchKernelGGL(dft_dbias_kernel, dim3((C + 63) / 64), dim3(64), 0, st, (const float*)dbpart, dbias, R, C);
         TVAE_CHECK_LAUNCH();
diff --git a/target-vae_amd/csrc/abi_dense_wgrad_x6.hip b/target-vae_amd/csrc/abi_dense_wgrad_x6.hip
--- a/target-vae_amd/csrc/abi_dense_wgrad_x6.hip
+++ b/target-vae_amd/csrc/abi_dense_wgrad_x6.hip
@@ -120,14 +120,19 @@
                                       H3Scale{a_amax, x_amax, 0, 0, 0, x_amax_rows ? 1 : 0, x_amax_rows ? K : 0});
     } else if (parts == 2) {
         float* slots = ws + (long)splits * per;
-        rc = h3_zero_slots(slots, 4 + K, 256, S(stream));
-        if (rc) return rc;
         const long nlb = va_lb ? (long)(N / vas.Np) * K : 0;
-        rc = dec_l0_bound(va_xr, N, va_wc, va_bc, va_lb, nlb, K, slots, S(stream));
-        if (rc) return rc;
-        hipLaunchKernelGGL(dense_absmax_kernel, dim3(grid1d((long)N, 256 * 8, 512)), dim3(256), 0, S(stream), vg_gy, (long)N, 1, N,
-                           0, (const float*)nullptr, slots + 3);
-        TVAE_CHECK_LAUNCH();
+        if (side_fusion() && K <= 512 && dec_l0_bound_scratch_floats(N, K) <= (long)splits * per) {
+            rc = dec_l0_bound_fused(va_xr, N, va_wc, va_bc, va_lb, nlb, K, vg_gy, slots, ws, S(stream));
+            if (rc) return rc;
+        } else {
+            rc = h3_zero_slots(slots, 4 + K, 256, S(stream));
+            if (rc) return rc;
+            rc = dec_l0_bound(va_xr, N, va_wc, va_bc, va_lb, nlb, K, slots, S(stream));
+            if (rc) return rc;
+            hipLaunchKernelGGL(dense_absmax_kernel, dim3(grid1d((long)N, 256 * 8, 512)), dim3(256), 0, S(stream), vg_gy, (long)N, 1,
+                               N, 0, (const float*)nullptr, slots + 3);
+            TVAE_CHECK_LAUNCH();
+        }
         rc = dense_wgrad_x6_launch_p2(variant, dpre, ldd, X, ldx, ws, M, K, N, nchunk, tmk, DenseBatch{0, 0, 0}, 0L, vgs, vas,
                                       ATILE_PLAIN, S(stream), H3Scale{nullptr, slots, 0, 0, 0, 0, 0});
     } else {
diff --git a/target-vae_amd/csrc/abi_dense_x6.hip b/target-vae_amd/csrc/abi_dense_x6.hip
--- a/target-vae_amd/csrc/abi_dense_x6.hip
+++ b/target-vae_amd/csrc/abi_dense_x6.hip
@@ -40,6 +40,19 @@
                  hipStream_t st) {
     hipLaunchKernelGGL(dec_l0_bound_kernel, dim3(grid1d(N / 2, 256, 512)), dim3(256), 0, st, xr, 2L * N, wc, bc, lb, nlb, K,
                        slots);
+    return (int)hipGetLastError();
+}
+static int dec_l0_bound_groups(int N) { return grid1d(N / 2, 1024, 256); }
+long dec_l0_bound_scratch_floats(int N, int K) { return 2L * dec_l0_bound_groups(N) + (long)DEC_BOUND_CHUNKS * K; }
+int dec_l0_bound_fused(const float* xr, int N, const float* wc, const float* bc, const float* lb, long nlb, int K, const float* gy,
+                       float* slots, float* scratch, hipStream_t st) {
+    const int G = dec_l0_bound_groups(N);
+    float* pk = scratch + 2 * G;
+    hipLaunchKernelGGL(dec_l0_bound_p1_kernel, dim3(G), dim3(1024), 0, st, xr, 2L * N, bc, lb, nlb, K, gy, (long)N, scratch, pk);
+    hipError_t e = hipGetLastError();
+    if (e != hipSuccess) return (int)e;
+    hipLaunchKernelGGL(dec_l0_bound_p2_kernel, dim3(1), dim3(1024), 0, st, (const float*)scratch, G, (const float*)pk, lb ? 1 : 0,
+                       wc, bc, K, slots);
     return (int)hipGetLastError();
 }
 
@@ -139,14 +152,26 @@
     const long total = (long)K8pad * Rpad;
     if (parts == 2) {
         float* tr = h3_trailer(a3, rows, K);
-        if (transpose)
-            hipLaunchKernelGGL(dense_rowmax_kernel, dim3(Rpad / 64), dim3(1024), 0, S(stream), W, ldw, rows, Rpad, K, transpose,
-                               scale, tr);
-        else
-            hipLaunchKernelGGL(dense_rowmax_rows_kernel, dim3(Rpad / 4), dim3(256), 0, S(stream), W, ldw, rows, Rpad, K, scale, tr);
-        TVAE_CHECK_LAUNCH();
-        const int rc = dense_split2h(W, ldw, (uint4*)a3, rows, Rpad, K, K8pad, transpose, scale, tr, S(stream));
-        if (rc) return rc;
+        if (side_fusion() && transpose) {
+            hipLaunchKernelGGL(dense_maxsplit2h_t_kernel, dim3(Rpad / 64), dim3(1024), 0, S(stream), W, ldw, (uint4*)a3, rows, Rpad,
+                               K, K8pad, scale, tr, rowsum);
+            TVAE_CHECK_LAUNCH();
+            return 0;
+        }
+        if (side_fusion()) {
+            hipLaunchKernelGGL(dense_maxsplit2h_wave_kernel, dim3(Rpad / 4), dim3(256), 0, S(stream), W, ldw, (uint4*)a3, rows, Rpad,
+                               K, K8pad, scale, tr);
+            TVAE_CHECK_LAUNCH();
+        } else {
+            if (transpose)
+                hipLaunchKernelGGL(dense_rowmax_kernel, dim3(Rpad / 64), dim3(1024), 0, S(stream), W, ldw, rows, Rpad, K, transpose,
+                                   scale, tr);
+            else
+                hipLaunchKernelGGL(dense_rowmax_rows_kernel, dim3(Rpad / 4), dim3(256), 0, S(stream), W, ldw, rows, Rpad, K, scale, tr);
+            TVAE_CHECK_LAUNCH();
+            const int rc = dense_split2h(W, ldw, (uint4*)a3, rows, Rpad, K, K8pad, transpose, scale, tr, S(stream));
+            if (rc) return rc;
+        }
     } else {
         hipLaunchKernelGGL(dense_split3_kernel, dim3(grid1d(total, 256)), dim3(256), 0, S(stream), W, ldw, (uint4*)a3, rows,
                            Rpad, K, K8pad, transpose, scale);
@@ -185,10 +210,16 @@
         hs.a_rows = 1;
         if (va.xr) {
             float* bw = tr + Rpad;
-            int rc = h3_zero_slots(bw, 4 + K, 256, st);
-            if (rc) return rc;
             const long nlb = va.lb ? (long)(N / va.Np) * K : 0;
-            rc = dec_l0_bound(va.xr, N, va.wc, va.bc, va.lb, nlb, K, bw, st);
+            const long third = (long)K8pad * Rpad * 4;
+            int rc;
+            if (side_fusion() && K <= 512 && Rpad + 4 + K + dec_l0_bound_scratch_floats(N, K) <= third) {
+                rc = dec_l0_bound_fused(va.xr, N, va.wc, va.bc, va.lb, nlb, K, nullptr, bw, bw + 4 + K, st);
+            } else {
+                rc = h3_zero_slots(bw, 4 + K, 256, st);
+                if (rc) return rc;
+                rc = dec_l0_bound(va.xr, N, va.wc, va.bc, va.lb, nlb, K, bw, st);
+            }
             if (rc) return rc;
             hs.amax_x = bw;
         } else if (x_amax && !vg.wo && !vg.csum) {
diff --git a/target-vae_amd/csrc/abi_dense_x6.hpp b/target-vae_amd/csrc/abi_dense_x6.hpp
--- a/target-vae_amd/csrc/abi_dense_x6.hpp
+++ b/target-vae_amd/csrc/abi_dense_x6.hpp
@@ -49,6 +49,9 @@
                                 const float* scale, const float* rowmax, hipStream_t st);
 TVAE_INTERNAL int dec_l0_bound(const float* xr, int N, const float* wc, const float* bc, const float* lb, long nlb, int K,
                                float* slots, hipStream_t st);
+TVAE_INTERNAL long dec_l0_bound_scratch_floats(int N, int K);
+TVAE_INTERNAL int dec_l0_bound_fused(const float* xr, int N, const float* wc, const float* bc, const float* lb, long nlb, int K,
+                                     const float* gy, float* slots, float* scratch, hipStream_t st);
 
 TVAE_INTERNAL int dense_x6_batched4(const void* w3, const float* X, long ldx, const Epilogue& ep, int rows_per_problem,
                                     int rows_total, int N, int K, const TileMap& tm, const DenseBatch& bt, int parts,
diff --git a/target-vae_amd/csrc/abi_small.hip b/target-vae_amd/csrc/abi_small.hip
--- a/target-vae_amd/csrc/abi_small.hip
+++ b/target-vae_amd/csrc/abi_small.hip
@@ -18,9 +18,25 @@
                        C, N, act, slope, part, vec);
 }
 
+namespace {
+int side_fusion_default() {
+    const char* e = std::getenv("TVAE_SIDE_FUSION");
+    return (e && e[0] == '0' && e[1] == '\0') ? 0 : 1;
+}
+int g_side_fusion = side_fusion_default();
+}
+namespace tvae {
+bool side_fusion() { return g_side_fusion != 0; }
+}
+
 extern "C" {
 
 int tvae_abi_version(void) { return 7; }
+
+int tvae_side_fusion(int on) {
+    if (on >= 0) g_side_fusion = on ? 1 : 0;
+    return g_side_fusion;
+}
 
 int tvae_rotate_bank_fwd(const float* weight, const int* tap_idx, const float* tap_w, float* bank, int C, int Cin,
                          int ksz, int R, tvae_stream_t stream) {
@@ -204,8 +220,12 @@
     const long used = (long)np * C * (nh + 1), mv = (long)C * (nh + 1);
     if (np >= 4 * PT_GROUPS && mv % 4 == 0 && part_floats >= ((used + 3) & ~3L) + PT_GROUPS * mv && aligned16(part)) {
         float* partial = part + ((used + 3) & ~3L);
-        hipLaunchKernelGGL(part_total_s1_kernel, dim3(PT_GROUPS), dim3(256), 0, S(stream), (const float*)part, np, (int)(mv / 4),
-                           partial);
+        if (side_fusion())
+            hipLaunchKernelGGL(part_total_s1_wide_kernel, dim3(PT_GROUPS), dim3(256), 0, S(stream), (const float*)part, np,
+                               (int)(mv / 4), partial);
+        else
+            hipLaunchKernelGGL(part_total_s1_kernel, dim3(PT_GROUPS), dim3(256), 0, S(stream), (const float*)part, np, (int)(mv / 4),
+                               partial);
         TVAE_CHECK_LAUNCH();
         hipLaunchKernelGGL(part_total_s2_kernel, dim3((unsigned)((mv + 255) / 256)), dim3(256), 0, S(stream),
                            (const float*)partial, C, nh + 1, tot);
@@ -359,6 +379,12 @@
                     tvae_stream_t stream) {
     const int tot = (F * zd > B * zd) ? F * zd : B * zd;
     if (tot <= 0) return 0;
+    if (side_fusion()) {
+        const int gw = (F * zd + 63) / 64, gz = (B * zd + 63) / 64;
+        hipLaunchKernelGGL(latent_bwd_wide_kernel, dim3(gw + gz), dim3(1024), 0, S(stream), S_, Wl, z, dWl, dz, B, F, zd, gw);
+        TVAE_CHECK_LAUNCH();
+        return 0;
+    }
     hipLaunchKernelGGL(latent_bwd_kernel, dim3((tot + 63) / 64), dim3(1024), 0, S(stream), S_, Wl, z, dWl, dz, B, F, zd);
     TVAE_CHECK_LAUNCH();
     return 0;
@@ -431,6 +457,14 @@
 }
 int tvae_dec_in_total(float* part, int B, int cpi, int F, float* Simg, float* dbc, float* dWc, tvae_stream_t stream) {
     if (B <= 0 || F <= 0 || cpi <= 0) return 0;
+    if (side_fusion()) {
+        hipLaunchKernelGGL(dec_in_total_img_wide_kernel, dim3(B, (3 * F + 255) / 256), dim3(256), 0, S(stream), part, cpi, F, Simg);
+        TVAE_CHECK_LAUNCH();
+        hipLaunchKernelGGL(dec_in_total_sum_wide_kernel, dim3((3 * F + 63) / 64), dim3(256), 0, S(stream), (const float*)part, B,
+                           cpi, F, dbc, dWc);
+        TVAE_CHECK_LAUNCH();
+        return 0;
+    }
     hipLaunchKernelGGL(dec_in_total_img_kernel, dim3(B), dim3(256), 0, S(stream), part, cpi, F, Simg);
     TVAE_CHECK_LAUNCH();
     hipLaunchKernelGGL(dec_in_total_sum_kernel, dim3((3 * F + 63) / 64), dim3(256), 0, S(stream), (const float*)part, B, cpi, F,
diff --git a/target-vae_amd/csrc/conv_dft_kernels.hpp b/target-vae_amd/csrc/conv_dft_kernels.hpp
--- a/target-vae_amd/csrc/conv_dft_kernels.hpp
+++ b/target-vae_amd/csrc/conv_dft_kernels.hpp
@@ -1221,6 +1221,40 @@
     block_sum<1>(acc, sm);
     if (threadIdx.x == 0) part[m] = acc[0];
 }
+static __global__ void dft_dbias_rows_wide_kernel(const float* __restrict__ Sp, float* __restrict__ part, int Lh, long NB, int M,
+                                                  int s16) {
+    __shared__ float sm[16];
+    const int m = blockIdx.x;
+    const unsigned short* S16p = reinterpret_cast<const unsigned short*>(Sp);
+    float acc[1] = {0.f};
+    if (s16) {
+        for (long n0 = threadIdx.x; n0 < NB; n0 += 8L * blockDim.x) {
+            float v[8];
+#pragma unroll
+            for (int u = 0; u < 8; ++u) {
+                const long n = n0 + (long)u * blockDim.x;
+                v[u] = n < NB ? __uint_as_float((unsigned)S16p[dft_t_off(n, m, 2 * M, Lh)] << 16) : 0.f;
+            }
+#pragma unroll
+            for (int u = 0; u < 8; ++u)
+                if (n0 + (long)u * blockDim.x < NB) acc[0] += v[u];
+        }
+    } else {
+        for (long n0 = threadIdx.x; n0 < NB; n0 += 8L * blockDim.x) {
+            float v[8];
+#pragma unroll
+            for (int u = 0; u < 8; ++u) {
+                const long n = n0 + (long)u * blockDim.x;
+                v[u] = n < NB ? Sp[dft_t_off(n, m, 2 * M, Lh)] : 0.f;
+            }
+#pragma unroll
+            for (int u = 0; u < 8; ++u)
+                if (n0 + (long)u * blockDim.x < NB) acc[0] += v[u];
+        }
+    }
+    block_sum<1>(acc, sm);
+    if (threadIdx.x == 0) part[m] = acc[0];
+}
 static __global__ void dft_dbias_kernel(const float* __restrict__ part, float* __restrict__ db, int R, int C) {
     const int c = blockIdx.x * blockDim.x + threadIdx.x;
     if (c >= C) return;
diff --git a/target-vae_amd/csrc/dense_prepass_kernels.hpp b/target-vae_amd/csrc/dense_prepass_kernels.hpp
--- a/target-vae_amd/csrc/dense_prepass_kernels.hpp
+++ b/target-vae_amd/csrc/dense_prepass_kernels.hpp
@@ -130,6 +130,98 @@
         const long ci = (long)o * Rpad + r0 + rl;
         A3[ci] = Hs[c];
         A3[total + ci] = Ls[c];
+    }
+}
+
+static __global__ __launch_bounds__(256) void dense_maxsplit2h_wave_kernel(const float* __restrict__ W, long ldw, uint4* __restrict__ A3,
+                                                                           int Rrows, int Rpad, int K, int K8pad,
+                                                                           const float* __restrict__ scale,
+                                                                           float* __restrict__ rowmax) {
+    const int lane = threadIdx.x & 63, row = blockIdx.x * 4 + (threadIdx.x >> 6);
+    if (row >= Rpad) return;
+    const long total = (long)K8pad * Rpad;
+    float mx = 0.f;
+    if (row < Rrows)
+        for (int k = lane; k < K; k += 64) {
+            float v = W[(long)row * ldw + k];
+            if (scale) v *= scale[k];
+            mx = fmaxf(mx, fabsf(v));
+        }
+    mx = h3_wave_max(mx);
+    if (lane == 0) rowmax[row] = mx;
+    const float s = h3_scale(mx);
+    for (int o = lane; o < K8pad; o += 64) {
+        const long ci = (long)o * Rpad + row;
+        float r[8];
+#pragma unroll
+        for (int j = 0; j < 8; ++j) {
+            const int k = 8 * o + j;
+            r[j] = (row < Rrows && k < K) ? W[(long)row * ldw + k] : 0.f;
+            if (scale && k < K) r[j] *= scale[k];
+            r[j] *= s;
+        }
+        Cell16 h, l;
+        split2hx8(r, h, l);
+        A3[ci] = h.u;
+        A3[total + ci] = l.u;
+    }
+}
+static __global__ __launch_bounds__(1024) void dense_maxsplit2h_t_kernel(const float* __restrict__ W, long ldw, uint4* __restrict__ A3,
+                                                                         int Rrows, int Rpad, int K, int K8pad,
+                                                                         const float* __restrict__ scale, float* __restrict__ rowmax,
+                                                                         float* __restrict__ rowsum) {
+    __shared__ float pmax[16][64], psum[16][64], rmax[64];
+    const int r = threadIdx.x & 63, sl = threadIdx.x >> 6;
+    const int row = blockIdx.x * 64 + r;
+    const long total = (long)K8pad * Rpad;
+    float mx = 0.f, s = 0.f;
+    if (row < Rrows)
+        for (int k0 = sl; k0 < K; k0 += 128) {
+            float v[8];
+#pragma unroll
+            for (int u = 0; u < 8; ++u) {
+                const int k = k0 + 16 * u;
+                v[u] = k < K ? W[(long)k * ldw + row] : 0.f;
+                if (scale && k < K) v[u] *= scale[k];
+            }
+#pragma unroll
+            for (int u = 0; u < 8; ++u)
+                if (k0 + 16 * u < K) {
+                    mx = fmaxf(mx, fabsf(v[u]));
+                    s += v[u];
+                }
+        }
+    pmax[sl][r] = mx;
+    psum[sl][r] = s;
+    __syncthreads();
+    if (sl == 0) {
+        float t = 0.f;
+#pragma unroll
+        for (int q = 0; q < 16; ++q) t = fmaxf(t, pmax[q][r]);
+        rowmax[row] = t;
+        rmax[r] = t;
+    } else if (sl == 1 && rowsum && row < Rrows) {
+        float t = 0.f;
+#pragma unroll
+        for (int q = 0; q < 16; ++q) t += psum[q][r];
+        rowsum[row] = t;
+    }
+    __syncthreads();
+    const float sc = h3_scale(rmax[r]);
+    for (int o = sl; o < K8pad; o += 16) {
+        const long ci = (long)o * Rpad + row;
+        float v[8];
+#pragma unroll
+        for (int j = 0; j < 8; ++j) {
+            const int k = 8 * o + j;
+            v[j] = (row < Rrows && k < K) ? W[(long)k * ldw + row] : 0.f;
+            if (scale && k < K) v[j] *= scale[k];
+            v[j] *= sc;
+        }
+        Cell16 h, l;
+        split2hx8(v, h, l);
+        A3[ci] = h.u;
+        A3[total + ci] = l.u;
     }
 }
 
@@ -170,6 +262,97 @@
     h3_block_amax(m2, slots + 2);
 }
 
+constexpr int DEC_BOUND_CHUNKS = 16;
+static __global__ __launch_bounds__(1024) void dec_l0_bound_p1_kernel(const float* __restrict__ xr, long nxr,
+                                                                      const float* __restrict__ bc, const float* __restrict__ lb,
+                                                                      long nlb, int K, const float* __restrict__ gy, long ngy,
+                                                                      float* __restrict__ pw, float* __restrict__ pk) {
+    __shared__ float red[2][16];
+    const long gid = (long)blockIdx.x * blockDim.x + threadIdx.x, gsz = (long)gridDim.x * blockDim.x;
+    float m0 = 0.f, m3 = 0.f;
+    const long n4 = (reinterpret_cast<size_t>(xr) & 15) == 0 ? nxr / 4 : 0;
+    const float4* x4 = reinterpret_cast<const float4*>(xr);
+#pragma unroll 4
+    for (long i = gid; i < n4; i += gsz) {
+        const float4 v = x4[i];
+        m0 = fmaxf(fmaxf(m0, fabsf(v.x)), fmaxf(fabsf(v.y), fmaxf(fabsf(v.z), fabsf(v.w))));
+    }
+    for (long i = 4 * n4 + gid; i < nxr; i += gsz) m0 = fmaxf(m0, fabsf(xr[i]));
+    if (gy) {
+        const long g4 = (reinterpret_cast<size_t>(gy) & 15) == 0 ? ngy / 4 : 0;
+        const float4* y4 = reinterpret_cast<const float4*>(gy);
+#pragma unroll 4
+        for (long i = gid; i < g4; i += gsz) {
+            const float4 v = y4[i];
+            m3 = fmaxf(fmaxf(m3, fabsf(v.x)), fmaxf(fabsf(v.y), fmaxf(fabsf(v.z), fabsf(v.w))));
+        }
+        for (long i = 4 * g4 + gid; i < ngy; i += gsz) m3 = fmaxf(m3, fabsf(gy[i]));
+    }
+    if (lb) {
+        const long nimg = nlb / K, per = (nimg + DEC_BOUND_CHUNKS - 1) / DEC_BOUND_CHUNKS;
+        for (long t = gid; t < (long)DEC_BOUND_CHUNKS * K; t += gsz) {
+            const int k = (int)(t % K);
+            const long b0 = (t / K) * per, b1 = b0 + per < nimg ? b0 + per : nimg;
+            const float bk = bc[k];
+            float v = 0.f;
+#pragma unroll 4
+            for (long b = b0; b < b1; ++b) v = fmaxf(v, fabsf(bk + lb[b * K + k]));
+            pk[t] = v;
+        }
+    }
+    m0 = h3_wave_max(m0);
+    m3 = h3_wave_max(m3);
+    if ((threadIdx.x & 63) == 0) {
+        red[0][threadIdx.x >> 6] = m0;
+        red[1][threadIdx.x >> 6] = m3;
+    }
+    __syncthreads();
+    if (threadIdx.x < 2) {
+        float m = red[threadIdx.x][0];
+        for (int i = 1; i < (int)((blockDim.x + 63) >> 6); ++i) m = fmaxf(m, red[threadIdx.x][i]);
+        pw[2 * blockIdx.x + threadIdx.x] = m;
+    }
+}
+static __global__ __launch_bounds__(1024) void dec_l0_bound_p2_kernel(const float* __restrict__ pw, int G, const float* __restrict__ pk,
+                                                                      int has_lb, const float* __restrict__ wc,
+                                                                      const float* __restrict__ bc, int K,
+                                                                      float* __restrict__ slots) {
+    __shared__ float red[4][16];
+    float m[4] = {0.f, 0.f, 0.f, 0.f};
+    for (int g = threadIdx.x; g < G; g += blockDim.x) {
+        m[0] = fmaxf(m[0], pw[2 * g]);
+        m[3] = fmaxf(m[3], pw[2 * g + 1]);
+    }
+    for (int k = threadIdx.x; k < K; k += blockDim.x) {
+        m[1] = fmaxf(m[1], fabsf(wc[2 * k]) + fabsf(wc[2 * k + 1]));
+        float v;
+        if (has_lb) {
+            float c[DEC_BOUND_CHUNKS];
+#pragma unroll
+            for (int q = 0; q < DEC_BOUND_CHUNKS; ++q) c[q] = pk[(long)q * K + k];
+            v = 0.f;
+#pragma unroll
+            for (int q = 0; q < DEC_BOUND_CHUNKS; ++q) v = fmaxf(v, c[q]);
+        } else {
+            v = fabsf(bc[k]);
+        }
+        m[2] = fmaxf(m[2], v);
+        slots[4 + k] = v;
+    }
+#pragma unroll
+    for (int j = 0; j < 4; ++j) m[j] = h3_wave_max(m[j]);
+    if ((threadIdx.x & 63) == 0) {
+#pragma unroll
+        for (int j = 0; j < 4; ++j) red[j][threadIdx.x >> 6] = m[j];
+    }
+    __syncthreads();
+    if (threadIdx.x < 4) {
+        float t = red[threadIdx.x][0];
+        for (int i = 1; i < (int)((blockDim.x + 63) >> 6); ++i) t = fmaxf(t, red[threadIdx.x][i]);
+        slots[threadIdx.x] = t;
+    }
+}
+
 static __global__ __launch_bounds__(1024) void dense_rowsum_kernel(const float* __restrict__ W, long ldw, int Rrows, int K,
                                                                    int transpose, const float* __restrict__ scale,
                                                                    float* __restrict__ rowsum) {
diff --git a/target-vae_amd/csrc/fused_tail_kernels.hpp b/target-vae_amd/csrc/fused_tail_kernels.hpp
--- a/target-vae_amd/csrc/fused_tail_kernels.hpp
+++ b/target-vae_amd/csrc/fused_tail_kernels.hpp
@@ -54,6 +54,36 @@
     for (int idx = threadIdx.x; idx < MV4; idx += 256) {
         float4 a = make_float4(0.f, 0.f, 0.f, 0.f), b = make_float4(0.f, 0.f, 0.f, 0.f);
         int p = pb;
+        for (; p + 1 < pe; p += 2) {
+            const float4 u = p4[(long)p * MV4 + idx], v = p4[(long)(p + 1) * MV4 + idx];
+            a.x += u.x; a.y += u.y; a.z += u.z; a.w += u.w;
+            b.x += v.x; b.y += v.y; b.z += v.z; b.w += v.w;
+        }
+        if (p < pe) {
+            const float4 u = p4[(long)p * MV4 + idx];
+            a.x += u.x; a.y += u.y; a.z += u.z; a.w += u.w;
+        }
+        reinterpret_cast<float4*>(partial)[(long)blockIdx.x * MV4 + idx] = make_float4(a.x + b.x, a.y + b.y, a.z + b.z, a.w + b.w);
+    }
+}
+static __global__ __launch_bounds__(256) void part_total_s1_wide_kernel(const float* __restrict__ part, int npanels, int MV4,
+                                                                       float* __restrict__ partial) {
+    const float4* p4 = reinterpret_cast<const float4*>(part);
+    const int per = (npanels + PT_GROUPS - 1) / PT_GROUPS;
+    const int pb = blockIdx.x * per, pe = min(npanels, pb + per);
+    for (int idx = threadIdx.x; idx < MV4; idx += 256) {
+        float4 a = make_float4(0.f, 0.f, 0.f, 0.f), b = make_float4(0.f, 0.f, 0.f, 0.f);
+        int p = pb;
+        for (; p + 7 < pe; p += 8) {
+            float4 u[8];
+#pragma unroll
+            for (int j = 0; j < 8; ++j) u[j] = p4[(long)(p + j) * MV4 + idx];
+#pragma unroll
+            for (int j = 0; j < 8; j += 2) {
+                a.x += u[j].x; a.y += u[j].y; a.z += u[j].z; a.w += u[j].w;
+                b.x += u[j + 1].x; b.y += u[j + 1].y; b.z += u[j + 1].z; b.w += u[j + 1].w;
+            }
+        }
         for (; p + 1 < pe; p += 2) {
             const float4 u = p4[(long)p * MV4 + idx], v = p4[(long)(p + 1) * MV4 + idx];
             a.x += u.x; a.y += u.y; a.z += u.z; a.w += u.w;
@@ -222,6 +252,47 @@
     }
 }
 
+static __global__ __launch_bounds__(256) void dec_in_total_img_wide_kernel(float* part, int cpi, int F, float* __restrict__ Simg) {
+    const int b = blockIdx.x, n3 = 3 * F, e = blockIdx.y * 256 + threadIdx.x;
+    if (e >= n3) return;
+    float* base = part + (long)b * cpi * n3;
+    float s = 0.f;
+    for (int c0 = 0; c0 < cpi; c0 += 8) {
+        float v[8];
+#pragma unroll
+        for (int u = 0; u < 8; ++u) v[u] = c0 + u < cpi ? base[(long)(c0 + u) * n3 + e] : 0.f;
+#pragma unroll
+        for (int u = 0; u < 8; ++u)
+            if (c0 + u < cpi) s += v[u];
+    }
+    base[e] = s;
+    const int f = e / 3;
+    if (e - 3 * f == 0) Simg[(long)b * F + f] = s;
+}
+static __global__ __launch_bounds__(256) void dec_in_total_sum_wide_kernel(const float* __restrict__ part, int B, int cpi, int F,
+                                                                          float* __restrict__ dbc, float* __restrict__ dWc) {
+    __shared__ float sm[4][64];
+    const int n3 = 3 * F, e = blockIdx.x * 64 + (threadIdx.x & 63), q = threadIdx.x >> 6;
+    float s = 0.f;
+    if (e < n3)
+        for (int b0 = q; b0 < B; b0 += 32) {
+            float v[8];
+#pragma unroll
+            for (int u = 0; u < 8; ++u) v[u] = b0 + 4 * u < B ? part[(long)(b0 + 4 * u) * cpi * n3 + e] : 0.f;
+#pragma unroll
+            for (int u = 0; u < 8; ++u)
+                if (b0 + 4 * u < B) s += v[u];
+        }
+    sm[q][threadIdx.x & 63] = s;
+    __syncthreads();
+    if (q == 0 && e < n3) {
+        const float t = (sm[0][threadIdx.x] + sm[1][threadIdx.x]) + (sm[2][threadIdx.x] + sm[3][threadIdx.x]);
+        const int f = e / 3, k = e - 3 * f;
+        if (k == 0) dbc[f] = t;
+        else dWc[2 * f + k - 1] = t;
+    }
+}
+
 template <int NO>
 static __global__ __launch_bounds__(256) void heads_fwd_kernel(const float* __restrict__ W, const float* __restrict__ X,
                                                         long ldx, const float* __restrict__ bias,
diff --git a/target-vae_amd/csrc/small_kernels.hpp b/target-vae_amd/csrc/small_kernels.hpp
--- a/target-vae_amd/csrc/small_kernels.hpp
+++ b/target-vae_amd/csrc/small_kernels.hpp
@@ -240,6 +240,59 @@
         for (int q = 0; q < 16; ++q) t += part[sl][q][o];
         if (sl == 0 && i < F * zd) dWl[i] = t;
         if (sl == 1 && i < B * zd) dz[i] = t;
+    }
+}
+
+static __global__ __launch_bounds__(1024) void latent_bwd_wide_kernel(const float* __restrict__ S, const float* __restrict__ Wl,
+                                                                      const float* __restrict__ z, float* __restrict__ dWl,
+                                                                      float* __restrict__ dz, int B, int F, int zd, int gw) {
+    __shared__ float part[16][64];
+    const int o = threadIdx.x & 63, sl = threadIdx.x >> 6;
+    const bool isw = (int)blockIdx.x < gw;
+    const int i = (isw ? blockIdx.x : blockIdx.x - gw) * 64 + o;
+    float s = 0.f;
+    if (isw) {
+        if (i < F * zd) {
+            const int f = i / zd, d = i - f * zd;
+            for (int b0 = sl; b0 < B; b0 += 128) {
+                float a[8], c[8];
+#pragma unroll
+                for (int u = 0; u < 8; ++u) {
+                    const int b = b0 + 16 * u;
+                    a[u] = b < B ? S[(long)b * F + f] : 0.f;
+                    c[u] = b < B ? z[b * zd + d] : 0.f;
+                }
+#pragma unroll
+                for (int u = 0; u < 8; ++u)
+                    if (b0 + 16 * u < B) s += a[u] * c[u];
+            }
+        }
+    } else if (i < B * zd) {
+        const int b = i / zd, d = i - b * zd;
+        for (int f0 = sl; f0 < F; f0 += 128) {
+            float a[8], c[8];
+#pragma unroll
+            for (int u = 0; u < 8; ++u) {
+                const int f = f0 + 16 * u;
+                a[u] = f < F ? Wl[f * zd + d] : 0.f;
+                c[u] = f < F ? S[(long)b * F + f] : 0.f;
+            }
+#pragma unroll
+            for (int u = 0; u < 8; ++u)
+                if (f0 + 16 * u < F) s += a[u] * c[u];
+        }
+    }
+    part[sl][o] = s;
+    __syncthreads();
+    if (sl == 0) {
+        float t = 0.f;
+#pragma unroll
+        for (int q = 0; q < 16; ++q) t += part[q][o];
+        if (isw) {
+            if (i < F * zd) dWl[i] = t;
+        } else if (i < B * zd) {
+            dz[i] = t;
+        }
     }
 }
 
diff --git a/target-vae_amd/tvae/_lib.py b/target-vae_amd/tvae/_lib.py
--- a/target-vae_amd/tvae/_lib.py
+++ b/target-vae_amd/tvae/_lib.py
@@ -80,6 +80,7 @@
     'tvae_enc_tail_wgrad_x6_ws_floats': ('l', 'l'),
     'tvae_enc_tail_wide_max_rows': ('', 'i'),
     'tvae_linear_wgrad_x6_ws_floats': ('iii', 'l'),
+    'tvae_side_fusion': ('i', 'i'),
 }
 
 OPTIONAL_TAIL = {'tvae_linear_wgrad_x6': 6}
@@ -133,6 +134,17 @@
     return _mode
 
 
+def set_side_fusion(on: bool) -> bool:
+    L = lib()
+    old = bool(L.tvae_side_fusion(-1))
+    L.tvae_side_fusion(1 if on else 0)
+    return old
+
+
+def get_side_fusion() -> bool:
+    return bool(lib().tvae_side_fusion(-1))
+
+
 def split_pipe() -> bool:
     return _mode in ('x6', 'h3', 'bf16')
 
```
